# SpaceLearner/SessionRec-pytorch

Measured on AMD Instinct MI355X. Metric: sessions/sec training, Yoochoose-1/64 batch 512, higher is better.
Workload: dtype bf16 (MFMA operands; fp32 accumulate, master weights, scoring); 1 GPU; MSGIFSR training step, synthetic Yoochoose-1/64 shape (V=37484 items, d=256, batch 512 per GPU, session length<=20, order 3, dropout 0.1); global_batch=512, parallelism=single GPU

## Files before the change

### include/srec.h

```cpp
#ifndef SREC_H
#define SREC_H
#include "srec_hg.h"

#ifdef __cplusplus
extern "C" {
#endif

#define SREC_BAD_ARG 1001

int srec_gemm_f32(const float* A, int a_rs, int a_cs, const float* B, int b_rs, int b_cs, float* C, int ldc,
                  const float* bias, int M, int N, int K, const int* dyn, int dyn_mode, float alpha, float beta,
                  float* ws, long ws_floats, void* stream);

int srec_gemm_bf16_nt(const float* A, int lda, const float* B, int ldb, float* C, int ldc, const float* bias, int M,
                      int N, int K, const int* dyn, float alpha, float beta, float* ws, long ws_floats, void* stream);

int srec_gemm_bf16_tn(const float* A, int lda, const float* B, int ldb, float* C, int ldc, int Mred, int N, int K,
                      const int* dyn, float alpha, float beta, float* ws, long ws_floats, void* stream);

int srec_ce_plan(int B, int V, int d, int* n_item_tiles, int* n_ranges);
int srec_score_ce_fwd(const float* sr, int ld_sr, const float* E, int ld_e, const float* cs, const int* labels,
                      int B, int V, int d, const int* dynB, float* ws_stats, float* lab_logit, float* lse,
                      float* lossvec, float* loss, void* stream);
int srec_score_ce_bwd(const float* sr, int ld_sr, const float* E, int ld_e, const float* cs, const int* labels,
                      const float* lse, const float* gscale, const float* ga, const float* gc, int B, int V, int d,
                      const int* dynB, float* dE, int ld_de, float* ws_dsr, float* dsr, int parts, void* stream);
int srec_score_logp(const float* sr, int ld_sr, const float* E, int ld_e, const float* cs, const float* lse, int B,
                    int V, int d, const int* dynB, float* logp, long ld_logp, void* stream);

int srec_bf16_prepare(const float* src, int ld, int R, const int* dynR, int d, void* dst16, void* dstT16, int Rp,
                      void* stream);
int srec_ce_plan_bf16(int B, int V, int d, int* n_stat_slabs, int* n_ranges, int* d_pad);
int srec_score_ce_fwd_bf16(const void* sr16, int Bp, const void* E16, int Vp, const float* cs, const int* labels,
                           int B, int V, int d, const int* dynB, float* ws_stats, float* lab_logit, float* lse,
                           float* lossvec, float* loss, void* stream);
int srec_score_ce_bwd_bf16(const void* sr16, float* ws_de, int Bp, const void* E16, const void* ET16, int Vp,
                           const float* cs, const int* labels, const float* lse, const float* gscale, const float* ga,
                           const float* gc, int B, int V, int d, const int* dynB, float* dE, int ld_de, float* ws_dsr,
                           float* dsr, int parts, void* stream);
int srec_ce_de_split(int B, int V, int d, int* split);

int srec_gather_rows(const float* src, int ld_src, const int* idx, float* out, int ld_out, int n_cap,
                     const int* dyn, int d, void* stream);
int srec_expand_rows_sorted(const float* g, int ld_g, const int* idx, int n_cap, const int* dyn, int nrows, int d,
                            float* dst, int ld_dst, void* stream);
int srec_scatter_add_sorted(const float* g, int ld_g, const int* items, const int* ptr, const int* pos, float* dst,
                            int ld_dst, int u_cap, const int* dyn, int d, int accumulate, void* stream);
int srec_gather_rows_drop(const float* src, int ld_src, const int* idx, float* out, int ld_out, int n_cap, const int* dyn,
                          int d, float p, int seed, const int* counter, int salt, void* stream);
int srec_scatter_add_sorted_drop(const float* g, int ld_g, const int* items, const int* ptr, const int* pos, float* dst,
                                 int ld_dst, int u_cap, const int* dyn, int d, int accumulate, float p, int seed,
                                 const int* counter, int salt, void* stream);
int srec_scatter_add_sorted_ex(const float* g, int ld_g, const int* items, const int* ptr, const int* pos, float* dst,
                               int ld_dst, int u_cap, const int* dyn, int d, int accumulate, float p, int seed,
                               const int* counter, int salt, const float* projW, int ld_w, float* radial, void* stream);
int srec_add_rows_ranks(const float* rows, int d, const int* rel, const int* ids, int w, int ucap, float* dst, int ld_dst,
                        const float* projW, int ld_w, float* radial, void* stream);
int srec_renorm_rows(float* W, int ld, const int* idx, int n_cap, const int* dyn, int d, float max_norm,
                     void* stream);
int srec_renorm_rows_bf16(float* W, int ld, int n, int d, float max_norm, void* dst16, int Dp, void* stream);
int srec_row_invnorm(const float* W, int ld, int n, int d, int eps_mode, float eps, float scale, float* out,
                     void* stream);
int srec_normalize_fwd(const float* X, int ld_x, float* Y, int ld_y, float* inv, int n_cap, const int* dyn, int d,
                       int eps_mode, float eps, void* stream);
int srec_normalize_fwd_bf16(const float* X, int ld_x, float* Y, int ld_y, float* inv, int n_cap, const int* dyn, int d,
                            int eps_mode, float eps, void* dst16, int Dp, void* stream);
int srec_normalize_bwd(const float* Y, int ld_y, const float* dY, int ld_dy, const float* inv, float* dX, int ld_dx,
                       int n_cap, const int* dyn, int d, void* stream);
int srec_normalize_group_fwd(int np, const void* X, const int* ld, const int* n, const void* dyn, float* Y, int ld_y,
                             float* inv, int d, int eps_mode, float eps, void* stream);
int srec_normalize_group_bwd(int np, const void* dX, const int* ld, const int* n, const void* dyn, const float* Y, int ld_y,
                             const float* dY, int ld_dy, const float* inv, int d, void* stream);
int srec_cat_cols(const float* a, int lda, int da, const float* b, int ldb, int db, int n, float* out, void* stream);
int srec_rownorm_project(const float* W, int ld_w, const float* cs, float inv_scale, float* G, int ld_g, int n, int d,
                         void* stream);
int srec_rownorm_project_radial(const float* W, int ld_w, const float* cs, float inv_scale, float* G, int ld_g, int n, int d,
                                float* radial, void* stream);
int srec_col_sum(const float* X, int ld, const float* wgt, int H, int D, int n_cap, const int* dyn, int ncol,
                 float* out, int accumulate, float* ws, void* stream);

int srec_limits(int* max_session_nodes, int* max_degree, int* max_degree_sgat);

int srec_copy_words(const int* src, int* dst, long n, void* stream);
int srec_copy_words_mailbox(const int* mailbox, int M, const int* counter, int* dst, long cap, int* err, void* stream);

int srec_seg_attn_fwd(const float* U, int ld_u, const float* Vq, int ld_v, const float* we, const float* X, int ld_x,
                      const int* seg, int B, const int* dynB, int h, int D, float* alpha, float* out, int ld_out, void* stream);
int srec_seg_attn_bwd(const float* dout, int ld_do, const float* X, int ld_x, const float* alpha, const float* U,
                      int ld_u, const float* Vq, int ld_v, const float* we, const int* seg, int B, const int* dynB,
                      int h, int D, int n_cap, float* dX, int ld_dx, float* dU, int ld_du, float* dVq, int ld_dv,
                      float* dwe_part, int ld_dw, void* stream);
int srec_seg_mean_add_fwd(const float* H, int ld_h, const float* F, int ld_f, const int* seg, int B, const int* dynB,
                          int D, float* out, int ld_out, void* stream);
int srec_seg_mean_add_bwd(const float* dout, int ld_do, const int* seg, int B, const int* dynB, int D, float* dF,
                          int ld_df, void* stream);

int srec_head_dot(const float* X, int ld, const float* a, int n_cap, const int* dyn, int H, int D, float* out,
                  void* stream);
int srec_gat_agg_fwd(const float* Fs, int ld_s, const float* el, const float* er, const int* in_ptr,
                     const int* in_idx, const int* esrc, int nd_cap, const int* dyn_nd, int H, int D, float slope,
                     float* A, float* rst, int ld_r, void* stream);
int srec_gat_bwd_dst(const float* dR, int ld_r, const float* Fs, int ld_s, const float* el, const float* er,
                     const float* A, const int* in_ptr, const int* in_idx, const int* esrc, int nd_cap,
                     const int* dyn_nd, int H, int D, float slope, float* DP, float* der, void* stream);
int srec_gat_bwd_src(const float* dR, int ld_r, const float* A, const float* DP, const float* attn_l,
                     const int* out_ptr, const int* out_idx, const int* edst, int ns_cap, const int* dyn_ns, int H,
                     int D, float* dFs, int ld_s, float* del, const float* der, const float* attn_r, void* stream);
int srec_head_outer(const float* wgt, const float* a, int n_cap, const int* dyn, int H, int D, float* out, int ld,
                    void* stream);
int srec_head_combine_fwd(const float* const* rsts, int n_rst, int ld_r, const float* x, int ld_x, const float* bias,
                          float nres, int n_cap, const int* dyn, int H, int D, float* out, int ld_o,
                          unsigned char* arg, void* stream);
int srec_head_combine_bwd(const float* dout, int ld_o, const unsigned char* arg, int n_cap, const int* dyn, int H,
                          int D, float* dR, int ld_r, void* stream);

int srec_gru_pointwise_fwd(const float* GI, int ld_gi, const float* GH, int ld_gh, const float* bhh, const float* Hp,
                           int ld_hp, int n_cap, const int* dyn, int d, float* Hn, int ld_hn, float* gates,
                           void* stream);
int srec_gru_pointwise_bwd(const float* dHn, int ld_dh, const float* gates, const float* GH, int ld_gh,
                           const float* bhh, const float* Hp, int ld_hp, int n_cap, const int* dyn, int d, float* dGI,
                           int ld_dgi, float* dGH, int ld_dgh, float* dHp, int ld_dhp, void* stream);
int srec_gram_combine_fwd(const float* X, const float* Hl, int ld_h, int n_cap, const int* dyn, int k, int d,
                          float* out, int ld_o, void* stream);
int srec_gram_combine_bwd(const float* dout, int ld_o, int n_cap, const int* dyn, int k, int d, float* dX, float* dHl,
                          int ld_h, void* stream);

int srec_edge_coef(const int* ptr, const int* idx, const int* ew, int n_cap, const int* dyn, float* coef,
                   void* stream);
int srec_edge_agg(const float* X, int ld_x, const int* ptr, const int* idx, const int* other, const float* coef,
                  int n_cap, const int* dyn, int D, float* out, int ld_o, void* stream);

int srec_bn_fwd_train(const float* X, int ld_x, int n_cap, const int* dyn, int D, const float* gamma, const float* beta,
                      float eps, float momentum, float* rmean, float* rvar, long long* nbt, float* mean, float* var,
                      float* Y, int ld_y, float* ws, void* stream);
int srec_bn_apply_fwd(const float* X, int ld_x, const float* mean, const float* var, float eps, const float* gamma,
                      const float* beta, int n_cap, const int* dyn, int D, float* Y, int ld_y, void* stream);
int srec_bn_bwd(const float* dY, int ld_dy, const float* X, int ld_x, const float* mean, const float* var, float eps,
                const float* gamma, int training, int n_cap, const int* dyn, int D, float* dX, int ld_dx,
                float* dgamma, float* dbeta, float* ws, void* stream);
int srec_prelu_fwd(const float* X, int ld_x, const float* a, int n_cap, const int* dyn, int D, float* Y, int ld_y,
                   void* stream);
int srec_prelu_bwd(const float* dY, int ld_dy, const float* X, int ld_x, const float* a, int n_cap, const int* dyn,
                   int D, float* dX, int ld_dx, float* da, float* ws, void* stream);
int srec_gru_seq_fwd(const float* GI, int ld_gi, const float* Whh, const float* WhhT, const float* bhh,
                     const int* in_ptr, const int* in_idx, const int* esrc, int n_cap, const int* dyn, int D,
                     float* neigh, int ld_n, float* gates, float* Hprev, float* ghn, void* stream);
int srec_gru_seq_bwd(const float* dneigh, int ld_dn, const float* Whh, const float* gates, const float* Hprev,
                     const float* ghn, const int* in_ptr, const int* in_idx, int n_cap, const int* dyn, int D,
                     float* dGIe, float* dGHe, void* stream);
int srec_sgat_fwd(const float* Q, int ld_q, const float* K, int ld_k, const float* we, const float* Vf, int ld_v,
                  const int* in_ptr, const int* in_idx, const int* esrc, int n_cap, const int* dyn, int Hh, int Do,
                  float* A, float* out, int ld_o, void* stream);
int srec_sgat_bwd_dst(const float* dout, int ld_o, const float* Q, int ld_q, const float* K, int ld_k,
                      const float* we, const float* Vf, int ld_v, const float* A, const int* in_ptr,
                      const int* in_idx, const int* esrc, int n_cap, const int* dyn, int Hh, int Do, float* dQe,
                      float* dK, int ld_dk, float* dwe_part, int ld_dw, void* stream);
int srec_sgat_bwd_src(const float* dout, int ld_o, const float* A, const float* dQe, const int* out_ptr,
                      const int* out_idx, const int* edst, int n_cap, const int* dyn, int Hh, int Do, float* dQ,
                      int ld_dq, float* dVf, int ld_dv, void* stream);

int srec_localize_idx(const long long* idx, long n, long lo, int n_loc, int* out, void* stream);
int srec_localize_idx32(const int* idx, long n, long lo, int n_loc, int* out, float* zero, long zero_from, void* stream);

int srec_inverse_index(const int* ptr, const int* pos, int U, int n, int* inv, void* stream);
int srec_merge_stats(const float* st, int w, int B, const long long* lab_all, float* lse, float* lab, float* loss,
                     float* gw, void* stream);
int srec_merge_stats32(const float* st, int w, int B, const int* lab_all, float* lse, float* lab, float* loss,
                       float* gw, void* stream);

int srec_adam_flat(float* p, const float* g, float* m, float* v, long n, const float* hyper, int use_wd,
                   void* stream);
int srec_adam_hyper(int* counter, const void* cfg, float* hyper, void* stream);
int srec_adam_hyper_multi(int n, const void* counter, const void* cfg, const void* hyper, const int* tap_counter,
                          const float* tap_src, float* tap_ring, int tap_n, const int* skip, void* stream);
typedef struct srec_adam_multi_desc {
    int nt;
    const int* use_wd;
    const long* numel;
    float* const* p;
    const float* const* g;
    float* const* m;
    float* const* v;
} srec_adam_multi_desc;
int srec_adam_multi(const void* desc, const float* hyper, void* stream);
int srec_adam_rows(float* W, const float* G, float* M, float* V, int n, int d, int ld, const float* hyper,
                   int use_wd, float max_norm, int renorm_write, float* cs_out, float cs_scale, int eps_mode,
                   float cs_eps, void* dst16, int Dp, void* stream);
int srec_adam_rows_proj(float* W, const float* G, float* M, float* V, int n, int d, int ld, const float* hyper, int use_wd,
                        float max_norm, int renorm_write, float* cs_out, float cs_scale, int eps_mode, float cs_eps,
                        const float* proj_cs, float proj_inv_scale, float* radial, void* dst16, int Dp, void* stream);

int srec_hg_ws_floats(const void* desc, long* n_floats);
int srec_hg_fwd(const void* desc, const float* x, int ld_x, float* out, int ld_out, unsigned char* arg, void* stream);
int srec_hg_fold(const void* desc, void* stream);
int srec_step_prep(const void* desc, void* stream);
int srec_hg_drop_prep(const float* x, const float* cnt, int rows, int D, float p, int seed, const int* counter, int salt,
                      float* ms, float* xc, float* rm, float* xres, float pa, long na, float* mk, void* stream);
int srec_hg_drop_prep16(const float* x, const float* cnt, int rows, int D, float p, int seed, const int* counter, int salt,
                        float* ms, float* xc, float* rm, float* xres, float pa, long na, float* mk, void* xc16, void* stream);
int srec_hg_drop_merge(const float* t, int S, const float* ms, long n, float* dx, float p, int seed, const int* counter,
                       int salt, void* stream);
int srec_hg_pre_merge(const void* desc, const float* g, int ld_g, const float* t, int S, float* dx, int ld_dx, void* stream);
int srec_hg_bwd(const void* desc, const float* x, int ld_x, const float* g, int ld_g, const unsigned char* arg, float* dx,
                int ld_dx, float* ws, void* stream);

int srec_gemm_group_bf16(const void* desc, int mode, void* stream);

int srec_gemm_f32_group_run(const void* desc, float* ws, long ws_floats, void* stream);
int srec_gemm_f32_group_run_defer(const void* desc, float* ws, long ws_floats, long* slab_off, int* slab_n, void* stream);
int srec_gemm16_nt(const void* desc, void* stream);
int srec_gemm16_tn(const void* desc, void* stream);
int srec_rows_bf16(const float* src, int ld, int n, const int* dyn, int d, void* dst16, void* stream);
int srec_sum_slabs(const float* part, int C, int R, long n, float* out, void* stream);
int srec_weights_bf16(int n, const void* W, const void* W16, const void* WT16, const int* R, const int* Cc, void* stream);
int srec_norm_perm_pick_fwd(const float* x, int ld_x, const int* perm, int n_cap, const int* dyn_t, int D, int eps_mode,
                            float eps, float* allf, float* invr, int npick, int B, const int* dyn_b, const void* pick,
                            const void* pout, const int* ld_p, void* stream);
int srec_norm_perm_pick_bwd(const float* allf, const float* invr, const float* g_allf, int ld_g, const int* perm, int n_cap,
                            const int* cat_seg, int B, const int* dyn_b, int D, int npick, const void* pick, const void* g_pick,
                            const int* ld_gp, float* dx, int ld_dx, int nt, const int* row0, const int* ncap, const void* dyn_n,
                            int n_rows, void* stream);
int srec_gru_step_fwd(const void* desc, void* stream);
int srec_gru_step_bwd(const void* desc, void* stream);
int srec_gru_fused_fwd(const void* desc, void* stream);
int srec_gru_wfrag(int n, const void* W, const void* dst, int d, void* stream);
int srec_gru_fused_bwd(const void* desc, void* stream);
int srec_gru_fused_nodes(int np, const int* n, int d, int* nodes);
int srec_gru_fused_wide(int np, const int* n, const int* k, int* mask);
int srec_gru_fused_waves(int d, int* waves);
int srec_gru_wfrag_t(int n, const void* W, const void* dst, int d, void* stream);
int srec_gru_wfrag_both(int n, const void* W, const void* dst_fwd, const void* dst_bwd, int d, void* stream);
int srec_gru_bias_final(int np, const void* part, const int* rows, int ncol, const void* out, void* stream);
int srec_sum_slabs_multi(int np, const void* part, const int* R, const long* n, const void* out, const int* tall,
                         void* stream);
int srec_sum_slabs_multi_ld(int np, const void* part, const int* R, const long* n, const void* out, const int* tall,
                            const int* w, const int* ld, void* stream);
int srec_sum_slabs_multi_hyper(int np, const void* part, const int* R, const long* n, const void* out, const int* tall,
                               const int* w, const int* ld, int nh, const void* counter, const void* cfg, const void* hyper,
                               const int* tap_counter, const float* tap_src, float* tap_ring, int tap_n, const int* skip,
                               void* stream);

int srec_score_topk_ws(int B, int V, int K, long* bytes);
int srec_score_topk(const float* sr, int ld_sr, const float* E, int ld_e, const float* cs, int B, int V, int d, int K,
                    float* out_val, int* out_idx, void* ws, void* stream);

int srec_score_rank_ws(int B, int V, int d, int C, int L, long* bytes);
int srec_score_rank(const float* sr, int ld_sr, long comp_stride, const float* E, int ld_e, const float* cs,
                    const float* off_ex, const float* off_in, const int* listed, int L, const int* labels, long id_lo,
                    int B, int V, int d, int C, float* target, int target_given, int* rank, void* ws, void* stream);

#define SREC_SELECT_MAXK 128
#define SREC_LISTED_SCORE 0
#define SREC_LISTED_DROP 1
int srec_score_select_ws(int B, int V, int d, int C, int L, int K, long* bytes);
int srec_score_select(const float* sr, int ld_sr, long comp_stride, const float* E, int ld_e, const float* cs,
                      const float* off_ex, const float* off_in, const int* listed, int L, int listed_mode,
                      long id_lo, int B, int V, int d, int C, int K,
                      float* out_val, int* out_idx, void* ws, void* stream);

int srec_head_wfrag(int n, const void* W, const void* dst, const int* rows, const int* cols, const int* trans, void* stream);
int srec_head_fwd(const void* desc, void* stream);
int srec_head_bwd(const void* desc, void* stream);

#ifdef __cplusplus
}
#endif
#endif
```

### include/srec_hg.h

```cpp
#ifndef SREC_HG_H
#define SREC_HG_H

#define SREC_HG_MAXT 4
#define SREC_HG_MAXM 8
#define SREC_HG_MAXB 16
#define SREC_HG_MAXI 16

#define SREC_HG_P16_BF16 1
#define SREC_HG_SKIP_DEAD_DP 2
#define SREC_HG_LATE_DX 4
#define SREC_HG_FOLDED 8

typedef struct {
    int H, D, n_types, n_mods, n_blocks, n_inst, B;
    float slope;
    int p16;
    const int* dynB;
    int row0[SREC_HG_MAXT], ncap[SREC_HG_MAXT];
    const int* dyn_n[SREC_HG_MAXT];
    const int* seg[SREC_HG_MAXT];
    const void* P[SREC_HG_MAXM];
    void* dP[SREC_HG_MAXM];
    const float* W[SREC_HG_MAXM];
    float* V[SREC_HG_MAXM];
// ... 128 lines not shown
    const float* H[SREC_GRU_MAXP];
    const float* dout[SREC_GRU_MAXP];
    const void* Wih_f[SREC_GRU_MAXP];
    const void* Whh_f[SREC_GRU_MAXP];
    void* dGI16[SREC_GRU_MAXP];
    void* dGH16[SREC_GRU_MAXP];
    float* dX[SREC_GRU_MAXP];
    float* bias_part[SREC_GRU_MAXP];
    int part_row0[SREC_GRU_MAXP];
} srec_gru_fused_bwd_desc;

#define SREC_HEAD_SESSIONS 16
#define SREC_HEAD_ROWS 64
#define SREC_HEAD_WINDOW 32
#define SREC_HEAD_MAXH 4
#define SREC_HEAD_MAXW 16
typedef struct {
    int nh, d, B, NT, ld_x, ld16, eps_mode;
    float eps;
    const float* X;
    const int* seg;
    const int* dynB;
    float* cat[SREC_HEAD_MAXH];
    const void* Wu_f[SREC_HEAD_MAXH];
    const void* Wv_f[SREC_HEAD_MAXH];
    const void* Wsr_f[SREC_HEAD_MAXH];
    const float* bu[SREC_HEAD_MAXH];
    const float* we[SREC_HEAD_MAXH];
    float* alpha[SREC_HEAD_MAXH];
    float* U[SREC_HEAD_MAXH];
    float* Vq[SREC_HEAD_MAXH];
    float* y[SREC_HEAD_MAXH];
    float* inv[SREC_HEAD_MAXH];
    void* y16[SREC_HEAD_MAXH];
} srec_head_desc;

typedef struct {
    int nh, d, B, NT, ld_x, ld_gy;
    const float* X;
    const int* seg;
    const int* dynB;
    const float* gy[SREC_HEAD_MAXH];
    const float* y[SREC_HEAD_MAXH];
    const float* inv[SREC_HEAD_MAXH];
    const void* WsrT_f[SREC_HEAD_MAXH];
    const float* alpha[SREC_HEAD_MAXH];
    const float* U[SREC_HEAD_MAXH];
    const float* Vq[SREC_HEAD_MAXH];
    const float* we[SREC_HEAD_MAXH];
    float* gs[SREC_HEAD_MAXH];
    float* gcat[SREC_HEAD_MAXH];
    float* dX[SREC_HEAD_MAXH];
    float* dU[SREC_HEAD_MAXH];
    float* dVq[SREC_HEAD_MAXH];
    float* dwp[SREC_HEAD_MAXH];
} srec_head_bwd_desc;

typedef struct {
    const void* hg;
    int n_w16;
    const void* w16_W;
    const void* w16_out;
    const void* w16_T;
    const int* w16_R;
    const int* w16_C;
    int n_gru, gru_d;
    const void* gru_W;
    const void* gru_fwd;
    const void* gru_bwd;
    int n_head;
    const void* head_W;
    const void* head_out;
    const int* head_rows;
    const int* head_cols;
    const int* head_trans;
    const int* mailbox;
    int M;
    const int* counter;
    int* box_dst;
    long box_cap;
    int* box_err;
} srec_step_prep_desc;

#endif
```

### sessionrec-pytorch_amd/csrc/adam.hip

```cpp
#include "common.h"
#include "hyper_role.h"

namespace {

struct Hyper { float step, b1, b2, eps, wd, omb1, omb2, bc2s; };

__device__ __forceinline__ Hyper load_hyper(const float* __restrict__ h) {
    Hyper r{h[0], h[1], h[2], h[3], h[4], h[5], h[6], h[7]};
    return r;
}

__device__ __forceinline__ float adam1(float& p, float g, float& m, float& v, const Hyper& h, float wd,
                                       float step, float bc2s) {
    g += wd * p;
    m = m + h.omb1 * (g - m);
    v = h.b2 * v + h.omb2 * g * g;
    p -= step * (m / (sqrtf(v) / bc2s + h.eps));
    return p;
}

__global__ void adam_flat_kernel(float* __restrict__ p, const float* __restrict__ g, float* __restrict__ m,
                                 float* __restrict__ v, size_t n, const float* __restrict__ hyper, int use_wd) {
    const Hyper h = load_hyper(hyper);
    const float wd = use_wd ? h.wd : 0.f, step = h.step, rs2 = h.bc2s;
    const size_t stride = (size_t)gridDim.x * blockDim.x * 4;
    for (size_t i = ((size_t)blockIdx.x * blockDim.x + threadIdx.x) * 4; i < n; i += stride) {
        if (i + 3 < n) {
            float4 pp = *reinterpret_cast<float4*>(p + i);
            const float4 gg = *reinterpret_cast<const float4*>(g + i);
            float4 mm = *reinterpret_cast<float4*>(m + i);
            float4 vv = *reinterpret_cast<float4*>(v + i);
            adam1(pp.x, gg.x, mm.x, vv.x, h, wd, step, rs2);
            adam1(pp.y, gg.y, mm.y, vv.y, h, wd, step, rs2);
            adam1(pp.z, gg.z, mm.z, vv.z, h, wd, step, rs2);
            adam1(pp.w, gg.w, mm.w, vv.w, h, wd, step, rs2);
            *reinterpret_cast<float4*>(p + i) = pp;
            *reinterpret_cast<float4*>(m + i) = mm;
            *reinterpret_cast<float4*>(v + i) = vv;
        } else {
            for (size_t j = i; j < n; ++j) adam1(p[j], g[j], m[j], v[j], h, wd, step, rs2);
        }
    }
}

template <bool HOLD>
__global__ void adam_rows_kernel(float* __restrict__ W, const float* __restrict__ G, float* __restrict__ M,
                                 float* __restrict__ Vv, int n, int d, int ld, const float* __restrict__ hyper,
                                 int use_wd, float max_norm, int renorm_write, float* __restrict__ cs_out, float cs_scale,
                                 int eps_mode, float cs_eps, const float* __restrict__ proj_cs, float proj_inv_scale,
                                 float* __restrict__ radial, unsigned short* __restrict__ dst16, int Dp) {
    const int i = blockIdx.x * 4 + (threadIdx.x >> 6), lane = threadIdx.x & 63;
    if (i >= n) return;
    const Hyper h = load_hyper(hyper);
    const float wd = use_wd ? h.wd : 0.f, step = h.step, rs2 = h.bc2s;
    if (h.step == 0.f && h.omb1 == 0.f && h.omb2 == 0.f && h.b2 == 1.f) renorm_write = 0;
    const size_t off = (size_t)i * ld;
    float pcoef = 0.f;
    float4 pw[4], gw[4];
    if (HOLD) {
#pragma unroll
        for (int j = 0; j < 4; ++j) {
            const int c = lane * 4 + j * 256;
            pw[j] = make_float4(0.f, 0.f, 0.f, 0.f); gw[j] = pw[j];
            if (c < d) { pw[j] = *reinterpret_cast<const float4*>(W + off + c); gw[j] = *reinterpret_cast<const float4*>(G + off + c); }
        }
    }
    if (proj_cs != nullptr) {
        float dot = 0.f;
        if (HOLD) {
#pragma unroll
            for (int j = 0; j < 4; ++j) dot += pw[j].x * gw[j].x + pw[j].y * gw[j].y + pw[j].z * gw[j].z + pw[j].w * gw[j].w;
        } else {
            for (int c = lane * 4; c < d; c += 256) {
                const float4 pp = *reinterpret_cast<const float4*>(W + off + c);
                const float4 gg = *reinterpret_cast<const float4*>(G + off + c);
                dot += pp.x * gg.x + pp.y * gg.y + pp.z * gg.z + pp.w * gg.w;
            }
        }
        dot = wave_sum(dot);
        const float iv = proj_cs[i] * proj_inv_scale;
        if (radial != nullptr) {
            dot -= radial[i];
            if (lane == 0) radial[i] = 0.f;
        }
        pcoef = dot * iv * iv;
    }
    float ss = 0.f;
    if (HOLD) {
#pragma unroll
        for (int j = 0; j < 4; ++j) {
            const int c = lane * 4 + j * 256;
            if (c < d) {
                float4 pp = pw[j], gg = gw[j];
                gg.x -= pp.x * pcoef; gg.y -= pp.y * pcoef; gg.z -= pp.z * pcoef; gg.w -= pp.w * pcoef;
                float4 mm = *reinterpret_cast<float4*>(M + off + c);
                float4 vv = *reinterpret_cast<float4*>(Vv + off + c);
                adam1(pp.x, gg.x, mm.x, vv.x, h, wd, step, rs2);
                adam1(pp.y, gg.y, mm.y, vv.y, h, wd, step, rs2);
                adam1(pp.z, gg.z, mm.z, vv.z, h, wd, step, rs2);
                adam1(pp.w, gg.w, mm.w, vv.w, h, wd, step, rs2);
                ss += pp.x * pp.x + pp.y * pp.y + pp.z * pp.z + pp.w * pp.w;
                pw[j] = pp;
                *reinterpret_cast<float4*>(M + off + c) = mm;
                *reinterpret_cast<float4*>(Vv + off + c) = vv;
            }
        }
        float nrm = 0.f;
        float sc = 1.f;
        if (max_norm > 0.f || cs_out != nullptr) {
            nrm = sqrtf(wave_sum(ss));
            if (max_norm > 0.f && nrm > max_norm) {
                const float s1 = max_norm / (nrm + 1e-7f);
                if (renorm_write) sc = s1;
                nrm *= s1;
            }
        }
#pragma unroll
        for (int j = 0; j < 4; ++j) {
            const int c = lane * 4 + j * 256;
            float4 pp = pw[j];
            if (sc != 1.f) { pp.x *= sc; pp.y *= sc; pp.z *= sc; pp.w *= sc; }
            if (c < d) *reinterpret_cast<float4*>(W + off + c) = pp;
            if (dst16 != nullptr && c < Dp)
                *reinterpret_cast<uint2*>(dst16 + (size_t)i * Dp + c) = make_uint2(srec_pack_bf16(pp.x, pp.y), srec_pack_bf16(pp.z, pp.w));
        }
        if (cs_out != nullptr && lane == 0)
            cs_out[i] = cs_scale * (eps_mode == 0 ? 1.f / fmaxf(nrm, cs_eps) : 1.f / (nrm + cs_eps));
        return;
    }
    for (int c = lane * 4; c < d; c += 256) {
        float4 pp = *reinterpret_cast<float4*>(W + off + c);
        float4 gg = *reinterpret_cast<const float4*>(G + off + c);
        gg.x -= pp.x * pcoef; gg.y -= pp.y * pcoef; gg.z -= pp.z * pcoef; gg.w -= pp.w * pcoef;
        float4 mm = *reinterpret_cast<float4*>(M + off + c);
        float4 vv = *reinterpret_cast<float4*>(Vv + off + c);
        adam1(pp.x, gg.x, mm.x, vv.x, h, wd, step, rs2);
        adam1(pp.y, gg.y, mm.y, vv.y, h, wd, step, rs2);
        adam1(pp.z, gg.z, mm.z, vv.z, h, wd, step, rs2);
        adam1(pp.w, gg.w, mm.w, vv.w, h, wd, step, rs2);
        ss += pp.x * pp.x + pp.y * pp.y + pp.z * pp.z + pp.w * pp.w;
        *reinterpret_cast<float4*>(W + off + c) = pp;
        *reinterpret_cast<float4*>(M + off + c) = mm;
        *reinterpret_cast<float4*>(Vv + off + c) = vv;
    }
    if (max_norm <= 0.f && cs_out == nullptr) return;
    float nrm = sqrtf(wave_sum(ss));
    if (max_norm > 0.f && nrm > max_norm) {
        const float sc = max_norm / (nrm + 1e-7f);
        for (int c = lane * 4; renorm_write && c < d; c += 256) {
            float4 pp = *reinterpret_cast<float4*>(W + off + c);
            pp.x *= sc; pp.y *= sc; pp.z *= sc; pp.w *= sc;
            *reinterpret_cast<float4*>(W + off + c) = pp;
        }
        nrm *= sc;
    }
    if (cs_out != nullptr && lane == 0)
        cs_out[i] = cs_scale * (eps_mode == 0 ? 1.f / fmaxf(nrm, cs_eps) : 1.f / (nrm + cs_eps));
}

constexpr int MT = 88;
constexpr int MCHUNK = 4096;
struct MultiArgs {
    float* p[MT];
    const float* g[MT];
    float* m[MT];
    float* v[MT];
    int n[MT];
    int blk0[MT + 1];
    unsigned long long wd_mask[2];
    const float* hyper;
    int nt;
};

__global__ __launch_bounds__(256) void adam_multi_kernel(MultiArgs a) {
    int lo = 0, hi = a.nt;
    while (hi - lo > 1) {
        const int mid = (lo + hi) >> 1;
        if (a.blk0[mid] <= (int)blockIdx.x) lo = mid; else hi = mid;
    }
    const int t = lo;
    float* __restrict__ p = a.p[t];
    const float* __restrict__ g = a.g[t];
    float* __restrict__ m = a.m[t];
    float* __restrict__ v = a.v[t];
    const int n = a.n[t];
    const Hyper h = load_hyper(a.hyper);
    const float wd = ((a.wd_mask[t >> 6] >> (t & 63)) & 1ull) ? h.wd : 0.f, step = h.step, rs2 = h.bc2s;
    const int e0 = ((int)blockIdx.x - a.blk0[t]) * MCHUNK;
    const bool vec = ((((uintptr_t)p | (uintptr_t)g | (uintptr_t)m | (uintptr_t)v) & 15) == 0);
#pragma unroll
    for (int u = 0; u < MCHUNK / 1024; ++u) {
        const int i = e0 + u * 1024 + (int)threadIdx.x * 4;
        if (i >= n) break;
        if (vec && i + 3 < n) {
            float4 pp = *reinterpret_cast<float4*>(p + i);
            const float4 gg = *reinterpret_cast<const float4*>(g + i);
            float4 mm = *reinterpret_cast<float4*>(m + i);
            float4 vv = *reinterpret_cast<float4*>(v + i);
            adam1(pp.x, gg.x, mm.x, vv.x, h, wd, step, rs2);
            adam1(pp.y, gg.y, mm.y, vv.y, h, wd, step, rs2);
            adam1(pp.z, gg.z, mm.z, vv.z, h, wd, step, rs2);
            adam1(pp.w, gg.w, mm.w, vv.w, h, wd, step, rs2);
            *reinterpret_cast<float4*>(p + i) = pp;
            *reinterpret_cast<float4*>(m + i) = mm;
            *reinterpret_cast<float4*>(v + i) = vv;
        } else {
            for (int j = i; j < n && j < i + 4; ++j) adam1(p[j], g[j], m[j], v[j], h, wd, step, rs2);
        }
    }
}

}

extern "C" int srec_adam_multi(const void* desc_, const float* hyper, void* stream) {
    struct Desc { int nt; const int* use_wd; const long* numel; float* const* p; const float* const* g; float* const* m; float* const* v; };
    const Desc* d = (const Desc*)desc_;
    if (d == nullptr || d->nt < 0 || hyper == nullptr) return SREC_BAD_ARG;
    for (int t0 = 0; t0 < d->nt; t0 += MT) {
        MultiArgs a{};
        a.nt = d->nt - t0 < MT ? d->nt - t0 : MT;
        a.hyper = hyper;
        int blocks = 0;
        for (int t = 0; t < a.nt; ++t) {
            const int s = t0 + t;
            if (d->numel[s] <= 0 || d->numel[s] > 0x7fffffffL || d->p[s] == nullptr || d->g[s] == nullptr ||
                d->m[s] == nullptr || d->v[s] == nullptr || (((uintptr_t)d->p[s] | (uintptr_t)d->g[s] | (uintptr_t)d->m[s] | (uintptr_t)d->v[s]) & 3))
                return SREC_BAD_ARG;
            a.p[t] = d->p[s]; a.g[t] = d->g[s]; a.m[t] = d->m[s]; a.v[t] = d->v[s];
            a.n[t] = (int)d->numel[s];
            if (d->use_wd[s]) a.wd_mask[t >> 6] |= 1ull << (t & 63);
            a.blk0[t] = blocks;
            blocks += (a.n[t] + MCHUNK - 1) / MCHUNK;
        }
        a.blk0[a.nt] = blocks;
        hipLaunchKernelGGL(adam_multi_kernel, dim3(blocks), dim3(256), 0, (hipStream_t)stream, a);
    }
    SREC_LAUNCH_CHECK();
    return 0;
}

namespace {
__global__ void adam_hyper_kernel(int* __restrict__ counter, const double* __restrict__ cfg, float* __restrict__ hyper) {
    if (threadIdx.x != 0 || blockIdx.x != 0) return;
    const int t = *counter + 1;
    *counter = t;
    const double lr = cfg[0], b1 = cfg[1], b2 = cfg[2], eps = cfg[3], wd = cfg[4];
    hyper[0] = (float)(lr / (1.0 - pow(b1, (double)t)));
    hyper[1] = (float)b1; hyper[2] = (float)b2; hyper[3] = (float)eps; hyper[4] = (float)wd;
    hyper[5] = (float)(1.0 - b1); hyper[6] = (float)(1.0 - b2);
    hyper[7] = (float)sqrt(1.0 - pow(b2, (double)t));
}
}

namespace {
__global__ void adam_hyper_multi_kernel(HyperArgs a) { hyper_role(a, (int)threadIdx.x); }
}

extern "C" int srec_adam_hyper_multi(int n, const void* counter, const void* cfg, const void* hyper, const int* tap_counter,
                                     const float* tap_src, float* tap_ring, int tap_n, const int* skip, void* stream) {
    if (n <= 0) return 0;
    HyperArgs a{};
    if (int rc = hyper_fill(n, counter, cfg, hyper, tap_counter, tap_src, tap_ring, tap_n, skip, a)) return rc;
    hipLaunchKernelGGL(adam_hyper_multi_kernel, dim3(1), dim3(64), 0, (hipStream_t)stream, a);
    SREC_LAUNCH_CHECK();
    return 0;
}

extern "C" int srec_adam_hyper(int* counter, const void* cfg, float* hyper, void* stream) {
    if (counter == nullptr || cfg == nullptr || hyper == nullptr) return SREC_BAD_ARG;
    hipLaunchKernelGGL(adam_hyper_kernel, dim3(1), dim3(64), 0, (hipStream_t)stream, counter, (const double*)cfg, hyper);
    SREC_LAUNCH_CHECK();
    return 0;
}

extern "C" int srec_adam_flat(float* p, const float* g, float* m, float* v, long n, const float* hyper, int use_wd,
                              void* stream) {
    if (n <= 0) return 0;
    if (((uintptr_t)p | (uintptr_t)g | (uintptr_t)m | (uintptr_t)v) & 15) return SREC_BAD_ARG;
    long blocks = (n / 4 + 255) / 256;
    if (blocks > 2048) blocks = 2048;
    if (blocks < 1) blocks = 1;
    hipLaunchKernelGGL(adam_flat_kernel, dim3((unsigned)blocks), dim3(256), 0, (hipStream_t)stream, p, g, m, v,
                       (size_t)n, hyper, use_wd);
    SREC_LAUNCH_CHECK();
    return 0;
}

static int adam_rows_run(float* W, const float* G, float* M, float* V, int n, int d, int ld, const float* hyper, int use_wd,
                         float max_norm, int renorm_write, float* cs_out, float cs_scale, int eps_mode, float cs_eps,
                         const float* proj_cs, float proj_inv_scale, float* radial, void* dst16, int Dp, void* stream) {
    if (n <= 0) return 0;
    if (d <= 0 || (d & 3) || (ld & 3)) return SREC_BAD_ARG;
    if (dst16 != nullptr && (d > 1024 || Dp < d || (Dp & 3) || Dp > 1024)) return SREC_BAD_ARG;
    if (d <= 1024)
        hipLaunchKernelGGL(adam_rows_kernel<true>, dim3(cdiv(n, 4)), dim3(256), 0, (hipStream_t)stream, W, G, M, V, n, d, ld, hyper,
                           use_wd, max_norm, renorm_write, cs_out, cs_scale, eps_mode, cs_eps, proj_cs, proj_inv_scale, radial,
                           (unsigned short*)dst16, Dp);
    else
        hipLaunchKernelGGL(adam_rows_kernel<false>, dim3(cdiv(n, 4)), dim3(256), 0, (hipStream_t)stream, W, G, M, V, n, d, ld, hyper,
                           use_wd, max_norm, renorm_write, cs_out, cs_scale, eps_mode, cs_eps, proj_cs, proj_inv_scale, radial,
                           (unsigned short*)nullptr, 0);
    SREC_LAUNCH_CHECK();
    return 0;
}

extern "C" int srec_adam_rows(float* W, const float* G, float* M, float* V, int n, int d, int ld, const float* hyper,
                              int use_wd, float max_norm, int renorm_write, float* cs_out, float cs_scale, int eps_mode,
                              float cs_eps, void* dst16, int Dp, void* stream) {
    return adam_rows_run(W, G, M, V, n, d, ld, hyper, use_wd, max_norm, renorm_write, cs_out, cs_scale, eps_mode, cs_eps, nullptr,
                         0.f, nullptr, dst16, Dp, stream);
}

extern "C" int srec_adam_rows_proj(float* W, const float* G, float* M, float* V, int n, int d, int ld, const float* hyper,
                                   int use_wd, float max_norm, int renorm_write, float* cs_out, float cs_scale, int eps_mode,
                                   float cs_eps, const float* proj_cs, float proj_inv_scale, float* radial, void* dst16, int Dp,
                                   void* stream) {
    if (proj_cs == nullptr) return SREC_BAD_ARG;
    return adam_rows_run(W, G, M, V, n, d, ld, hyper, use_wd, max_norm, renorm_write, cs_out, cs_scale, eps_mode, cs_eps, proj_cs,
                         proj_inv_scale, radial, dst16, Dp, stream);
}
```

### sessionrec-pytorch_amd/csrc/hgat.hip

```cpp
#include "common.h"
#include "../../include/srec_hg.h"

extern "C" int srec_hg_fold(const void* desc, void* stream);

namespace {

constexpr int WPB = 4;
constexpr int MAXDEG = SREC_MAX_DEGREE;
constexpr int MAXH = 8;
constexpr int NCHUNK_C = 32;
constexpr int SEGCAP = 1025;
constexpr int NCHUNK = 16;
constexpr int MAXT = SREC_HG_MAXT, MAXM = SREC_HG_MAXM, MAXB = SREC_HG_MAXB, MAXI = SREC_HG_MAXI;

typedef __bf16 bf16x4_t __attribute__((ext_vector_type(4)));
typedef float f32x4_t __attribute__((ext_vector_type(4)));
__device__ __forceinline__ float4 ld4(const float* p) { return *reinterpret_cast<const float4*>(p); }
__device__ __forceinline__ float4 ld4(const unsigned short* p) {
    const uint2 v = *reinterpret_cast<const uint2*>(p);
    return make_float4(__uint_as_float(v.x << 16), __uint_as_float(v.x & 0xffff0000u), __uint_as_float(v.y << 16),
                       __uint_as_float(v.y & 0xffff0000u));
}
__device__ __forceinline__ float ld1(const float* p) { return *p; }
__device__ __forceinline__ float ld1(const unsigned short* p) { return __uint_as_float((unsigned)*p << 16); }
__device__ __forceinline__ void st4(float* p, float4 v) { *reinterpret_cast<float4*>(p) = v; }
__device__ __forceinline__ void st4(unsigned short* p, float4 v) {
    const f32x4_t f = {v.x, v.y, v.z, v.w};
    const bf16x4_t b = __builtin_convertvector(f, bf16x4_t);
    *reinterpret_cast<uint2*>(p) = __builtin_bit_cast(uint2, b);
}

template <int N>
__device__ __forceinline__ int find_range(const int (&start)[N], int n, int x) {
    int b = 0;
#pragma unroll
    for (int i = 1; i < N; ++i)
        if (i < n && x >= start[i]) b = i;
    return b;
}

struct DotsArgs {
    const float* V[MAXB];
    float* eL[MAXB]; float* eR[MAXB];
    const int* dyn[MAXB];
    int ncap[MAXB], row0[MAXB];
    int start[MAXB + 1];
    int nb, H, D;
    const float* x[MAXB]; int ld_x;
    int nt, B; const int* dynB;
    const int* seg[MAXT]; int trow0[MAXT];
    const float* xm;
    float* smean[MAXT]; int* sess;
};

#ifndef SREC_DOTS_NODES
#define SREC_DOTS_NODES 64
#endif
constexpr int DOTS_NODES = SREC_DOTS_NODES;
typedef float f32x4v __attribute__((ext_vector_type(4)));
__global__ __launch_bounds__(256) void hg_dots_kernel(DotsArgs a) {
    extern __shared__ float vt[];
    if ((int)blockIdx.x >= a.start[a.nb]) {
        const int e = (int)blockIdx.x - a.start[a.nb], t = e / a.B, sb = e - t * a.B;
        if (t >= a.nt || sb >= dyn_count(a.dynB, a.B)) return;
        const int s0 = a.seg[t][sb], s1 = a.seg[t][sb + 1];
        for (int j = s0 + (int)threadIdx.x; j < s1; j += 256) a.sess[a.trow0[t] + j] = sb;
        for (int c = threadIdx.x; c < a.D; c += 256) {
            const float* xp = a.xm + (size_t)a.trow0[t] * a.ld_x + c;
            float m = 0.f;
            int j = s0;
            for (; j + 3 < s1; j += 4) {
                const float x0 = xp[(size_t)j * a.ld_x], x1 = xp[(size_t)(j + 1) * a.ld_x], x2 = xp[(size_t)(j + 2) * a.ld_x],
                            x3 = xp[(size_t)(j + 3) * a.ld_x];
                m += x0; m += x1; m += x2; m += x3;
            }
            for (; j < s1; ++j) m += xp[(size_t)j * a.ld_x];
            a.smean[t][(size_t)sb * a.D + c] = m / (float)(s1 - s0 > 0 ? s1 - s0 : 1);
        }
        return;
    }
    const int b = find_range(a.start, a.nb, (int)blockIdx.x);
    const int H = a.H, D = a.D, LDV = D + 4;
    const int Dp = (D + 15) & ~15;
    for (int i = threadIdx.x; i < 16 * LDV + 16; i += 256) vt[i] = 0.f;
    __syncthreads();
    if ((H & 3) == 0) {
// ... 609 lines not shown
    const int c = lane * 4;
    float4 g4 = make_float4(0.f, 0.f, 0.f, 0.f);
    uchar4 a4 = make_uchar4(0, 0, 0, 0);
    if (c < D) {
        const size_t row = (size_t)(a.row0_d[i] + v);
        g4 = *reinterpret_cast<const float4*>(a.g + row * a.ld_g + c);
        a4 = *reinterpret_cast<const uchar4*>(a.arg + row * D + c);
    }
    const T* P = static_cast<const T*>(a.Ps[i]);
    for (int j = 0; j < deg; ++j) {
        float ph[MAXH];
#pragma unroll
        for (int h = 0; h < MAXH; ++h) ph[h] = 0.f;
        if (c < D) {
            const T* pr = P + (size_t)su[w][j] * HD + c;
            const float v0 = g4.x * ld1(pr + a4.x * D), v1 = g4.y * ld1(pr + a4.y * D + 1);
            const float v2 = g4.z * ld1(pr + a4.z * D + 2), v3 = g4.w * ld1(pr + a4.w * D + 3);
#pragma unroll
            for (int h = 0; h < MAXH; ++h)
                ph[h] = (a4.x == h ? v0 : 0.f) + (a4.y == h ? v1 : 0.f) + (a4.z == h ? v2 : 0.f) + (a4.w == h ? v3 : 0.f);
        }
        {
            const bool b0 = lane & 1, b1 = lane & 2, b2 = lane & 4;
            float q4[4];
#pragma unroll
            for (int k = 0; k < 4; ++k) {
                const float keep = b0 ? ph[k + 4] : ph[k], send = b0 ? ph[k] : ph[k + 4];
                q4[k] = keep + __shfl_xor(send, 1, 64);
            }
            float q2[2];
#pragma unroll
            for (int k = 0; k < 2; ++k) {
                const float keep = b1 ? q4[k + 2] : q4[k], send = b1 ? q4[k] : q4[k + 2];
                q2[k] = keep + __shfl_xor(send, 2, 64);
            }
            float t = (b2 ? q2[1] : q2[0]) + __shfl_xor(b2 ? q2[0] : q2[1], 4, 64);
            t += __shfl_xor(t, 8, 64); t += __shfl_xor(t, 16, 64); t += __shfl_xor(t, 32, 64);
            const int hb = (b0 ? 4 : 0) + (b1 ? 2 : 0) + (b2 ? 1 : 0);
            if (lane < MAXH) {
                if (a.Mk[i] != nullptr && hb < H) t *= a.Mk[i][(size_t)idx[j] * H + hb];
                da[w][j][hb] = t;
            }
        }
    }
    __builtin_amdgcn_wave_barrier();
    if (hl >= H) return;
    float tsum = 0.f;
    for (int j = jl; j < deg; j += 8) tsum += a.A[i][(size_t)idx[j] * H + hl] * da[w][j][hl];
    tsum += __shfl_xor(tsum, 8, 64); tsum += __shfl_xor(tsum, 16, 64); tsum += __shfl_xor(tsum, 32, 64);
    const float erv = a.eRd[i][(size_t)v * H + hl];
    float dsum = 0.f;
    for (int j = jl; j < deg; j += 8) {
        const int e = idx[j];
        const float p = a.A[i][(size_t)e * H + hl];
        const float pre = a.eLs[i][(size_t)su[w][j] * H + hl] + erv;
        const float dp = p * (da[w][j][hl] - tsum) * (pre > 0.f ? 1.f : a.slope);
        a.DP[i][(size_t)e * H + hl] = dp;
        dsum += dp;
    }
    dsum += __shfl_xor(dsum, 8, 64); dsum += __shfl_xor(dsum, 16, 64); dsum += __shfl_xor(dsum, 32, 64);
    if (jl == 0) a.der[i][(size_t)v * H + hl] = dsum;
}

__device__ __forceinline__ float head_sums8(const float (&ph)[MAXH], int lane, int* hb) {
    const bool b0 = lane & 1, b1 = lane & 2, b2 = lane & 4;
    float q4[4];
#pragma unroll
    for (int k = 0; k < 4; ++k) {
        const float keep = b0 ? ph[k + 4] : ph[k], send = b0 ? ph[k] : ph[k + 4];
        q4[k] = keep + __shfl_xor(send, 1, 64);
    }
    float q2[2];
#pragma unroll
    for (int k = 0; k < 2; ++k) {
        const float keep = b1 ? q4[k + 2] : q4[k], send = b1 ? q4[k] : q4[k + 2];
        q2[k] = keep + __shfl_xor(send, 2, 64);
    }
    float t = (b2 ? q2[1] : q2[0]) + __shfl_xor(b2 ? q2[0] : q2[1], 4, 64);
    t += __shfl_xor(t, 8, 64); t += __shfl_xor(t, 16, 64); t += __shfl_xor(t, 32, 64);
    *hb = (b0 ? 4 : 0) + (b1 ? 2 : 0) + (b2 ? 1 : 0);
    return t;
}

template <typename T, int DIF, int WV>
__global__ __launch_bounds__(256, WV) void hg_bwd_dst_node_kernel(DstArgs a) {
    __shared__ float da[WPB][MAXDEG][MAXH];
    __shared__ int su[WPB][MAXDEG];
    const int w = __builtin_amdgcn_readfirstlane(threadIdx.x >> 6), lane = threadIdx.x & 63;
    HGT_BEGIN();
    const int row = blockIdx.x * WPB + w;
    if (row >= a.row0_t[a.nt]) return;
    const int t = find_range(a.row0_t, a.nt, row);
    const int v = row - a.row0_t[t];
    const int H = a.H, D = a.D, HD = H * D;
    const int ni = a.ninst_t[t];
    if (v >= dyn_count(a.dyn_t[t], a.ncap_t[t])) {
        for (int q = 0; q < ni; ++q)
            if (lane < H) a.der[a.inst_t[t][q]][(size_t)v * H + lane] = 0.f;
        return;
    }
    const int q = lane >> 3, j = lane & 7;
    int i = -1, beg = 0, deg = 0;
    if (q < ni && q < 8) {
        i = a.inst_t[t][q];
        beg = a.in_ptr[i][v];
        deg = a.in_ptr[i][v + 1] - beg;
    }
    const int c = lane * 4;
    float4 g4 = make_float4(0.f, 0.f, 0.f, 0.f);
    uchar4 a4 = make_uchar4(0, 0, 0, 0);
    if (c < D) {
        g4 = *reinterpret_cast<const float4*>(a.g + (size_t)row * a.ld_g + c);
        a4 = *reinterpret_cast<const uchar4*>(a.arg + (size_t)row * D + c);
    }
    const bool valid = i >= 0 && j < deg;
    HGT_W(1);
    int e = 0, src = 0;
    if (valid) {
        e = a.in_idx[i][beg + j];
        src = a.esrc[i][e];
    }
    HGT_W(2);
    if (__ballot(deg > 8) != 0ull) {
        for (int qq = 0; qq < ni; ++qq) {
            const int ig = a.inst_t[t][qq];
            const int bg = a.in_ptr[ig][v];
            const int dg = min(a.in_ptr[ig][v + 1] - bg, MAXDEG);
            const int* idx = a.in_idx[ig] + bg;
            for (int jj = lane; jj < dg; jj += 64) su[w][jj] = a.esrc[ig][idx[jj]];
            __builtin_amdgcn_wave_barrier();
            const T* P = static_cast<const T*>(a.Ps[ig]);
            for (int jj = 0; jj < dg; ++jj) {
                float ph[MAXH];
#pragma unroll
                for (int h = 0; h < MAXH; ++h) ph[h] = 0.f;
                if (c < D) {
                    const T* pr = P + (size_t)su[w][jj] * HD + c;
                    const float v0 = g4.x * ld1(pr + a4.x * D), v1 = g4.y * ld1(pr + a4.y * D + 1);
                    const float v2 = g4.z * ld1(pr + a4.z * D + 2), v3 = g4.w * ld1(pr + a4.w * D + 3);
#pragma unroll
                    for (int h = 0; h < MAXH; ++h)
                        ph[h] = (a4.x == h ? v0 : 0.f) + (a4.y == h ? v1 : 0.f) + (a4.z == h ? v2 : 0.f) + (a4.w == h ? v3 : 0.f);
                }
                int hb;
                float ts = head_sums8(ph, lane, &hb);
                if (lane < MAXH) {
                    if (a.Mk[ig] != nullptr && hb < H) ts *= a.Mk[ig][(size_t)idx[jj] * H + hb];
                    da[w][jj][hb] = ts;
                }
            }
            __builtin_amdgcn_wave_barrier();
            const int hl = lane & 7, jl = lane >> 3;
            if (hl < H) {
                float tsum = 0.f;
                for (int jj = jl; jj < dg; jj += 8) tsum += a.A[ig][(size_t)idx[jj] * H + hl] * da[w][jj][hl];
                tsum += __shfl_xor(tsum, 8, 64); tsum += __shfl_xor(tsum, 16, 64); tsum += __shfl_xor(tsum, 32, 64);
                const float erv = a.eRd[ig][(size_t)v * H + hl];
                float dsum = 0.f;
                for (int jj = jl; jj < dg; jj += 8) {
                    const int ee = idx[jj];
                    const float p = a.A[ig][(size_t)ee * H + hl];
                    const float pre = a.eLs[ig][(size_t)su[w][jj] * H + hl] + erv;
                    const float dp = p * (da[w][jj][hl] - tsum) * (pre > 0.f ? 1.f : a.slope);
                    a.DP[ig][(size_t)ee * H + hl] = dp;
                    dsum += dp;
                }
                dsum += __shfl_xor(dsum, 8, 64); dsum += __shfl_xor(dsum, 16, 64); dsum += __shfl_xor(dsum, 32, 64);
                if (jl == 0) a.der[ig][(size_t)v * H + hl] = dsum;
            }
            __builtin_amdgcn_wave_barrier();
        }
        return;
    }
// ... 37 lines not shown
#pragma unroll
        for (int u = 0; u < DIF; ++u) {
            const bool on = mask != 0ull;
            const int l = on ? __builtin_ctzll(mask) : 0;
            if (on) mask &= mask - 1ull;
            ls[u] = on ? l : -1;
            const int ii = __builtin_amdgcn_readlane(i, l), ss = __builtin_amdgcn_readlane(src, l);
            const T* rp = static_cast<const T*>(a.Ps[ii >= 0 ? ii : 0]) + (size_t)ss * HD + half * D + c8;
#pragma unroll
            for (int k = 0; k < 4; ++k)
                if (on && cok8) f[u][k].load(rp + 2 * k * D); else f[u][k].zero();
        }
#pragma unroll
        for (int u = 0; u < DIF; ++u) {
            if (ls[u] < 0) break;
            float ph[4];
#pragma unroll
            for (int k = 0; k < 4; ++k) {
                float fv[8];
                f[u][k].get(fv);
                float sacc = 0.f;
#pragma unroll
                for (int x = 0; x < 8; ++x) sacc += (kx[x] == k ? gsel[x] : 0.f) * fv[x];
                ph[k] = sacc;
            }
            const bool b0 = lane & 1, b1 = lane & 2;
            const float k0 = b0 ? ph[2] : ph[0], s0 = b0 ? ph[0] : ph[2];
            const float k1 = b0 ? ph[3] : ph[1], s1 = b0 ? ph[1] : ph[3];
            const float q0 = k0 + __shfl_xor(s0, 1, 64), q1 = k1 + __shfl_xor(s1, 1, 64);
            float ts = (b1 ? q1 : q0) + __shfl_xor(b1 ? q0 : q1, 2, 64);
            ts += __shfl_xor(ts, 4, 64); ts += __shfl_xor(ts, 8, 64); ts += __shfl_xor(ts, 16, 64);
            const int hb = 2 * ((b0 ? 2 : 0) + (b1 ? 1 : 0)) + half;
            if ((lane & 28) == 0) da[w][ls[u]][hb] = ts;
        }
    }
    HGT_W(4);
    __builtin_amdgcn_wave_barrier();
    float dv[8];
    ld8f(&da[w][lane][0], dv);
    float dp[8];
#pragma unroll
    for (int h = 0; h < 8; ++h) {
        const float d_a = valid ? dv[h] * mk[h] : 0.f;
        float tsum = valid ? pa[h] * d_a : 0.f;
        tsum += __shfl_xor(tsum, 1, 64); tsum += __shfl_xor(tsum, 2, 64); tsum += __shfl_xor(tsum, 4, 64);
        dp[h] = valid ? pa[h] * (d_a - tsum) * ((pos >> h) & 1u ? 1.f : a.slope) : 0.f;
    }
    if (valid) {
        float* o = a.DP[i] + (size_t)e * 8;
        *reinterpret_cast<float4*>(o) = make_float4(dp[0], dp[1], dp[2], dp[3]);
        *reinterpret_cast<float4*>(o + 4) = make_float4(dp[4], dp[5], dp[6], dp[7]);
    }
#pragma unroll
    for (int h = 0; h < 8; ++h) {
        float dsum = dp[h];
        dsum += __shfl_xor(dsum, 1, 64); dsum += __shfl_xor(dsum, 2, 64); dsum += __shfl_xor(dsum, 4, 64);
        dp[h] = dsum;
    }
    if (i >= 0 && j == 0) {
        float* o = a.der[i] + (size_t)v * 8;
        *reinterpret_cast<float4*>(o) = make_float4(dp[0], dp[1], dp[2], dp[3]);
        *reinterpret_cast<float4*>(o + 4) = make_float4(dp[4], dp[5], dp[6], dp[7]);
    }
    HGT_W(5);
    HGT_END();
}

struct SrcArgs {
    void* dP[MAXB]; float* wL[MAXB]; float* wR[MAXB];
    const float* al[MAXB]; const float* ar[MAXB];
    const int* dyn[MAXB];
    int ncap[MAXB], nsrc[MAXB], ndst[MAXB], src[MAXB][4], dst[MAXB][4];
    int start[MAXB + 1];
    const float* A[MAXI]; const float* DP[MAXI]; const float* der[MAXI]; const float* Mk[MAXI];
    const int* out_ptr[MAXI]; const int* out_idx[MAXI]; const int* edst[MAXI];
    int row0_d[MAXI];
    int nb, H, D;
    const float* g; int ld_g;
    const unsigned char* arg;
    int skip_dead;
};

constexpr int WPB_SRC = 4;
template <typename T, int WV, bool DER_FIRST>
__global__ __launch_bounds__(64 * WPB_SRC, WV) void hg_bwd_src_kernel(SrcArgs a) {
    extern __shared__ __attribute__((aligned(16))) float alr[];
    HGT_BEGIN();
    const int b = find_range(a.start, a.nb, (int)blockIdx.x);
    const int lane = threadIdx.x & 63;
    const int u = ((int)blockIdx.x - a.start[b]) * WPB_SRC + (threadIdx.x >> 6);
    const int H = a.H, D = a.D, HD = H * D;
    {
        const float* al = a.al[b]; const float* ar = a.ar[b];
        for (int i = threadIdx.x * 4; i < HD; i += 64 * WPB_SRC * 4) {
            *reinterpret_cast<float4*>(alr + i) = *reinterpret_cast<const float4*>(al + i);
            *reinterpret_cast<float4*>(alr + HD + i) = *reinterpret_cast<const float4*>(ar + i);
        }
    }
    const bool in_range = u < a.ncap[b];
    const bool live = in_range && u < dyn_count(a.dyn[b], a.ncap[b]);
    const int c = lane * 4, hl = lane & 7, jl = lane >> 3;
    float4 o[MAXH];
#pragma unroll
    for (int h = 0; h < MAXH; ++h) o[h] = make_float4(0.f, 0.f, 0.f, 0.f);
    float wl = 0.f, wr = 0.f;
    if (DER_FIRST && live && hl < H)
        for (int q = 0; q < a.ndst[b]; ++q) wr += a.der[a.dst[b][q]][(size_t)u * H + hl];
    bool fast = false;
    if (H == MAXH) {
        const int sl = lane >> 4, j = lane & 15;
        int i = -1, beg = 0, deg = 0;
        if (live && sl < a.nsrc[b]) {
            i = a.src[b][sl];
            beg = a.out_ptr[i][u];
            deg = a.out_ptr[i][u + 1] - beg;
        }
        fast = __ballot(deg > 16) == 0ull;
        if (fast) {
            const bool valid = i >= 0 && j < deg;
            int drow = 0;
            float p8[8], d8[8];
#pragma unroll
            for (int h = 0; h < 8; ++h) { p8[h] = 0.f; d8[h] = 0.f; }
            if (valid) {
                const int e = a.out_idx[i][beg + j];
                drow = a.row0_d[i] + a.edst[i][e];
                ld8f(a.DP[i] + (size_t)e * 8, d8);
                ld8f(a.A[i] + (size_t)e * 8, p8);
                if (a.Mk[i] != nullptr) {
                    float m8[8];
                    ld8f(a.Mk[i] + (size_t)e * 8, m8);
#pragma unroll
                    for (int h = 0; h < 8; ++h) p8[h] *= m8[h];
                }
            }
            HGT_W(1);
            {
                int hb;
                const float ts = head_sums8(d8, lane, &hb);
                const int rev = ((hl & 1) << 2) | (hl & 2) | ((hl & 4) >> 2);
                wl = __shfl(ts, rev, 64);
            }
            unsigned long long mask = __ballot(valid);
            while (mask != 0ull) {
                constexpr int SIF = 2;
                float4 gv[SIF]; uchar4 bi[SIF]; int ls[SIF];
#pragma unroll
                for (int x = 0; x < SIF; ++x) {
                    const bool on = mask != 0ull;
                    const int l = on ? __builtin_ctzll(mask) : 0;
                    if (on) mask &= mask - 1ull;
                    ls[x] = on ? l : -1;
                    const size_t row = (size_t)__builtin_amdgcn_readlane(drow, l);
                    gv[x] = make_float4(0.f, 0.f, 0.f, 0.f); bi[x] = make_uchar4(255, 255, 255, 255);
                    if (on && c < D) {
                        gv[x] = *reinterpret_cast<const float4*>(a.g + row * a.ld_g + c);
                        bi[x] = *reinterpret_cast<const uchar4*>(a.arg + row * D + c);
                    }
                }
#pragma unroll
                for (int x = 0; x < SIF; ++x) {
                    if (ls[x] < 0) break;
#pragma unroll
                    for (int h = 0; h < MAXH; ++h) {
                        const float ph = rdlane(p8[h], ls[x]);
                        o[h].x += bi[x].x == h ? ph * gv[x].x : 0.f; o[h].y += bi[x].y == h ? ph * gv[x].y : 0.f;
                        o[h].z += bi[x].z == h ? ph * gv[x].z : 0.f; o[h].w += bi[x].w == h ? ph * gv[x].w : 0.f;
                    }
                }
// ... 341 lines not shown
            const int m = d->blk_mod[b], t = d->blk_type[b];
            a.V[b] = d->V[m];
            a.x[b] = d->xin[m] != nullptr ? d->xin[m] : x;
            a.eL[b] = d->eL[b]; a.eR[b] = d->eR[b];
            a.dyn[b] = d->dyn_n[t]; a.ncap[b] = d->ncap[t]; a.row0[b] = d->row0[t];
            a.start[b] = blocks;
            blocks += cdiv(d->ncap[t], DOTS_NODES);
        }
        a.start[d->n_blocks] = blocks;
        a.nt = d->n_types; a.B = d->B; a.dynB = d->dynB; a.xm = x; a.sess = d->sess;
        for (int t = 0; t < d->n_types; ++t) { a.seg[t] = d->seg[t]; a.trow0[t] = d->row0[t]; a.smean[t] = d->smean[t]; }
        blocks += d->n_types * d->B;
        if (blocks > 0) hipLaunchKernelGGL(hg_dots_kernel, dim3(blocks), dim3(256), (size_t)(16 * (D + 4) + 16) * 4, st, a);
    }
    AggArgs g{};
    g.nt = d->n_types; g.B = d->B; g.dynB = d->dynB; g.H = H; g.D = D; g.slope = d->slope;
    g.x = x; g.ld_x = ld_x; g.out = out; g.ld_out = ld_out; g.arg = arg; g.xres = d->xres; g.sess = d->sess;
    for (int t = 0; t < d->n_types; ++t) g.smean[t] = d->smean[t];
    int rows = 0;
    for (int t = 0; t < d->n_types; ++t) {
        if (d->row0[t] != rows) return SREC_BAD_ARG;
        g.seg[t] = d->seg[t]; g.dyn_n[t] = d->dyn_n[t]; g.row0[t] = d->row0[t]; g.ncap[t] = d->ncap[t];
        g.ninst[t] = 0;
        g.bsum[t] = d->Z[t];
        rows += d->ncap[t];
    }
    g.row0[d->n_types] = rows;
    for (int i = 0; i < d->n_inst; ++i) {
        const int sb = d->inst_sblk[i], db = d->inst_dblk[i], m = d->inst_mod[i], t = d->blk_type[db];
        if (g.ninst[t] >= 8) return SREC_BAD_ARG;
        g.inst[t][g.ninst[t]++] = i;
        g.Ps[i] = (const char*)d->P[m] + (size_t)d->blk_row[sb] * HD * esz;
        g.eLs[i] = d->eL[sb]; g.eRd[i] = d->eR[db]; g.bias[i] = d->bias[m];
        g.in_ptr[i] = d->in_ptr[i]; g.in_idx[i] = d->in_idx[i]; g.esrc[i] = d->esrc[i];
        g.A[i] = d->A[i]; g.Mk[i] = d->Mk[i];
    }
    if (rows > 0) {
        auto al16 = [](const void* p) { return ((size_t)p & 15) == 0; };
        bool node = H == MAXH && (D & 7) == 0 && (ld_x & 3) == 0 && (ld_out & 3) == 0 && al16(out) && al16(arg) &&
                    al16(x) && al16(g.xres);
        for (int t = 0; node && t < d->n_types; ++t) node = al16(g.smean[t]) && (g.ninst[t] == 0 || al16(g.bsum[t]));
        for (int i = 0; node && i < d->n_inst; ++i)
            node = al16(g.Ps[i]) && al16(g.eLs[i]) && al16(g.eRd[i]) && al16(g.A[i]) && al16(g.Mk[i]);
        if (node) {
            if (d->p16 & SREC_HG_P16_BF16) hipLaunchKernelGGL((hg_agg_node_kernel<unsigned short, 1, 5>), dim3(cdiv(rows, WPB)), dim3(64 * WPB), 0, st, g);
            else hipLaunchKernelGGL((hg_agg_node_kernel<float, 2, 3>), dim3(cdiv(rows, WPB)), dim3(64 * WPB), 0, st, g);
        } else if (d->p16 & SREC_HG_P16_BF16) hipLaunchKernelGGL(hg_agg_kernel<unsigned short>, dim3(rows), dim3(512), 0, st, g);
        else hipLaunchKernelGGL(hg_agg_kernel<float>, dim3(rows), dim3(512), 0, st, g);
    }
    SREC_LAUNCH_CHECK();
    return 0;
}

static int fill_pre(const srec_hg_desc* d, const float* g, int ld_g, float* dx, int ld_dx, PreArgs& a) {
    int ninst_t[MAXT] = {0, 0, 0, 0};
    for (int i = 0; i < d->n_inst; ++i) ninst_t[d->blk_type[d->inst_dblk[i]]]++;
    a.nt = d->n_types; a.B = d->B; a.D = d->D; a.dynB = d->dynB; a.g = g; a.ld_g = ld_g; a.dx = dx; a.ld_dx = ld_dx; a.rm = d->rm;
    a.rm_cnt = d->rm_cnt; a.rm_p = d->rm_p; a.rm_rng = srec_rng{(unsigned)d->rm_seed, d->rm_counter, (unsigned)d->rm_salt, d->rm_p};
    a.sess = d->sess;
    if (d->sess == nullptr) return SREC_BAD_ARG;
    int rows = 0;
    for (int t = 0; t < d->n_types; ++t) {
        a.seg[t] = d->seg[t]; a.dyn_n[t] = d->dyn_n[t]; a.row0[t] = d->row0[t]; a.ncap[t] = d->ncap[t];
        a.ninst[t] = ninst_t[t];
        rows += d->ncap[t];
    }
    a.row0[d->n_types] = rows;
    return 0;
}

extern "C" int srec_hg_pre_merge(const void* desc_, const float* g, int ld_g, const float* t, int S, float* dx, int ld_dx,
                                 void* stream) {
    const srec_hg_desc* d = (const srec_hg_desc*)desc_;
    if (bad_desc(d) || (ld_g & 3) || (ld_dx & 3) || t == nullptr || S < 1 || d->rm_cnt == nullptr) return SREC_BAD_ARG;
    PreArgs a{};
    if (int rc = fill_pre(d, g, ld_g, dx, ld_dx, a)) return rc;
    const int rows = a.row0[d->n_types];
    if ((long)2 * rows * d->D > 0xffffffffL) return SREC_BAD_ARG;
    if (rows > 0) hipLaunchKernelGGL(hg_pre_kernel<true>, dim3(cdiv(rows, WPB)), dim3(256), 0, (hipStream_t)stream, a, t, S);
    SREC_LAUNCH_CHECK();
    return 0;
}

extern "C" int srec_hg_bwd(const void* desc_, const float* x, int ld_x, const float* g, int ld_g, const unsigned char* arg,
                           float* dx, int ld_dx, float* ws, void* stream) {
    const srec_hg_desc* d = (const srec_hg_desc*)desc_;
    if (bad_desc(d) || (ld_g & 3) || (ld_dx & 3) || (ld_x & 3) || ws == nullptr) return SREC_BAD_ARG;
    hipStream_t st = (hipStream_t)stream;
    const int H = d->H, D = d->D, HD = H * D;
    const size_t esz = (d->p16 & SREC_HG_P16_BF16) ? 2 : 4;
    int ninst_t[MAXT] = {0, 0, 0, 0};
    for (int i = 0; i < d->n_inst; ++i) ninst_t[d->blk_type[d->inst_dblk[i]]]++;
    int rows = 0;
    for (int t = 0; t < d->n_types; ++t) rows += d->ncap[t];
    if (!(d->p16 & SREC_HG_LATE_DX)) {
        PreArgs a{};
        if (int rc = fill_pre(d, g, ld_g, dx, ld_dx, a)) return rc;
        if (rows > 0) hipLaunchKernelGGL(hg_pre_kernel<false>, dim3(cdiv(rows, WPB)), dim3(256), 0, st, a, (const float*)nullptr, 0);
    }
    if (d->n_inst > 0) {
        DstArgs a{};
        a.ni = d->n_inst; a.H = H; a.D = D; a.slope = d->slope; a.g = g; a.ld_g = ld_g; a.arg = arg;
        int blocks = 0;
        for (int i = 0; i < d->n_inst; ++i) {
            const int sb = d->inst_sblk[i], db = d->inst_dblk[i], m = d->inst_mod[i], t = d->blk_type[db];
            a.Ps[i] = (const char*)d->P[m] + (size_t)d->blk_row[sb] * HD * esz;
            a.eLs[i] = d->eL[sb]; a.eRd[i] = d->eR[db]; a.A[i] = d->A[i];
            a.in_ptr[i] = d->in_ptr[i]; a.in_idx[i] = d->in_idx[i]; a.esrc[i] = d->esrc[i];
            a.DP[i] = d->DP[i]; a.der[i] = d->der[i]; a.Mk[i] = d->Mk[i];
            a.dyn_d[i] = d->dyn_n[t]; a.ncap_d[i] = d->ncap[t]; a.row0_d[i] = d->row0[t];
            a.start[i] = blocks;
            blocks += cdiv(d->ncap[t], WPB);
        }
        a.start[d->n_inst] = blocks;
        auto al16 = [](const void* p) { return ((size_t)p & 15) == 0; };
        bool node = H == MAXH && (D & 7) == 0 && al16(g) && al16(arg);
        a.nt = d->n_types;
        int trows = 0;
        for (int t = 0; t < d->n_types; ++t) {
            a.dyn_t[t] = d->dyn_n[t]; a.row0_t[t] = d->row0[t]; a.ncap_t[t] = d->ncap[t]; a.ninst_t[t] = 0;
            trows += d->ncap[t];
        }
        a.row0_t[d->n_types] = trows;
        for (int i = 0; i < d->n_inst; ++i) {
            const int t = d->blk_type[d->inst_dblk[i]];
            if (a.ninst_t[t] >= 8) { node = false; continue; }
            a.inst_t[t][a.ninst_t[t]++] = i;
            node = node && al16(a.A[i]) && al16(a.Mk[i]) && al16(a.eLs[i]) && al16(a.eRd[i]) && al16(a.DP[i]) && al16(a.der[i]);
        }
        if (node && trows > 0) {
            if (d->p16 & SREC_HG_P16_BF16) hipLaunchKernelGGL((hg_bwd_dst_node_kernel<unsigned short, 2, 4>), dim3(cdiv(trows, WPB)), dim3(256), 0, st, a);
            else hipLaunchKernelGGL((hg_bwd_dst_node_kernel<float, 1, 3>), dim3(cdiv(trows, WPB)), dim3(256), 0, st, a);
        } else if (blocks > 0) {
            if (d->p16 & SREC_HG_P16_BF16) hipLaunchKernelGGL(hg_bwd_dst_kernel<unsigned short>, dim3(blocks), dim3(256), 0, st, a);
            else hipLaunchKernelGGL(hg_bwd_dst_kernel<float>, dim3(blocks), dim3(256), 0, st, a);
        }
    }
    if (d->n_blocks > 0) {
        SrcArgs a{};
        a.nb = d->n_blocks; a.H = H; a.D = D; a.g = g; a.ld_g = ld_g; a.arg = arg;
        a.skip_dead = (d->p16 & SREC_HG_SKIP_DEAD_DP) ? 1 : 0;
        int blocks = 0;
        for (int b = 0; b < d->n_blocks; ++b) {
            const int m = d->blk_mod[b], t = d->blk_type[b];
            a.dP[b] = (char*)d->dP[m] + (size_t)d->blk_row[b] * HD * esz;
            a.wL[b] = d->wL[b]; a.wR[b] = d->wR[b]; a.al[b] = d->attn_l[m]; a.ar[b] = d->attn_r[m];
            a.dyn[b] = d->dyn_n[t]; a.ncap[b] = d->ncap[t];
            a.nsrc[b] = a.ndst[b] = 0;
            a.start[b] = blocks;
            blocks += cdiv(d->ncap[t], WPB_SRC);
        }
        a.start[d->n_blocks] = blocks;
        for (int i = 0; i < d->n_inst; ++i) {
            const int sb = d->inst_sblk[i], db = d->inst_dblk[i];
            if (a.nsrc[sb] >= 4 || a.ndst[db] >= 4) return SREC_BAD_ARG;
            a.src[sb][a.nsrc[sb]++] = i;
            a.dst[db][a.ndst[db]++] = i;
            a.A[i] = d->A[i]; a.DP[i] = d->DP[i]; a.der[i] = d->der[i]; a.Mk[i] = d->Mk[i];
            a.out_ptr[i] = d->out_ptr[i]; a.out_idx[i] = d->out_idx[i]; a.edst[i] = d->edst[i];
            a.row0_d[i] = d->row0[d->blk_type[db]];
        }
        if (blocks > 0) {
            const size_t lds = (size_t)2 * HD * sizeof(float);
            if (d->p16 & SREC_HG_P16_BF16) hipLaunchKernelGGL((hg_bwd_src_kernel<unsigned short, 6, false>), dim3(blocks), dim3(64 * WPB_SRC), lds, st, a);
            else hipLaunchKernelGGL((hg_bwd_src_kernel<float, 4, false>), dim3(blocks), dim3(64 * WPB_SRC), lds, st, a);
        }
    }
    {
        ColArgs a{};
        a.nt = d->n_types; a.nm = d->n_mods; a.H = H; a.D = D; a.g = g; a.ld_g = ld_g; a.arg = arg; a.part = ws;
        a.ld_x = ld_x;
        for (int b = 0; b < d->n_blocks; ++b) {
            const int m = d->blk_mod[b], t = d->blk_type[b];
            a.xb[b] = d->xin[m] != nullptr ? d->xin[m] : x;
            a.wL[b] = d->wL[b]; a.wR[b] = d->wR[b]; a.dyn_b[b] = d->dyn_n[t]; a.ncap_b[b] = d->ncap[t];
            a.row0_b[b] = d->row0[t];
            if (a.mod_nb[m] >= 4) return SREC_BAD_ARG;
            a.mod_blk[m][a.mod_nb[m]++] = b;
        }
        int r = 0;
        for (int t = 0; t < d->n_types; ++t) {
            a.dyn_t[t] = d->dyn_n[t]; a.row0[t] = d->row0[t]; a.ncap_t[t] = d->ncap[t];
            r += d->ncap[t];
        }
        a.row0[d->n_types] = r;
        const bool cols = H == 8 && D <= 256 && (D & 3) == 0 && (a.ld_x & 3) == 0 && (a.ld_g & 3) == 0;
        ColFinalArgs f{};
        f.nm = d->n_mods; f.H = H; f.D = D; f.part = ws;
        if (cols) {
            hipLaunchKernelGGL(hg_colsum_cols_kernel, dim3(NCHUNK_C, d->n_types + d->n_blocks), dim3(256), 0, st, a);
            f.nchunk = NCHUNK_C;
        } else {
            hipLaunchKernelGGL(hg_colsum_part_kernel, dim3(cdiv(HD, 64), NCHUNK, d->n_types + d->n_mods), dim3(256), 0, st, a);
            f.nchunk = NCHUNK;
        }
        for (int m = 0; m < d->n_mods; ++m) {
            f.out[m] = d->d_bias[m];
            f.out[d->n_mods + m] = d->Z[m];
            if (cols) {
                for (int q = 0; q < a.mod_nb[m]; ++q) f.jobs[d->n_mods + m][f.njob[d->n_mods + m]++] = d->n_types + a.mod_blk[m][q];
            } else {
                f.njob[d->n_mods + m] = 1;
                f.jobs[d->n_mods + m][0] = d->n_types + m;
            }
        }
        for (int i = 0; i < d->n_inst; ++i) {
            const int m = d->inst_mod[i], t = d->blk_type[d->inst_dblk[i]];
            if (f.njob[m] >= 8) return SREC_BAD_ARG;
            f.jobs[m][f.njob[m]++] = t;
        }
        if (d->n_mods > 0) {
            hipLaunchKernelGGL(hg_colsum_final_kernel, dim3(cdiv(2 * HD, 256), 2 * d->n_mods), dim3(256), 0, st, f);
            DattnArgs q{};
            q.H = H; q.D = D;
            for (int m = 0; m < d->n_mods; ++m) { q.W[m] = d->W[m]; q.Z[m] = d->Z[m]; q.dal[m] = d->d_attn_l[m]; q.dar[m] = d->d_attn_r[m]; }
            hipLaunchKernelGGL(hg_dattn_kernel, dim3(d->n_mods * HD / WPB), dim3(256), 0, st, q);
        }
    }
    SREC_LAUNCH_CHECK();
    return 0;
}

namespace {
__global__ void hg_drop_prep_kernel(const float* __restrict__ x, const float* __restrict__ cnt, long n, int D, long rows,
                                    float p, srec_rng rng, float* __restrict__ ms, float* __restrict__ xc,
                                    float* __restrict__ rm, float* __restrict__ xres, int nb1, float pa, long na,
                                    float* __restrict__ mk, unsigned short* __restrict__ xc16) {
    const unsigned key = srec_rng_key(rng);
    if ((int)blockIdx.x >= nb1) {
        const long j = ((long)((int)blockIdx.x - nb1) * blockDim.x + threadIdx.x) * 4;
        const float sa = 1.f / (1.f - pa);
        for (int e = 0; e < 4; ++e)
            if (j + e < na) mk[j + e] = srec_keep(key ^ 0xA5A5A5A5u, (unsigned)(j + e), pa, sa);
        return;
    }
    const long i = ((long)blockIdx.x * blockDim.x + threadIdx.x) * 4;
    if (i >= n) return;
    const float sc = p > 0.f ? 1.f / (1.f - p) : 1.f;
    const long row = i / D;
    const float c0 = cnt[row], c1 = cnt[rows + row];
    const float4 xv = *reinterpret_cast<const float4*>(x + i);
    float4 m0, m1;
    const unsigned i0 = (unsigned)i, i1 = (unsigned)(n + i);
    m0.x = srec_keep(key, i0, p, sc); m0.y = srec_keep(key, i0 + 1, p, sc); m0.z = srec_keep(key, i0 + 2, p, sc); m0.w = srec_keep(key, i0 + 3, p, sc);
    m1.x = srec_keep(key, i1, p, sc); m1.y = srec_keep(key, i1 + 1, p, sc); m1.z = srec_keep(key, i1 + 2, p, sc); m1.w = srec_keep(key, i1 + 3, p, sc);
    if (ms != nullptr) {
        *reinterpret_cast<float4*>(ms + i) = m0;
        *reinterpret_cast<float4*>(ms + n + i) = m1;
    }
    const float4 x0 = make_float4(xv.x * m0.x, xv.y * m0.y, xv.z * m0.z, xv.w * m0.w);
    const float4 x1 = make_float4(xv.x * m1.x, xv.y * m1.y, xv.z * m1.z, xv.w * m1.w);
    *reinterpret_cast<float4*>(xc + i) = x0;
    *reinterpret_cast<float4*>(xc + n + i) = x1;
    if (xc16 != nullptr) {
        *reinterpret_cast<uint2*>(xc16 + i) = make_uint2(srec_pack_bf16(x0.x, x0.y), srec_pack_bf16(x0.z, x0.w));
        *reinterpret_cast<uint2*>(xc16 + n + i) = make_uint2(srec_pack_bf16(x1.x, x1.y), srec_pack_bf16(x1.z, x1.w));
    }
    const float4 r = make_float4(c0 * m0.x + c1 * m1.x, c0 * m0.y + c1 * m1.y, c0 * m0.z + c1 * m1.z, c0 * m0.w + c1 * m1.w);
    if (rm != nullptr) *reinterpret_cast<float4*>(rm + i) = r;
    *reinterpret_cast<float4*>(xres + i) = make_float4(xv.x * r.x, xv.y * r.y, xv.z * r.z, xv.w * r.w);
}

__global__ void hg_drop_merge_kernel(const float* __restrict__ t, int S, const float* __restrict__ ms, long n,
                                     float* __restrict__ dx, float p, srec_rng rng) {
    const long i = ((long)blockIdx.x * blockDim.x + threadIdx.x) * 4;
    if (i >= n) return;
    float4 a = *reinterpret_cast<const float4*>(t + i), b = *reinterpret_cast<const float4*>(t + (size_t)S * n + i);
    for (int s = 1; s < S; ++s) {
        const float4 a2 = *reinterpret_cast<const float4*>(t + (size_t)s * n + i);
        const float4 b2 = *reinterpret_cast<const float4*>(t + (size_t)(S + s) * n + i);
        a.x += a2.x; a.y += a2.y; a.z += a2.z; a.w += a2.w;
        b.x += b2.x; b.y += b2.y; b.z += b2.z; b.w += b2.w;
    }
    float4 m0, m1;
    if (ms != nullptr) {
        m0 = *reinterpret_cast<const float4*>(ms + i); m1 = *reinterpret_cast<const float4*>(ms + n + i);
    } else {
        const unsigned key = srec_rng_key(rng);
        const float sc = p > 0.f ? 1.f / (1.f - p) : 1.f;
        const unsigned i0 = (unsigned)i, i1 = (unsigned)(n + i);
        m0.x = srec_keep(key, i0, p, sc); m0.y = srec_keep(key, i0 + 1, p, sc); m0.z = srec_keep(key, i0 + 2, p, sc); m0.w = srec_keep(key, i0 + 3, p, sc);
        m1.x = srec_keep(key, i1, p, sc); m1.y = srec_keep(key, i1 + 1, p, sc); m1.z = srec_keep(key, i1 + 2, p, sc); m1.w = srec_keep(key, i1 + 3, p, sc);
    }
    float4 d = *reinterpret_cast<float4*>(dx + i);
    d.x += a.x * m0.x + b.x * m1.x; d.y += a.y * m0.y + b.y * m1.y; d.z += a.z * m0.z + b.z * m1.z; d.w += a.w * m0.w + b.w * m1.w;
    *reinterpret_cast<float4*>(dx + i) = d;
}

}

static int hg_drop_prep_run(const float* x, const float* cnt, int rows, int D, float p, int seed, const int* counter,
                            int salt, float* ms, float* xc, float* rm, float* xres, float pa, long na, float* mk,
                            unsigned short* xc16, void* stream) {
    if (rows <= 0) return 0;
    if (D <= 0 || (D & 3) || p < 0.f || p >= 1.f || pa < 0.f || pa >= 1.f) return SREC_BAD_ARG;
    const long n = (long)rows * D;
    if (2 * n > 0xffffffffL || na > 0xffffffffL) return SREC_BAD_ARG;
    const int nb1 = (int)((n / 4 + 255) / 256);
    const int nb2 = (pa > 0.f && na > 0 && mk != nullptr) ? (int)(((na + 3) / 4 + 255) / 256) : 0;
    hipLaunchKernelGGL(hg_drop_prep_kernel, dim3((unsigned)(nb1 + nb2)), dim3(256), 0, (hipStream_t)stream, x, cnt, n, D,
                       (long)rows, p, srec_rng{(unsigned)seed, counter, (unsigned)salt, p}, ms, xc, rm, xres, nb1, pa, na, mk, xc16);
    SREC_LAUNCH_CHECK();
    return 0;
// ... 24 lines not shown
```

### sessionrec-pytorch_amd/csrc/hyper_role.h

```cpp
#pragma once
#include "common.h"

namespace {
constexpr int HYPER_MAX = 16;
struct HyperArgs {
    int* counter[HYPER_MAX]; const double* cfg[HYPER_MAX]; float* hyper[HYPER_MAX]; int n;
    const int* tap_counter; const float* tap_src; float* tap_ring; int tap_n;
    const int* skip;
};

__device__ __forceinline__ void hyper_role(const HyperArgs& a, const int i) {
    if (i >= a.n) return;
    const int t = *a.counter[i] + 1;
    *a.counter[i] = t;
    const bool skip = a.skip != nullptr && *a.skip != 0;
    if (a.tap_ring != nullptr && a.counter[i] == a.tap_counter) a.tap_ring[(t - 1) % a.tap_n] = skip ? __int_as_float(0x7fc00000) : *a.tap_src;
    const double* cfg = a.cfg[i];
    float* hyper = a.hyper[i];
    const double lr = cfg[0], b1 = cfg[1], b2 = cfg[2], eps = cfg[3], wd = cfg[4];
    if (skip) {
        hyper[0] = 0.f; hyper[1] = 1.f; hyper[2] = 1.f; hyper[3] = (float)eps; hyper[4] = 0.f; hyper[5] = 0.f; hyper[6] = 0.f;
        hyper[7] = 1.f;
        return;
    }
    hyper[0] = (float)(lr / (1.0 - pow(b1, (double)t)));
    hyper[1] = (float)b1; hyper[2] = (float)b2; hyper[3] = (float)eps; hyper[4] = (float)wd;
    hyper[5] = (float)(1.0 - b1); hyper[6] = (float)(1.0 - b2);
    hyper[7] = (float)sqrt(1.0 - pow(b2, (double)t));
}

inline int hyper_fill(int n, const void* counter, const void* cfg, const void* hyper, const int* tap_counter, const float* tap_src,
                      float* tap_ring, int tap_n, const int* skip, HyperArgs& a) {
    a = HyperArgs{};
    if (n <= 0) return 0;
    if (n > HYPER_MAX || counter == nullptr || cfg == nullptr || hyper == nullptr) return SREC_BAD_ARG;
    if (tap_ring != nullptr && (tap_counter == nullptr || tap_src == nullptr || tap_n <= 0)) return SREC_BAD_ARG;
    a.n = n;
    a.tap_counter = tap_counter; a.tap_src = tap_src; a.tap_ring = tap_ring; a.tap_n = tap_n; a.skip = skip;
    for (int i = 0; i < n; ++i) {
        a.counter[i] = ((int* const*)counter)[i];
        a.cfg[i] = ((const double* const*)cfg)[i];
        a.hyper[i] = ((float* const*)hyper)[i];
        if (a.counter[i] == nullptr || a.cfg[i] == nullptr || a.hyper[i] == nullptr) return SREC_BAD_ARG;
    }
    return 0;
}
}
```

### sessionrec-pytorch_amd/csrc/rowops.hip

```cpp
#include "common.h"

namespace {

constexpr int WPB = 4;

__global__ void gather_rows_kernel(const float* __restrict__ src, int ld_src, const int* __restrict__ idx,
                                   float* __restrict__ out, int ld_out, int n_cap, const int* __restrict__ dyn,
                                   int d, srec_rng rng) {
    const int row = blockIdx.x * WPB + (threadIdx.x >> 6), lane = threadIdx.x & 63;
    if (row >= n_cap) return;
    const int n = dyn_count(dyn, n_cap);
    const int s = row < n ? idx[row] : -1;
    const bool live = s >= 0;
    const bool drop = rng.p > 0.f;
    const unsigned key = drop ? srec_rng_key(rng) : 0u;
    const float sc = drop ? 1.f / (1.f - rng.p) : 1.f;
    for (int c = lane * 4; c < d; c += 256) {
        float4 v = make_float4(0.f, 0.f, 0.f, 0.f);
        if (live) {
            v = *reinterpret_cast<const float4*>(src + (size_t)s * ld_src + c);
            if (drop) {
                const unsigned i0 = (unsigned)row * (unsigned)d + (unsigned)c;
                v.x *= srec_keep(key, i0, rng.p, sc); v.y *= srec_keep(key, i0 + 1, rng.p, sc);
                v.z *= srec_keep(key, i0 + 2, rng.p, sc); v.w *= srec_keep(key, i0 + 3, rng.p, sc);
            }
        }
        *reinterpret_cast<float4*>(out + (size_t)row * ld_out + c) = v;
    }
}

__global__ void expand_rows_sorted_kernel(const float* __restrict__ g, int ld_g, const int* __restrict__ idx, int n_cap,
                                          const int* __restrict__ dyn, int nrows, int d, float* __restrict__ dst, int ld_dst) {
    const int j = blockIdx.x * WPB + (threadIdx.x >> 6), lane = threadIdx.x & 63;
    if (j >= n_cap) return;
    const int n = dyn_count(dyn, n_cap);
    const float4 z = make_float4(0.f, 0.f, 0.f, 0.f);
    if (j < n) {
        const int hi = idx[j], lo = j > 0 ? idx[j - 1] + 1 : 0;
        for (int r = lo; r < hi; ++r)
            for (int c = lane * 4; c < d; c += 256) *reinterpret_cast<float4*>(dst + (size_t)r * ld_dst + c) = z;
        if (hi >= 0 && hi < nrows)
            for (int c = lane * 4; c < d; c += 256)
                *reinterpret_cast<float4*>(dst + (size_t)hi * ld_dst + c) = *reinterpret_cast<const float4*>(g + (size_t)j * ld_g + c);
    }
    const int tail = n > 0 ? idx[n - 1] + 1 : 0;
    for (int r = tail + j; r < nrows; r += n_cap)
        for (int c = lane * 4; c < d; c += 256) *reinterpret_cast<float4*>(dst + (size_t)r * ld_dst + c) = z;
}

__global__ void scatter_add_sorted_kernel(const float* __restrict__ g, int ld_g, const int* __restrict__ items,
                                          const int* __restrict__ ptr, const int* __restrict__ pos,
                                          float* __restrict__ dst, int ld_dst, int u_cap,
                                          const int* __restrict__ dyn, int d, int accumulate, srec_rng rng,
                                          const float* __restrict__ projW = nullptr, int ld_w = 0,
                                          float* __restrict__ radial = nullptr) {
    const int u = blockIdx.x * WPB + (threadIdx.x >> 6), lane = threadIdx.x & 63;
    if (u >= dyn_count(dyn, u_cap)) return;
    const int beg = ptr[u], end = ptr[u + 1], item = items[u];
    if (item < 0) return;
    float rdot = 0.f;
    if (rng.p > 0.f) {
        const unsigned key = srec_rng_key(rng);
        const float sc = 1.f / (1.f - rng.p);
        for (int c = lane * 4; c < d; c += 256) {
            float4 s = make_float4(0.f, 0.f, 0.f, 0.f);
            auto add = [&](int pp, const float4& v) {
                const unsigned i0 = (unsigned)pp * (unsigned)d + (unsigned)c;
                s.x += v.x * srec_keep(key, i0, rng.p, sc); s.y += v.y * srec_keep(key, i0 + 1, rng.p, sc);
                s.z += v.z * srec_keep(key, i0 + 2, rng.p, sc); s.w += v.w * srec_keep(key, i0 + 3, rng.p, sc);
            };
            int e = beg;
            for (; e + 4 <= end; e += 4) {
                const int p0 = pos[e], p1 = pos[e + 1], p2 = pos[e + 2], p3 = pos[e + 3];
                const float4 v0 = *reinterpret_cast<const float4*>(g + (size_t)p0 * ld_g + c);
                const float4 v1 = *reinterpret_cast<const float4*>(g + (size_t)p1 * ld_g + c);
                const float4 v2 = *reinterpret_cast<const float4*>(g + (size_t)p2 * ld_g + c);
                const float4 v3 = *reinterpret_cast<const float4*>(g + (size_t)p3 * ld_g + c);
                add(p0, v0); add(p1, v1); add(p2, v2); add(p3, v3);
            }
            for (; e < end; ++e) {
                const int pp = pos[e];
                add(pp, *reinterpret_cast<const float4*>(g + (size_t)pp * ld_g + c));
            }
            if (radial != nullptr) {
                const float4 wv = *reinterpret_cast<const float4*>(projW + (size_t)item * ld_w + c);
                rdot += wv.x * s.x + wv.y * s.y + wv.z * s.z + wv.w * s.w;
            }
            float4* o = reinterpret_cast<float4*>(dst + (size_t)item * ld_dst + c);
            if (accumulate) {
                const float4 t = *o;
                s.x += t.x; s.y += t.y; s.z += t.z; s.w += t.w;
            }
// ... 293 lines not shown
    const long long v = (long long)idx[i], r = v - lo;
    out[i] = (v >= 0 && r >= 0 && r < n_loc) ? (int)r : -1;
}

template <typename I>
__global__ __launch_bounds__(1024) void merge_stats_kernel(const float* __restrict__ st, int w, int B, const I* __restrict__ lab_all,
                                                          float* __restrict__ lse, float* __restrict__ lab, float* __restrict__ loss,
                                                          float* __restrict__ gw) {
    __shared__ float red[16];
    __shared__ int cnt[16];
    const int nw = blockDim.x >> 6;
    int c = 0;
    for (int b = threadIdx.x; b < B; b += blockDim.x) c += (lab_all == nullptr || lab_all[b] >= 0) ? 1 : 0;
#pragma unroll
    for (int o = 32; o > 0; o >>= 1) c += __shfl_xor(c, o, 64);
    if ((threadIdx.x & 63) == 0) cnt[threadIdx.x >> 6] = c;
    __syncthreads();
    int n_live = 0;
    for (int i = 0; i < nw; ++i) n_live += cnt[i];
    const float inv = 1.f / (float)(n_live > 0 ? n_live : 1);
    float acc = 0.f;
    for (int b = threadIdx.x; b < B; b += blockDim.x) {
        const bool live = lab_all == nullptr || lab_all[b] >= 0;
        float m = -INFINITY, t = 0.f, l = 0.f;
        for (int r0 = 0; r0 < w; r0 += 8) {
            float sv[8], tv[8];
#pragma unroll
            for (int k = 0; k < 8; ++k) {
                const int r = min(r0 + k, w - 1);
                sv[k] = st[((size_t)r * 2) * B + b];
                tv[k] = st[((size_t)r * 2 + 1) * B + b];
            }
            float mb = m;
#pragma unroll
            for (int k = 0; k < 8; ++k)
                if (r0 + k < w) { mb = fmaxf(mb, sv[k]); t += tv[k]; }
            l *= expf(m - mb);
            if (m == -INFINITY) l = 0.f;
#pragma unroll
            for (int k = 0; k < 8; ++k)
                if (r0 + k < w) l += expf(sv[k] - mb);
            m = mb;
        }
        const float v = m + logf(l);
        lse[b] = v;
        lab[b] = t;
        if (live) acc += v - t;
        if (gw != nullptr) gw[b] = live ? inv : 0.f;
    }
    acc = wave_sum(acc);
    if ((threadIdx.x & 63) == 0) red[threadIdx.x >> 6] = acc;
    __syncthreads();
    if (threadIdx.x == 0) {
        float s = 0.f;
        for (int i = 0; i < nw; ++i) s += red[i];
        loss[0] = s * inv;
    }
}

__global__ void inverse_index_kernel(const int* __restrict__ ptr, const int* __restrict__ pos, int U, int n,
                                     int* __restrict__ inv) {
    const int u = blockIdx.x * WPB + (threadIdx.x >> 6), lane = threadIdx.x & 63;
    if (u >= U) return;
    const int beg = ptr[u], end = ptr[u + 1];
    for (int e = beg + lane; e < end; e += 64) {
        const int p = pos[e];
        if (p >= 0 && p < n) inv[p] = u;
    }
}
__global__ void fill_int_kernel(int* __restrict__ p, int n, int v) {
    const int i = blockIdx.x * blockDim.x + threadIdx.x;
    if (i < n) p[i] = v;
}

inline bool bad_row_args(int d, int ld) { return d <= 0 || (d & 3) || (ld & 3); }

}

extern "C" int srec_gather_rows(const float* src, int ld_src, const int* idx, float* out, int ld_out, int n_cap,
                                const int* dyn, int d, void* stream) {
    if (n_cap <= 0) return 0;
    if (bad_row_args(d, ld_src) || (ld_out & 3)) return SREC_BAD_ARG;
    hipLaunchKernelGGL(gather_rows_kernel, dim3(cdiv(n_cap, WPB)), dim3(256), 0, (hipStream_t)stream, src, ld_src, idx,
                       out, ld_out, n_cap, dyn, d, srec_rng{0u, nullptr, 0u, 0.f});
    SREC_LAUNCH_CHECK();
    return 0;
}

extern "C" int srec_gather_rows_drop(const float* src, int ld_src, const int* idx, float* out, int ld_out, int n_cap,
                                     const int* dyn, int d, float p, int seed, const int* counter, int salt,
                                     void* stream) {
    if (n_cap <= 0) return 0;
    if (bad_row_args(d, ld_src) || (ld_out & 3) || p < 0.f || p >= 1.f || (long)n_cap * d > 0xffffffffL) return SREC_BAD_ARG;
    hipLaunchKernelGGL(gather_rows_kernel, dim3(cdiv(n_cap, WPB)), dim3(256), 0, (hipStream_t)stream, src, ld_src, idx,
                       out, ld_out, n_cap, dyn, d, srec_rng{(unsigned)seed, counter, (unsigned)salt, p});
    SREC_LAUNCH_CHECK();
    return 0;
}

extern "C" int srec_expand_rows_sorted(const float* g, int ld_g, const int* idx, int n_cap, const int* dyn, int nrows, int d,
                                       float* dst, int ld_dst, void* stream) {
    if (n_cap <= 0 || nrows <= 0) return 0;
    if (bad_row_args(d, ld_g) || (ld_dst & 3) || idx == nullptr) return SREC_BAD_ARG;
    hipLaunchKernelGGL(expand_rows_sorted_kernel, dim3(cdiv(n_cap, WPB)), dim3(256), 0, (hipStream_t)stream, g, ld_g, idx, n_cap,
                       dyn, nrows, d, dst, ld_dst);
    SREC_LAUNCH_CHECK();
    return 0;
}

extern "C" int srec_scatter_add_sorted(const float* g, int ld_g, const int* items, const int* ptr, const int* pos,
                                       float* dst, int ld_dst, int u_cap, const int* dyn, int d, int accumulate,
                                       void* stream) {
    if (u_cap <= 0) return 0;
    if (bad_row_args(d, ld_g) || (ld_dst & 3)) return SREC_BAD_ARG;
    hipLaunchKernelGGL(scatter_add_sorted_kernel, dim3(cdiv(u_cap, WPB)), dim3(256), 0, (hipStream_t)stream, g, ld_g,
                       items, ptr, pos, dst, ld_dst, u_cap, dyn, d, accumulate, srec_rng{0u, nullptr, 0u, 0.f});
    SREC_LAUNCH_CHECK();
    return 0;
}

extern "C" int srec_scatter_add_sorted_drop(const float* g, int ld_g, const int* items, const int* ptr, const int* pos,
                                            float* dst, int ld_dst, int u_cap, const int* dyn, int d, int accumulate,
                                            float p, int seed, const int* counter, int salt, void* stream) {
    if (u_cap <= 0) return 0;
    if (bad_row_args(d, ld_g) || (ld_dst & 3) || p < 0.f || p >= 1.f || ld_g != d) return SREC_BAD_ARG;
    hipLaunchKernelGGL(scatter_add_sorted_kernel, dim3(cdiv(u_cap, WPB)), dim3(256), 0, (hipStream_t)stream, g, ld_g,
                       items, ptr, pos, dst, ld_dst, u_cap, dyn, d, accumulate,
                       srec_rng{(unsigned)seed, counter, (unsigned)salt, p});
    SREC_LAUNCH_CHECK();
    return 0;
}

namespace {
__global__ void add_rows_ranks_kernel(const float* __restrict__ rows, int d, const int* __restrict__ rel,
                                      const int* __restrict__ ids, int w, int ucap, float* __restrict__ dst, int ld_dst,
                                      const float* __restrict__ projW, int ld_w, float* __restrict__ radial) {
    const int q = blockIdx.x * WPB + (threadIdx.x >> 6), lane = threadIdx.x & 63;
    if (q >= w * ucap) return;
    const int item = rel[q];
    if (item < 0) return;
    const int r_me = q / ucap, gid = ids[q];
    int found = -1;
    if (lane < w) {
        if (lane == r_me) found = q;
        else {
            const int* L = ids + (size_t)lane * ucap;
            int lo = 0, hi = ucap;
            while (lo < hi) {
                const int mid = (lo + hi) >> 1;
                const int v = L[mid];
                if (v >= 0 && v < gid) lo = mid + 1; else hi = mid;
            }
            if (lo < ucap && L[lo] == gid) found = lane * ucap + lo;
        }
    }
    const unsigned long long have = __ballot(found >= 0);
    if ((have & ((1ull << r_me) - 1ull)) != 0ull) return;
    float rd = 0.f;
    const bool proj = radial != nullptr;
    if (proj && lane == 0) rd = radial[item];
    float dots[16];
#pragma unroll
    for (int k = 0; k < 16; ++k) dots[k] = 0.f;
    for (int c = lane * 4; c < d; c += 256) {
        float4 s = *reinterpret_cast<const float4*>(dst + (size_t)item * ld_dst + c);
        float4 wv = make_float4(0.f, 0.f, 0.f, 0.f);
        if (proj) wv = *reinterpret_cast<const float4*>(projW + (size_t)item * ld_w + c);
        float4 v[16];
#pragma unroll
        for (int k = 0; k < 16; ++k) {
            const int slot = __shfl(found, k, 64);
            v[k] = (k < w && slot >= 0) ? *reinterpret_cast<const float4*>(rows + (size_t)slot * d + c) : make_float4(0.f, 0.f, 0.f, 0.f);
        }
#pragma unroll
        for (int k = 0; k < 16; ++k) {
            if (k < w && ((have >> k) & 1ull)) {
                s.x += v[k].x; s.y += v[k].y; s.z += v[k].z; s.w += v[k].w;
                dots[k] += wv.x * v[k].x + wv.y * v[k].y + wv.z * v[k].z + wv.w * v[k].w;
// ... 493 lines not shown
```

### sessionrec-pytorch_amd/graph.py

```python
import os

import torch

from .batch import FlatBatch


LOSS_RING = 512
_STAGE_SLOTS = 16
_MAILBOX = 64


class GraphedTrainStep:
    def __init__(self, model, optimizer, inputs, labels, after_backward=None, warmup=2):
        import gc
        gc.collect()
        assert all(x.meta.get('padded') for x in inputs), 'graph capture needs capacity-padded batches (collate caps=...)'
        self.model, self.opt, self.after_backward = model, optimizer, after_backward
        self.static_inputs = [FlatBatch(x.buf.clone(), x.layout, dict(x.meta)) for x in inputs]
        self.labels_in_batch = self.static_inputs[0].has('labels') and self.static_inputs[0].cap('labels') == labels.numel()
        self.static_labels = (self.static_inputs[0].field('labels') if self.labels_in_batch else labels.to(torch.int32))
        self._one = torch.ones((), device=labels.device, dtype=torch.float32)
        self._sig = [self._signature(x) for x in inputs]
        snap_o = optimizer.snapshot()
        snap_p = [p.detach().clone() for p in model.parameters()]
        snap_b = [b.detach().clone() for b in model.buffers()]
        T0 = getattr(optimizer, '_T', 0)
        s = self._stream = torch.cuda.Stream()
        try:
            s.wait_stream(torch.cuda.current_stream())
            with torch.cuda.stream(s):
                for _ in range(warmup):
                    self._eager()
            torch.cuda.current_stream().wait_stream(s)
            torch.cuda.synchronize()
        finally:
            self._restore(model, optimizer, snap_p, snap_b, snap_o)
        optimizer.zero_grad(set_to_none=True)
        ms = model.__dict__.get('_srec_state')
        if ms is not None and getattr(model, '_cosine', lambda: None)() is not None and hasattr(model, '_col_scale'):
            with torch.no_grad():
                if hasattr(model, '_prepare_table'):
                    model._prepare_table()
                ms['cs_fresh'] = False
                model._col_scale(ms)
            ms['cs_fresh'] = ms.get('cs') is not None
        ms = model.__dict__.get('_srec_state')
        if ms is not None and getattr(optimizer, 'folds_table_prep', lambda: False)() and hasattr(model, '_table_copy'):
            with torch.no_grad():
                W = model._table()
                mn = float(getattr(model, '_max_norm', 0.0) or 0.0)
                tb = model._table_copy(ms, W)
                ms.pop('table_prepared', None)
                from ._lib import lib as _lib, ptr as _ptr, stream as _stream
                if tb is not None:
                    tb.refresh(W, mn)
                elif mn > 0:
                    _lib.srec_renorm_rows(_ptr(W), W.stride(0), None, W.shape[0], None, W.shape[1], mn, _stream())
                ms['table_prepared'] = (True, tb is not None, W._version)
        import os
        try:
            self.graph = torch.cuda.CUDAGraph(keep_graph=True)
        except TypeError:
            self.graph = torch.cuda.CUDAGraph()
        self.loss_ring, self.last_T = None, None
        self._pending_advance = None
        self._setup_mailbox(optimizer, labels.device)
        if self._mb is not None:
            self.loss_ring = torch.zeros(LOSS_RING, device=labels.device, dtype=torch.float32)
        work = None
        from . import dist as _dist
        self.capture_mode = self._capture_mode()
        self._quiesce_collectives()
        c0 = dict(_dist.STATS)
        err = None
        try:
            with torch.cuda.graph(self.graph, stream=self._stream, capture_error_mode=self.capture_mode):
                try:
                    self._capture_intake()
                    self.loss = self.model.fused_loss(*self.static_inputs, self.static_labels)
                    from . import ops as _ops
                    if _ops.STEP.intake_pending():
                        raise RuntimeError('the model never launched the batch intake of its captured step (ops.flush_intake)')
                    tap = (self.loss.detach(), self.loss_ring) if self._mb is not None else None
                    skip = self._mb['err'] if self._mb is not None else None
                    if hasattr(optimizer, 'hyper_rider') and os.environ.get('SREC_HYPER_RIDER', '1') != '0':
                        optimizer.hyper_rider(tap, skip)
                    self.loss.backward(self._one)
                    if self.after_backward is not None:
                        self.after_backward()
                    work = optimizer._work()
                    optimizer._frozen = work
                    optimizer.advance(work)
                    optimizer.launch(work, tap=tap, skip=skip)
                    if self._mb is not None and (0, 0) not in getattr(optimizer, '_used_keys', ()):
                        raise RuntimeError('captured step does not advance the optimizer step counter the batch mailbox is keyed by')
                except BaseException as e:
                    err = e
                    if os.environ.get('SREC_DEBUG_CAPTURE'):
                        import traceback
                        traceback.print_exception(type(e), e, e.__traceback__)
            if err is not None:
                raise err
        except BaseException:
            self._discard((snap_p, snap_b, snap_o))
            raise
        self.collectives = {k: _dist.STATS[k] - c0[k] for k in c0}
        for _, _, items in work:
            for _, _, st in items:
                st['step'] -= 1
        optimizer._T -= 1
        assert optimizer._T == T0, (optimizer._T, T0)
        self.work = work
        if hasattr(self.graph, 'instantiate'):
            try:
                self.graph.instantiate()
            except Exception:
                pass

    @staticmethod
    def _nccl_group():
        import torch.distributed as dist
        if dist.is_available() and dist.is_initialized():
            try:
                return dist.get_backend() == 'nccl'
            except Exception:
                return False
        return False

    @classmethod
    def _capture_mode(cls):
        m = os.environ.get('SREC_CAPTURE_MODE')
        if m in ('global', 'thread_local', 'relaxed'):
            return m
        return 'thread_local' if cls._nccl_group() else 'global'

    @classmethod
    def _quiesce_collectives(cls):
        if cls._nccl_group():
            torch.cuda.synchronize()
            t = float(os.environ.get('SREC_CAPTURE_SLEEP', '0.3') or 0)
            if t > 0:
                import time
                time.sleep(t)

    def _setup_mailbox(self, optimizer, device):
        self._mb = None
        ent = getattr(optimizer, '_hyper', {}).get((0, 0)) if isinstance(getattr(optimizer, '_hyper', None), dict) else None
        if ent is None or (0, 0) not in getattr(optimizer, '_used_keys', ()) or any(x.buf.numel() % 4 for x in self.static_inputs):
            return
        n = len(self.static_inputs)
        box = torch.zeros(n, _MAILBOX, 4, dtype=torch.int32).pin_memory()
        box[:, :, 3] = -1
        self._mb = dict(box=box, np=box.numpy(), counter=ent['counter'], err=torch.zeros(1, dtype=torch.int32, device=device),
                        events=[], held=[], calls=0)

    def check(self):
        if self._mb is not None and int(self._mb['err'].item()):
            raise RuntimeError('a replayed step found another step count in its batch mailbox than the host wrote: that step and '
                               'every later one were skipped (parameters and optimizer state are those before it)')

    def _capture_intake(self):
        if self._mb is None:
            return
        from . import ops
        ops.STEP.offer_intake([(self._mb['box'][i].data_ptr(), _MAILBOX, self._mb['counter'].data_ptr(), st.buf.data_ptr(),
                                st.buf.numel(), self._mb['err'].data_ptr(), self._mb) for i, st in enumerate(self.static_inputs)])

    def _post(self, i, x, T):
        buf = x.buf
# ... 203 lines not shown
```

### sessionrec-pytorch_amd/hgat.py

```python
import ctypes as _ct
from collections import namedtuple

import torch

from . import ops
from ._lib import CONST, lib, ptr, stream
from .ops import GemmProb, HgDesc, _ld, _rows

DropState = namedtuple('DropState', 'xc xres mk ms rng cnt')


class HgPlan:

    def __init__(self, H, D, slope, B, dynB, types, modules, blocks, insts, mod_conv=None, layer_id=0, live=None):
        self.mod_conv = mod_conv if mod_conv is not None else [0] * len(modules)
        self.layer_id, self.live = layer_id, dict(live or {})
        self.H, self.D, self.slope, self.B, self.dynB = H, D, slope, B, dynB
        self.types, self.modules, self.blocks, self.insts, self._fold = types, modules, blocks, insts, None
        assert (len(types) <= CONST['SREC_HG_MAXT'] and len(modules) <= CONST['SREC_HG_MAXM'] and
                len(blocks) <= CONST['SREC_HG_MAXB'] and len(insts) <= CONST['SREC_HG_MAXI'])

    def put_fold(self, small, lay):
        self._fold = (small, lay)

# ... 68 lines not shown

_HG_WS = {}
_CNT_CACHE = {}


def _inst_counts(plan, NT, dev):
    key = (str(dev), NT, tuple(plan.mod_conv), tuple((m, tuple(plan.types[plan.blocks[db][1]][:2])) for (m, sb, db, gr) in plan.insts))
    cnt = _CNT_CACHE.get(key)
    if cnt is None:
        host = torch.zeros(2, NT, 1)
        for (m, sb, db, gr) in plan.insts:
            t0, nc = plan.types[plan.blocks[db][1]][:2]
            host[plan.mod_conv[m], t0:t0 + nc] += 1.0
        if torch.cuda.is_current_stream_capturing():
            raise RuntimeError('instance counts must be cached by an eager warm-up step before graph capture')
        cnt = _CNT_CACHE[key] = host.to(dev)
    return cnt


def gemm_strategy(mode, D, ldx, n_mods, w_contiguous):
    if mode != 'bf16' or D % 8 or ldx != D or not 0 < n_mods <= 8:
        return 'plain'
    return 'g16' if D % 64 == 0 and w_contiguous else 'grouped'


def _drop_prep(x, plan, drop, strategy):
    (pf, pa), (NT, D), dev, tap = drop, x.shape, x.device, ops.DROP_TAP
    cnt = _inst_counts(plan, NT, dev)
    ms = torch.empty(2, NT, D, device=dev, dtype=torch.float32) if tap is not None else None
    xcs, xres = torch.empty(2, NT, D, device=dev, dtype=torch.float32), torch.empty(NT, D, device=dev)
    sizes = [max(gr[4].numel(), 1) * plan.H for (_, _, _, gr) in plan.insts] if pa > 0 else []
    na = sum(sizes)
    allm = torch.empty(na, device=dev, dtype=torch.float32) if pa > 0 else None
    mk = list(torch.split(allm, sizes)) if pa > 0 else None
    seed, rc = ops.rng_args(dev)
    salt = 101 + 2 * plan.layer_id
    args = (ptr(x), ptr(cnt), NT, D, float(pf), seed, rc, salt, ptr(ms), ptr(xcs), None, ptr(xres), float(pa), na, ptr(allm))
    x16 = torch.empty(2, NT, D, device=dev, dtype=torch.bfloat16) if strategy == 'g16' else None
    if x16 is not None:
        lib.srec_hg_drop_prep16(*args, ptr(x16), stream())
    else:
        lib.srec_hg_drop_prep(*args, stream())
    if tap is not None:
        tap.append(dict(ms=ms.clone(), mk=[m.clone() for m in mk] if mk is not None else None))
    return DropState([xcs[0], xcs[1]], xres, mk, ms, (float(pf), seed, rc, salt), cnt), x16


def _project(xin, x16, plan, params, strategy, dev):
    D, HD, nm = plan.D, plan.H * plan.D, len(plan.modules)
    P = [torch.empty(nr, HD, device=dev, dtype=torch.float32 if strategy == 'plain' else torch.bfloat16)
         for (r0, nr, dyn) in plan.modules]
    if strategy == 'g16':
        w16, wt16 = ops.weights_bf16([params[4 * m] for m in range(nm)])
        xin16 = [x16[cv] for cv in plan.mod_conv] if x16 is not None else [ops.rows_bf16(xin[0])] * nm
        probs = [GemmProb(nc, HD, D, [(xin16[m][t0:t0 + nc], w16[m])], P[m][o:o + nc], dyn_t, mhint=plan.live.get(t0, 0))
                 for m in range(nm) for (o, t0, nc, dyn_t) in plan.pieces(m)]
        for i in range(0, len(probs), ops.G16_MAXP):
            ops.gemm16('nt', probs[i:i + ops.G16_MAXP], D, D, HD, c16=True, keep_dead=True)
        return P, (xin16, wt16)
    if strategy == 'grouped':
        ops.gemm_group(0, [(nr, HD, D, [(xin[m][r0:r0 + nr], params[4 * m])], P[m], dyn)
                           for m, (r0, nr, dyn) in enumerate(plan.modules)], D, D, HD, c16=True)
    else:
        for m, (r0, nr, dyn) in enumerate(plan.modules):
            ops.gemm_nt(xin[m][r0:r0 + nr], _rows(params[4 * m]), P[m], None, dyn, 1 if dyn is not None else 0)
    return P, None


def _backward_graph(ctx, x, g, small, arg, P, params, late_dx):
    plan, nm = ctx.plan, len(ctx.plan.modules)
    cov = [sum(plan.types[bt][1] for bm, bt in plan.blocks if bm == m) for m in range(nm)]
    dP = [torch.empty_like(p) if cov[m] == p.shape[0] else torch.zeros_like(p) for m, p in enumerate(P)]
    grads = [[ops.grad_buf(params[4 * m + 1 + j]).view(-1) for j in range(3)] for m in range(nm)]
    dx = torch.empty(x.shape, device=x.device, dtype=torch.float32)
    flat = [p.reshape(-1) if i % 4 else p for i, p in enumerate(params)]
    desc = plan.fill(HgDesc(), small, ctx.lay, P, dP, flat, grads, ctx.drop)
    desc.p16 |= (CONST['SREC_HG_SKIP_DEAD_DP'] if ctx.strategy == 'g16' else 0) | (CONST['SREC_HG_LATE_DX'] if late_dx else 0)
    n = _ct.c_long()
    lib.srec_hg_ws_floats(_ct.addressof(desc), _ct.addressof(n))
    key = (x.device.index, n.value)
    ws = _HG_WS.get(key)
    if ws is None:
        ws = _HG_WS[key] = torch.empty(max(n.value, 1), device=x.device, dtype=torch.float32)
    lib.srec_hg_bwd(_ct.addressof(desc), ptr(x), _ld(x), ptr(g), _ld(g), ptr(arg), ptr(dx), x.shape[1], ptr(ws), stream())
    return desc, dP, grads, dx


def _backward_data(ctx, dP, params, dx):
    plan, strategy, drop = ctx.plan, ctx.strategy, ctx.drop
    NT, D = dx.shape
    HD, nt = plan.H * D, len(plan.types)
    tgts, S, full = None, 1, False
    if drop is not None:
        nproj = {len(plan.projectors(cv, t)) for cv in (0, 1) for t in range(nt)}
        full = strategy != 'plain' and min(nproj) > 0
        if strategy == 'g16' and full and len(nproj) == 1 and 1 < min(nproj) <= 4:
            S = min(nproj)
        tgts = (torch.empty if full else torch.zeros)(2, S, NT, D, device=dx.device, dtype=torch.float32)
    beta, convs = 0.0 if full else 1.0, (0, 1) if drop is not None else (None,)
    tgt = lambda cv, j=0: dx if cv is None else tgts[cv, j]
    if strategy == 'plain':
        for cv in convs:
            for m, (r0, nr, dyn) in enumerate(plan.modules):
                if cv is None or plan.mod_conv[m] == cv:
                    ops.gemm_nn(dP[m], _rows(params[4 * m]), tgt(cv)[r0:r0 + nr], dyn, 1 if dyn is not None else 0, beta=1.0)
        return tgts, S
    W = ctx.g16[1] if strategy == 'g16' else params[::4]

    def problems(cv):
        out = []
        for t, (t0, nc, dyn_t, _) in enumerate(plan.types):
            mods = plan.projectors(cv, t)
            for j, grp in enumerate([[m] for m in mods] if S > 1 else [mods] if mods else []):
                segs = [(dP[m][t0 - plan.modules[m][0]:][:nc], W[m]) for m in grp]
                out.append(GemmProb(nc, D, HD, segs, tgt(cv, j)[t0:t0 + nc], dyn_t, mhint=plan.live.get(t0, 0)))
        return out
    if strategy == 'grouped':
        for probs in filter(None, map(problems, convs)):
            ops.gemm_group(1, probs, HD, D, D, beta=beta, a16=True)
    else:
        probs = [q for cv in convs for q in problems(cv)]
        for i in range(0, len(probs), ops.G16_MAXP):
            ops.gemm16('nt', probs[i:i + ops.G16_MAXP], HD, HD, D, beta=beta)
    return tgts, S


def _weight_grads(ctx, x, dP, gWs):
    plan, D, HD, nm = ctx.plan, x.shape[1], ctx.plan.H * x.shape[1], len(ctx.plan.modules)
    xin = [ctx.drop.xc[cv] for cv in plan.mod_conv] if ctx.drop is not None else [x] * nm
    if ctx.strategy == 'g16':
        xin16 = ctx.g16[0]
        pcs = [plan.pieces(m) for m in range(nm)]
        slabs = {m: torch.empty(len(pcs[m]), HD, D, device=x.device, dtype=torch.float32) for m in range(nm) if len(pcs[m]) > 1}
        probs = [GemmProb(HD, D, nc, [(dP[m][o:o + nc], xin16[m][t0:t0 + nc])], slabs[m][pi:pi + 1] if m in slabs else gWs[m], dyn_t)
                 for m in range(nm) for pi, (o, t0, nc, dyn_t) in enumerate(pcs[m])]
        for i in range(0, len(probs), ops.G16_MAXP):
            ops.gemm16('tn', probs[i:i + ops.G16_MAXP], HD, D, D)
        if slabs and ops.can_defer(ctx.defer, [ctx.wparams[m] for m in slabs]):
            for m, sl in slabs.items():
                ops.defer_slab_sum(sl, gWs[m])
        elif slabs:
            ops._launch_slab_sums([(sl, gWs[m]) for m, sl in slabs.items()])
    elif ctx.strategy == 'grouped':
        ops.gemm_group(2, [(HD, D, nr, [(dP[m], xin[m][r0:r0 + nr])], gWs[m], dyn)
                           for m, (r0, nr, dyn) in enumerate(plan.modules)], HD, D, D, a16=True)
    else:
        for m, (r0, nr, dyn) in enumerate(plan.modules):
            ops.gemm_tn(dP[m], xin[m][r0:r0 + nr], gWs[m], dyn)


class HGATLayer(torch.autograd.Function):

    @staticmethod
    def forward(ctx, x, plan, drop, *params):
        x = _rows(x)
        (NT, D), dev, nm = x.shape, x.device, len(plan.modules)
        strategy = gemm_strategy(ops.PRECISION['matmul'], D, _ld(x), nm, all(params[4 * m].is_contiguous() for m in range(nm)))
        dstate, x16 = None, None
        if drop is not None and (drop[0] > 0 or drop[1] > 0):
            x = x.contiguous()
            dstate, x16 = _drop_prep(x, plan, drop, strategy)
        xin = [dstate.xc[cv] for cv in plan.mod_conv] if dstate is not None else [x] * nm
        P, g16 = _project(xin, x16, plan, params, strategy, dev)
        fold = plan.take_fold()
        small, lay = fold or plan.scratch(dev)
        out = torch.empty(NT, D, device=dev, dtype=torch.float32)
        arg = torch.empty(NT, D, device=dev, dtype=torch.uint8)
# ... 33 lines not shown
```

### sessionrec-pytorch_amd/ops.py

```python
import ctypes as _ct
import os
from collections import namedtuple

import torch

from ._lib import CONST, STRUCTS, lib, ptr, ptr_array, stream
from .stepq import StepQueue

HgDesc = STRUCTS['srec_hg_desc']
GemmGroup = STRUCTS['srec_gemm_group']
GemmGroup16 = STRUCTS['srec_gemm16_group']
GemmF32Group = STRUCTS['srec_gemm_f32_group']
GruStepDesc = STRUCTS['srec_gru_step_desc']
GruFusedDesc = STRUCTS['srec_gru_fused_desc']
GruFusedBwdDesc = STRUCTS['srec_gru_fused_bwd_desc']
HeadDesc = STRUCTS['srec_head_desc']
HeadBwdDesc = STRUCTS['srec_head_bwd_desc']
StepPrepDesc = STRUCTS['srec_step_prep_desc']
G16_MAXP, GEMM32_MAXP, GRU_MAXP = CONST['SREC_G16_MAXP'], CONST['SREC_GEMM32_MAXP'], CONST['SREC_GRU_MAXP']
HEAD_MAXH, HEAD_MAXW = CONST['SREC_HEAD_MAXH'], CONST['SREC_HEAD_MAXW']


def _rows(t):
    assert t.dim() == 2 and t.dtype == torch.float32, (t.shape, t.dtype)
# ... 310 lines not shown
    return LinearCat.apply(weight, bias, dyn, exact, *xs)


class CatCols(torch.autograd.Function):

    @staticmethod
    def forward(ctx, a, b):
        a, b = _rows(a), _rows(b)
        n, da, db = a.shape[0], a.shape[1], b.shape[1]
        out = torch.empty(n, da + db, device=a.device, dtype=torch.float32)
        lib.srec_cat_cols(ptr(a), _ld(a), da, ptr(b), _ld(b), db, n, ptr(out), stream())
        ctx.da = da
        return out

    @staticmethod
    def backward(ctx, g):
        return g[:, :ctx.da], g[:, ctx.da:]


def cat_cols(a, b):
    return CatCols.apply(a, b)


RNG_COUNTER = {}


_NONCE = {'seed': None, 'gen': None}


def seed_dropout(seed=None):
    base = torch.initial_seed()
    _NONCE['seed'] = base
    _NONCE['gen'] = torch.Generator().manual_seed(base if seed is None else int(seed))


def _nonce():
    if _NONCE['gen'] is None or _NONCE['seed'] != torch.initial_seed():
        seed_dropout()
    return int(torch.randint(0, 0x7fffffff, (1,), generator=_NONCE['gen']).item())


def rng_args(device):
    c = RNG_COUNTER.get(str(device))
    dev = torch.device(device)
    if c is None and dev.type == 'cuda' and torch.cuda.is_current_stream_capturing():
        raise RuntimeError('dropout inside a captured step needs a device-side step counter: construct FusedAdam(..., '
                           'model=model) before capturing (a frozen nonce alone would replay the same mask every step)')
    return _nonce(), (c.data_ptr() if c is not None else None)


class TableGrad:

    def __init__(self, weight, defer=False):
        self.buf = torch.zeros_like(weight)
        self.fresh = False
        self.defer = defer
        self.pending = None
        self.radial = torch.zeros(weight.shape[0], device=weight.device, dtype=torch.float32) if defer else None
        self.radial_dirty = False

    def overwritten(self):
        self.pending = None
        if self.radial is not None and self.radial_dirty:
            self.radial.zero_()
        self.radial_dirty = False

    def reset(self):
        self.fresh = False
        self.overwritten()

    def materialize(self):
        if self.pending is not None:
            table, cs, inv_scale = self.pending
            lib.srec_rownorm_project_radial(ptr(table), table.stride(0), ptr(cs), float(inv_scale), ptr(self.buf),
                                            self.buf.stride(0), table.shape[0], table.shape[1], ptr(self.radial), stream())
            self.pending = None
            self.radial_dirty = False
        return self.buf


class EmbeddingLookup(torch.autograd.Function):

    @staticmethod
    def forward(ctx, table, idx, uniq, tgrad, dyn_n, dyn_u, drop=None):
        n = idx.numel()
        d = table.shape[1]
        out = torch.empty(n, d, device=table.device, dtype=torch.float32)
        ctx.drop = None
        if drop is not None and drop[0] > 0:
            seed, cnt = rng_args(table.device)
            ctx.drop = (float(drop[0]), seed, cnt, int(drop[1]))
            lib.srec_gather_rows_drop(ptr(table), table.stride(0), ptr(idx), ptr(out), d, n, ptr(dyn_n), d, ctx.drop[0],
                                      seed, cnt, ctx.drop[3], stream())
        else:
            lib.srec_gather_rows(ptr(table), table.stride(0), ptr(idx), ptr(out), d, n, ptr(dyn_n), d, stream())
        ctx.uniq, ctx.tgrad, ctx.dyn_u, ctx.shape = uniq, tgrad, dyn_u, tuple(table.shape)
        return out

    @staticmethod
    def backward(ctx, g):
        items, uptr, upos = ctx.uniq[:3]
        tg = ctx.tgrad
        g = _rows(g)
        V, d = ctx.shape
        if ctx.drop is not None:
            g = g.contiguous()
            pdrop, seed, cnt, salt = ctx.drop

            def first_level(gp, ldg, it, pt, ps, dst, ldd, ucap, dyn, acc):
                lib.srec_scatter_add_sorted_drop(gp, ldg, it, pt, ps, dst, ldd, ucap, dyn, d, acc, pdrop, seed, cnt, salt, stream())
        else:
            def first_level(gp, ldg, it, pt, ps, dst, ldd, ucap, dyn, acc):
                lib.srec_scatter_add_sorted(gp, ldg, it, pt, ps, dst, ldd, ucap, dyn, d, acc, stream())
        radial = ptable = None
        if tg is not None and tg.pending is not None:
            radial, ptable = tg.radial, tg.pending[0]
            tg.radial_dirty = True
        if tg is not None:
            dst, acc, ret = tg.buf, 1, None
        else:
            dst = torch.zeros(V, d, device=g.device, dtype=torch.float32)
            acc, ret = 0, dst
        if len(ctx.uniq) == 5:
            cptr, chunk_ptr = ctx.uniq[3], ctx.uniq[4]
            C = chunk_ptr.numel() - 1
            part = torch.empty(max(C, 1), d, device=g.device, dtype=torch.float32)
            ar = _arange(C + 1, g.device)
            first_level(ptr(g), _ld(g), ptr(ar), ptr(chunk_ptr), ptr(upos), ptr(part), d, C, None, 0)
            if radial is not None:
                lib.srec_scatter_add_sorted_ex(ptr(part), d, ptr(items), ptr(cptr), ptr(ar), ptr(dst), dst.stride(0),
                                               items.numel(), ptr(ctx.dyn_u), d, acc, 0.0, 0, None, 0, ptr(ptable),
                                               ptable.stride(0), ptr(radial), stream())
            else:
                lib.srec_scatter_add_sorted(ptr(part), d, ptr(items), ptr(cptr), ptr(ar), ptr(dst), dst.stride(0),
                                            items.numel(), ptr(ctx.dyn_u), d, acc, stream())
        elif radial is not None:
            pdrop, seed, cnt, salt = ctx.drop if ctx.drop is not None else (0.0, 0, None, 0)
            lib.srec_scatter_add_sorted_ex(ptr(g), _ld(g), ptr(items), ptr(uptr), ptr(upos), ptr(dst), dst.stride(0),
                                           items.numel(), ptr(ctx.dyn_u), d, acc, pdrop, seed, cnt, salt, ptr(ptable),
                                           ptable.stride(0), ptr(radial), stream())
        else:
            first_level(ptr(g), _ld(g), ptr(items), ptr(uptr), ptr(upos), ptr(dst), dst.stride(0), items.numel(),
                        ptr(ctx.dyn_u), acc)
        return ret, None, None, None, None, None, None


def embedding_lookup(table, idx, uniq, tgrad=None, dyn_n=None, dyn_u=None, drop=None):
    return EmbeddingLookup.apply(table, idx, uniq, tgrad, dyn_n, dyn_u, drop)


class RowGather(torch.autograd.Function):

    @staticmethod
    def forward(ctx, x, idx, dyn, ascending=False):
        x = _rows(x)
        n, d = idx.numel(), x.shape[1]
        out = torch.empty(n, d, device=x.device, dtype=torch.float32)
        lib.srec_gather_rows(ptr(x), _ld(x), ptr(idx), ptr(out), d, n, ptr(dyn), d, stream())
        ctx.save_for_backward(idx)
        ctx.nrows, ctx.dyn, ctx.ascending = x.shape[0], dyn, ascending
        return out

    @staticmethod
    def backward(ctx, g):
        (idx,) = ctx.saved_tensors
        g = _rows(g)
        n, d = g.shape
        if ctx.ascending and d % 4 == 0:
            gx = torch.empty(ctx.nrows, d, device=g.device, dtype=torch.float32)
            lib.srec_expand_rows_sorted(ptr(g), _ld(g), ptr(idx), n, ptr(ctx.dyn), ctx.nrows, d, ptr(gx), d, stream())
            return gx, None, None, None
        gx = torch.zeros(ctx.nrows, d, device=g.device, dtype=torch.float32)
        ar = _arange(n + 1, g.device)
        lib.srec_scatter_add_sorted(ptr(g), _ld(g), ptr(idx), ptr(ar), ptr(ar), ptr(gx), d, n, ptr(ctx.dyn), d, 0,
                                    stream())
        return gx, None, None, None


_ARANGE = {}


def _arange(n, device):
    key = (str(device),)
    t = _ARANGE.get(key)
    if t is None or t.numel() < n:
        t = torch.arange(max(n, 4096), device=device, dtype=torch.int32)
        _ARANGE[key] = t
    return t


def row_gather(x, idx, dyn=None, ascending=False):
    return RowGather.apply(x, idx, dyn, ascending)


class PermuteAndPick(torch.autograd.Function):

    @staticmethod
    def forward(ctx, x, perm, inv, dyn_n, dyn_b, *picks):
        x = _rows(x)
        d = x.shape[1]
        outs = []
        for k, (idx, dyn) in enumerate([(perm, dyn_n)] + [(p, dyn_b) for p in picks]):
            if k == 0:
                o = torch.empty(idx.numel(), d, device=x.device, dtype=torch.float32)
            else:
                o = torch.empty(idx.numel(), 2 * d, device=x.device, dtype=torch.float32)[:, :d]
            lib.srec_gather_rows(ptr(x), _ld(x), ptr(idx), ptr(o), _ld(o), idx.numel(), ptr(dyn), d, stream())
            outs.append(o)
        ctx.save_for_backward(inv, *picks)
        ctx.nrows, ctx.dyn_b = x.shape[0], dyn_b
        return tuple(outs)

    @staticmethod
    def backward(ctx, g_perm, *g_picks):
        inv, *picks = ctx.saved_tensors
        g_perm = _rows(g_perm)
        d = g_perm.shape[1]
        gx = torch.empty(ctx.nrows, d, device=g_perm.device, dtype=torch.float32)
        lib.srec_gather_rows(ptr(g_perm), _ld(g_perm), ptr(inv), ptr(gx), d, ctx.nrows, None, d, stream())
        for idx, g in zip(picks, g_picks):
            if g is None:
                continue
            g = _rows(g)
            ar = _arange(idx.numel() + 1, g.device)
            lib.srec_scatter_add_sorted(ptr(g), _ld(g), ptr(idx), ptr(ar), ptr(ar), ptr(gx), d, idx.numel(),
                                        ptr(ctx.dyn_b), d, 1, stream())
        return (gx, None, None, None, None) + (None,) * len(picks)


def permute_and_pick(x, perm, inv, picks, dyn_n=None, dyn_b=None):
    outs = PermuteAndPick.apply(x, perm, inv, dyn_n, dyn_b, *picks)
# ... 1117 lines not shown
```

### sessionrec-pytorch_amd/optim.py

```python
import ctypes as _ct

import torch

from ._lib import STRUCTS, lib, ptr, ptr_array, stream

_AdamMultiDesc = STRUCTS['srec_adam_multi_desc']


class FusedAdam(torch.optim.Optimizer):
    def __init__(self, params, lr=1e-3, betas=(0.9, 0.999), eps=1e-8, weight_decay=0, model=None, fuse_projection=False):
        defaults = dict(lr=lr, betas=betas, eps=eps, weight_decay=weight_decay)
        super().__init__(params, defaults)
        self.model = model
        if fuse_projection and model is not None and hasattr(model, '_cosine') and model._cosine() is not None \
                and model._table().is_cuda:
            model._defer_projection = True
            shard = getattr(model, 'shard', None)
            if shard is None:
                model.__dict__.pop('_srec_state', None)
            elif getattr(shard.local, 'fused_dropout', False):
                tg = shard.tgrad
                tg.defer = True
                if tg.radial is None:
                    tg.radial = torch.zeros(tg.buf.shape[0], device=tg.buf.device, dtype=torch.float32)
        self._hyper = {}
        self._frozen = None

    def folds_table_prep(self):
        m = self.model
        if m is None or not getattr(m, '_fold_table_prep', False) or not hasattr(m, '_table'):
            return False
        W = m._table()
        return bool(W.is_cuda and W.dim() == 2 and (W.shape[1] & 3) == 0 and W.shape[1] <= 1024 and W.is_contiguous()
                    and any(p is W for g in self.param_groups for p in g['params']))

    def zero_grad(self, set_to_none=True):
        super().zero_grad(set_to_none=set_to_none)
        st = self.model.__dict__.get('_srec_state') if self.model is not None else None
        if st is not None and st.get('tgrad') is not None:
            st['tgrad'].reset()

    def _table_info(self):
        model = self.model
        table, tgrad, st = None, None, None
        if model is not None and hasattr(model, '_table'):
            table = model._table()
            st = model.__dict__.get('_srec_state')
            if st is not None and st.get('tgrad') is not None and st['tgrad'].fresh:
                tgrad = st['tgrad']
        return table, tgrad, st

    grad_override = None

    def _grad_of(self, p, table, tgrad, zero_ids):
        g = p.grad
        if self.grad_override and id(p) in self.grad_override:
            g = self.grad_override[id(p)]
        if table is not None and p is table and tgrad is not None:
            if g is not None:
                tgrad.materialize()
            g = tgrad.buf if g is None else g.add_(tgrad.buf)
        if g is None and id(p) in zero_ids:
            cache = self.__dict__.setdefault('_zero_grads', {})
            g = cache.get(id(p))
            if g is None or g.shape != p.shape or g.device != p.device:
                g = cache[id(p)] = torch.zeros_like(p)
        return g

    def _buffers(self, gi, off, device):
        key = (gi, off)
        if key not in self._hyper:
            from . import ops
            self._hyper[key] = dict(counter=torch.zeros(1, dtype=torch.int32, device=device),
                                    cfg=torch.zeros(5, dtype=torch.float64, device=device),
                                    hyper=torch.zeros(8, dtype=torch.float32, device=device), cfg_host=None,
                                    fresh=True)
            if key == (0, 0):
                if self.model is not None:
                    self.model.__dict__['_srec_rng_counter'] = self._hyper[key]['counter']
                ops.RNG_COUNTER[str(device)] = self._hyper[key]['counter']
        return self._hyper[key]

    def _cfg(self, group):
        b1, b2 = group['betas']
        return (float(group['lr']), float(b1), float(b2), float(group['eps']), float(group['weight_decay']))

    def _vals(self, group, step):
        b1, b2 = group['betas']
        return [group['lr'] / (1.0 - b1 ** step), b1, b2, group['eps'], group['weight_decay'], 1.0 - b1, 1.0 - b2,
                (1.0 - b2 ** step) ** 0.5]

    def reset_steps(self):
        self._T = 0
        for st in self.state.values():
            if 'step' in st:
                st['step'] = 0
        for ent in self._hyper.values():
            if isinstance(ent, dict):
                ent['counter'].zero_()
                ent['fresh'] = False

    def snapshot(self):
        return dict(T=getattr(self, '_T', 0),
                    state={p: (st['step'], st['exp_avg'].clone(), st['exp_avg_sq'].clone())
                           for p, st in self.state.items() if 'exp_avg' in st})

    def restore(self, snap):
        self._T = snap['T']
        with torch.no_grad():
            for p, st in self.state.items():
                if 'exp_avg' not in st:
                    continue
                if p in snap['state']:
                    st['step'] = snap['state'][p][0]
                    st['exp_avg'].copy_(snap['state'][p][1])
                    st['exp_avg_sq'].copy_(snap['state'][p][2])
                else:
                    st['step'] = 0
                    st['exp_avg'].zero_()
                    st['exp_avg_sq'].zero_()
            for key, ent in self._hyper.items():
                ent['counter'].fill_(max(self._T - key[1], 0))
                ent['fresh'] = False

    def load_state_dict(self, state_dict):
        super().load_state_dict(state_dict)
        steps = [int(st['step']) for st in self.state.values() if 'step' in st]
        for st in self.state.values():
            if 'step' in st:
                st['step'] = int(st['step'])
        self._T = max(steps) if steps else 0
        self._hyper = {}
        self._frozen = None

    def _work(self):
        from . import ops
        ops.STEP.finish()
        table, tgrad, _ = self._table_info()
        zero_ids = {}
        if self.model is not None and hasattr(self.model, 'zero_grad_params'):
            zero_ids = {id(p): p for p in self.model.zero_grad_params()}
        work = []
        for gi, group in enumerate(self.param_groups):
            items = []
            for p in group['params']:
                g = self._grad_of(p, table, tgrad, zero_ids)
                if g is None:
                    continue
                state = self.state[p]
                if len(state) == 0:
                    state['step'] = 0
                    state['exp_avg'] = torch.zeros_like(p, memory_format=torch.contiguous_format)
                    state['exp_avg_sq'] = torch.zeros_like(p, memory_format=torch.contiguous_format)
                items.append((p, g, state))
            work.append((gi, group, items))
        return work

    def advance(self, work=None):
        if work is None:
            work = self._frozen
        self._T = getattr(self, '_T', 0) + 1
        for gi, group, items in work:
            offs = set()
            for p, g, state in items:
                state['step'] += 1
                offs.add(self._T - state['step'])
            cfg = self._cfg(group)
            for off in offs:
                ent = self._buffers(gi, off, items[0][0].device)
                if ent['fresh']:
                    ent['counter'].fill_(self._T - off - 1)
                    ent['fresh'] = False
                if ent['cfg_host'] != cfg:
                    ent['cfg'].copy_(torch.tensor(cfg, dtype=torch.float64))
                    ent['cfg_host'] = cfg
        return work

    def _hyper_args(self, ents, tap, skip):
        n = len(ents)
        cs, cf, hy = (ptr_array([e[k] for e in ents]) for k in ('counter', 'cfg', 'hyper'))
        first = self._hyper.get((0, 0)) if isinstance(self._hyper, dict) else None
        if tap is not None and first is not None and any(e is first for e in ents):
            tapped = (ptr(first['counter']), ptr(tap[0]), ptr(tap[1]), tap[1].numel())
        else:
            tapped = (None, None, None, 0)
        return (n, _ct.addressof(cs), _ct.addressof(cf), _ct.addressof(hy)) + tapped + (ptr(skip),), (cs, cf, hy, tap, skip)

    def hyper_rider(self, tap=None, skip=None):
        from . import ops
        ops.STEP.rider_result()
        keys = sorted(getattr(self, '_used_keys', ()) or ())
        if not keys or len(keys) > 16 or not isinstance(getattr(self, '_hyper', None), dict):
            return False
        ents = [self._hyper.get(k) for k in keys]
        if any(ent is None or ent.get('cfg_host') is None for ent in ents):
            return False
        args, keep = self._hyper_args(ents, tap, skip)
        ops.STEP.offer_rider(args, keys, keep)
        return True

    def launch(self, work, tap=None, skip=None):
        from . import ops as _ops
        done = _ops.STEP.rider_result()
        table, tgrad, st = self._table_info()
        model = self.model
        T = getattr(self, '_T', 0)
        ents, used = [], set()
        for gi, group, items in work:
            for off in sorted({T - state['step'] for _, _, state in items}):
                ent = self._buffers(gi, off, items[0][0].device)
                if ent['cfg_host'] is None:
                    ent['cfg'].copy_(torch.tensor(self._cfg(group), dtype=torch.float64))
                    ent['cfg_host'] = self._cfg(group)
                ents.append(ent)
                used.add((gi, off))
        self._used_keys = used
        if done is not None and done != frozenset(used):
            raise RuntimeError('the step scalars were advanced for other slots than this step uses (hyper_rider): %r vs %r'
                               % (sorted(done), sorted(used)))
        for i in range(0, len(ents) if done is None else 0, 16):
            args, keep = self._hyper_args(ents[i:i + 16], tap, skip)
            lib.srec_adam_hyper_multi(*args, stream())
        merged = {}
        for gi, group, items in work:
            if not items:
                continue
            use_wd = 1 if group['weight_decay'] != 0 else 0
            slot_of = {}
            for _, _, state in items:
                slot_of.setdefault(state['step'], T - state['step'])
            multi = {}
            for p, g, state in items:
                hyper = self._buffers(gi, slot_of[state['step']], p.device)['hyper']
                g = g.contiguous()
                is_table = table is not None and p is table
                if not is_table and p.is_contiguous() and p.numel() < (1 << 22):
                    multi.setdefault(slot_of[state['step']], []).append((p, g, state))
                    continue
                if is_table and p.dim() == 2 and (p.shape[1] & 3) == 0:
                    cos = model._cosine() if hasattr(model, '_cosine') else None
                    cs_out, cs_scale, eps_mode = None, 1.0, 0
                    if cos is not None and st is not None and st.get('cs') is not None:
                        cs_out, cs_scale, eps_mode = st['cs'], float(cos[0]), int(cos[1])
                    mn_model = float(getattr(model, '_max_norm', 0.0) or 0.0)
                    mn = mn_model if cs_out is not None else 0.0
                    fold = st is not None and self.folds_table_prep()
                    tb = model._table_copy(st, p) if (fold and hasattr(model, '_table_copy')) else None
                    renorm_write = 1 if (fold and mn_model > 0) else 0
                    if renorm_write:
                        mn = mn_model
                    d16, dp16 = (tb.E16, tb.E16.shape[1]) if tb is not None else (None, 0)
                    shard = getattr(model, 'shard', None)
                    n_rows = shard.n_live if (shard is not None and 0 < shard.n_live < p.shape[0]) else p.shape[0]
                    pend = tgrad.pending if (tgrad is not None and g.data_ptr() == tgrad.buf.data_ptr()) else None
                    if pend is not None:
                        lib.srec_adam_rows_proj(ptr(p), ptr(g), ptr(state['exp_avg']), ptr(state['exp_avg_sq']), n_rows,
                                                p.shape[1], p.stride(0), ptr(hyper), use_wd, mn, renorm_write, ptr(cs_out), cs_scale,
                                                eps_mode, 1e-12, ptr(pend[1]), float(pend[2]), ptr(tgrad.radial), ptr(d16), dp16,
                                                stream())
                        tgrad.pending = None
                        tgrad.radial_dirty = False
                    else:
                        if tgrad is not None:
                            tgrad.materialize()
                        lib.srec_adam_rows(ptr(p), ptr(g), ptr(state['exp_avg']), ptr(state['exp_avg_sq']), n_rows,
                                           p.shape[1], p.stride(0), ptr(hyper), use_wd, mn, renorm_write, ptr(cs_out), cs_scale,
                                           eps_mode, 1e-12, ptr(d16), dp16, stream())
                    if fold:
                        st['table_prepared'] = (bool(renorm_write) or mn_model <= 0, tb is not None, p._version)
                    if cs_out is not None:
                        st['cs_fresh'] = True
                else:
                    self._join_grads()
                    lib.srec_adam_flat(ptr(p), ptr(g), ptr(state['exp_avg']), ptr(state['exp_avg_sq']), p.numel(),
                                       ptr(hyper), use_wd, stream())
            for slot, rows in multi.items():
                b1, b2 = group['betas']
                key = (float(group['lr']), float(b1), float(b2), float(group['eps']), slot, str(rows[0][0].device))
                wd = float(group['weight_decay'])
                ent = merged.get(key)
                if ent is not None and wd != 0 and ent[1] != 0 and ent[1] != wd:
                    key = key + (wd,)
                    ent = merged.get(key)
                if ent is None:
                    ent = merged[key] = [gi, wd, []]
                elif wd != 0 and ent[1] == 0:
                    ent[0], ent[1] = gi, wd
                ent[2] += [(p, g, st_, use_wd) for p, g, st_ in rows]
        self._join_grads()
        for key, (gi, _, rows) in merged.items():
            slot = key[4]
            nt = len(rows)
            keep = [(_ct.c_int * nt)(*[r[3] for r in rows]), (_ct.c_long * nt)(*[r[0].numel() for r in rows]),
                    ptr_array([r[0] for r in rows]), ptr_array([r[1] for r in rows]),
                    ptr_array([r[2]['exp_avg'] for r in rows]), ptr_array([r[2]['exp_avg_sq'] for r in rows])]
            desc = _AdamMultiDesc(nt, *[_ct.addressof(a) for a in keep])
            hyper = self._buffers(gi, slot, rows[0][0].device)['hyper']
            lib.srec_adam_multi(_ct.addressof(desc), ptr(hyper), stream())
        if tgrad is not None:
            tgrad.fresh = False
        from . import ops
        ops.weights_changed()

    grad_join = None

    def _join_grads(self):
        j, self.grad_join = self.grad_join, None
        if j is not None:
            j()

    @torch.no_grad()
    def step(self, closure=None):
        work = self._work()
        self.advance(work)
        self.launch(work)
        return None
```

### sessionrec-pytorch_amd/srgnn.py

```python
import math

import torch
import torch.nn as nn
import torch.nn.functional as F

from . import ops


class _ScoringMixin:

    def _table(self):
        return self.embedding.weight

    def _cosine(self):
        return None

    def _state(self, B):
        dev = self._table().device
        st = self.__dict__.setdefault('_srec_state', {})
        if st.get('dev') != dev:
            st.clear()
            st['dev'] = dev
            st['tgrad'] = ops.TableGrad(self._table(), defer=bool(getattr(self, '_defer_projection', False)))
            st['ws'] = {}
# ... 3 lines not shown
            V, d = self._table().shape
            st['ws'][B] = ops.CEWorkspace(B, V, d, dev)
        return st

    @property
    def table_grad(self):
        tg = self._state(1)['tgrad']
        tg.materialize()
        return tg

    def _col_scale(self, st):
        cos = self._cosine()
        if cos is None:
            return None, 1.0
        scale, eps_mode = cos
        W = self._table()
        if st['cs'] is None:
            st['cs'] = torch.empty(W.shape[0], device=W.device, dtype=torch.float32)
        if not st['cs_fresh']:
            from ._lib import lib, ptr, stream
            lib.srec_row_invnorm(ptr(W), W.stride(0), W.shape[0], W.shape[1], eps_mode, 1e-12, float(scale),
                                 ptr(st['cs']), stream())
        st['cs_fresh'] = False
        return st['cs'], 1.0 / float(scale)

    def _prepare_table(self):
        self._table_ready = False

    _fold_table_prep = True

    def _table_copy(self, st, W):
        if not ops.use_bf16_scoring(W.shape[1]) or not W.is_cuda:
            return None
        if self.shard is not None:
            local, n_live = self.shard.local, self.shard.n_live
            if not hasattr(local, '_tb') or n_live <= 0:
                return None
            live = W[:n_live] if n_live < W.shape[0] else W
            tb = local._tb(live, False)
            local._tb_written = ((live.data_ptr(), tuple(live.shape)), W._version)
            return tb
        if st.get('tb16') is None:
            st['tb16'] = ops.TableBF16(W)
        return st['tb16']

    def _take_prepared(self, st, mark=True):
        prep = st.pop('table_prepared', None) if st is not None else None
        if prep is None or prep[2] != self._table()._version:
            return False, False
        if mark and prep[1] and self.shard is None:
            self._tb16_fresh = self._table()._version
        return prep[0], prep[1] and self.shard is None

    def _pop_tb16_fresh(self):
        v = self.__dict__.pop('_tb16_fresh', None)
        return v is not None and v is not False and v == self._table()._version

    def table_written(self):
        self.__dict__.pop('_tb16_fresh', None)
        self.__dict__.pop('_table_ready', None)
        st = self.__dict__.get('_srec_state')
        if st is not None:
            st.pop('table_prepared', None)
            st['cs_fresh'] = False

    shard = None
    graph_capable = False

    def _lookup(self, idx, uniq, tgrad, dyn_n=None, dyn_u=None, drop=None, inv=None):
        p = drop.p if isinstance(drop, nn.Dropout) and drop.training else 0.0
        ops.flush_intake()
        W = self._table()
        c = self.__dict__.get('_srec_rng_counter')
        if c is not None and c.device == W.device:
            ops.RNG_COUNTER[str(W.device)] = c
        else:
            ops.RNG_COUNTER.pop(str(W.device), None)
        if self.shard is not None:
            fused = p > 0 and getattr(self.shard.local, 'fused_dropout', False)
            rows = self.shard.lookup(self._table(), idx, uniq, (p, 7) if fused else None, inv=inv)
            return rows if (fused or drop is None) else drop(rows)
        if drop is not None and not isinstance(drop, nn.Dropout):
            return drop(ops.embedding_lookup(self._table(), idx, uniq, tgrad, dyn_n, dyn_u))
        return ops.embedding_lookup(self._table(), idx, uniq, tgrad, dyn_n, dyn_u, (p, 7) if p > 0 else None)

    def fused_loss(self, *inputs_and_labels, dynB=None):
        *inputs, labels = inputs_and_labels
        B = labels.numel()
        if dynB is None and hasattr(inputs[0], 'dynp'):
            dynB = inputs[0].dynp('B')
        st = self._state(B)
        self._prepare_table()
        cs, inv_scale = self._col_scale(st)
        if self.shard is not None:
            self.shard.labels_hint = labels
        self._sr_ws = st['ws'][B] if (self.shard is None and ops.use_bf16_scoring(self._table().shape[1])) else None
        defer = ops.STEP.may_defer or (self.training and self._table().is_cuda and getattr(self, 'defer_slab_sums', True))
        try:
            with ops.STEP.deferring(defer):
                sr = self.session_repr(*inputs, tgrad=st['tgrad'])
        finally:
            self._sr_ws = None
        if self.shard is not None:
            return self.shard.loss(sr, self._table(), cs, labels, inv_scale)
        loss, _ = ops.score_ce(sr, self._table(), cs, labels.to(torch.int32), st['ws'][B], st['tgrad'], dynB, inv_scale,
                               self._table_bf16(st))
        return loss

    def _table_bf16(self, st):
        W = self._table()
        if not ops.use_bf16_scoring(W.shape[1]):
            return None
        if st.get('tb16') is None:
            st['tb16'] = ops.TableBF16(W)
        if self._pop_tb16_fresh():
            return st['tb16']
        if self._take_prepared(st, mark=False)[1]:
            return st['tb16']
        return st['tb16'].refresh(W)

    def topk(self, *inputs, k=20):
        with torch.no_grad():
            sr = self.session_repr(*inputs)
            mixed = isinstance(sr, (list, tuple)) or getattr(self, 'extra', False)
            if mixed:
                v, i = self(*inputs).topk(k)
                return v, i.to(torch.int32)
            st = self._state(sr.shape[0])
            cs, _ = self._col_scale(st)
            if self.shard is not None:
                return self.shard.topk(sr, self._table(), cs, k, data_parallel=self.shard.eval_data_parallel)
            return ops.score_topk(sr, self._table(), cs, k)

    def target_rank(self, *inputs, labels):
        with torch.no_grad():
            sr = self.session_repr(*inputs)
            cs, _ = self._col_scale(self._state(sr.shape[0]))
            return self._rank_of([sr], cs, labels, None, None, None)

    def _rank_of(self, srs, cs, labels, off_ex, off_in, listed):
        if self.shard is not None:
            return self.shard.target_rank(srs, self._table(), cs, labels, off_ex, off_in, listed,
                                          data_parallel=self.shard.eval_data_parallel)
        rank = ops.score_rank(srs, self._table(), cs, labels, off_ex, off_in, listed)[0]
        if listed is not None:
            rank = torch.where(labels >= 0, rank.clamp(min=0), rank)
        return rank

    def recommend(self, *inputs, k=20, exclude_seen=False):
        was_training = self.training
        self.eval()
        try:
            with torch.no_grad():
                return self._recommend(*inputs, k=k, exclude_seen=exclude_seen)
        finally:
            self.train(was_training)

    def _recommend(self, *inputs, k, exclude_seen):
        sr = self.session_repr(*inputs)
        st = self._state(sr.shape[0])
        cs, inv_scale = self._col_scale(st)
        off_ex = -self._lse(sr, cs, inv_scale, st).unsqueeze(0)
        listed = self._session_items(inputs[0]) if exclude_seen else None
        return self._select_of([sr], cs, k, off_ex, None, listed, exclude_seen)

    def _lse(self, sr, cs, inv_scale, st, labels=None):
        B = sr.shape[0]
# ... 139 lines not shown
```

### sessionrec-pytorch_amd/stepq.py

```python
import contextlib

import torch


class StepQueue:

    def __init__(self, launch_slab_sums, launch_intake):
        self._launch_slab_sums, self._launch_intake = launch_slab_sums, launch_intake
        self._on, self._depth = False, 0
        self._sums, self._intake = [], []
        self._rider, self._done = None, None

    @property
    def may_defer(self):
        return self._on

    @contextlib.contextmanager
    def deferring(self, on):
        prev = self._on
        if not self._depth:
            self.drop_stale()
        self._depth += 1
        self._on = bool(on)
        try:
            yield
        finally:
            self._depth -= 1
            self._on = prev

    def defer_slab_sum(self, part, out, ok=True, tall=False):
        if ok and not self._sums:
            try:
                torch.autograd.Variable._execution_engine.queue_callback(self.finish)
            except RuntimeError:
                ok = False
        if not ok:
            self._launch_slab_sums([(part, out, tall)])
            return
        self._sums.append((part, out.detach(), tall))

    def waiting(self):
        return len(self._sums)

    def drop_stale(self):
        self._sums = []

    def flush(self):
        if self._sums:
            tasks, self._sums = self._sums, []
            self._launch_slab_sums(tasks, None)

    def finish(self):
        if self._sums:
            tasks, self._sums = self._sums, []
            rider, self._rider = self._rider, None
            self._launch_slab_sums(tasks, rider[0] if rider is not None else None)
            if rider is not None:
                self._done = rider[1]

    def offer_rider(self, args, slots, keepalive=None):
        self._rider, self._done = (args, frozenset(slots), keepalive), None

    def rider_result(self):
        done, self._rider, self._done = self._done, None, None
        return done

    def offer_intake(self, entries):
        self._intake = list(entries)

    def intake_pending(self):
        return bool(self._intake)

    def flush_intake(self):
        while self._intake:
            self._launch_intake(*self._intake.pop(0)[:6])

    def take_intake(self):
        box = self._intake.pop() if self._intake else None
        self.flush_intake()
        return box

    def abort(self):
        self._sums, self._intake, self._rider, self._done = [], [], None, None
```

Measured before the change: 675,600 sessions/s.

## Split item-table Adam pass so untouched rows update early during backward

```diff
diff --git a/include/srec.h b/include/srec.h
--- a/include/srec.h
+++ b/include/srec.h
@@ -48,6 +48,9 @@
                             int ld_dst, int u_cap, const int* dyn, int d, int accumulate, void* stream);
 int srec_gather_rows_drop(const float* src, int ld_src, const int* idx, float* out, int ld_out, int n_cap, const int* dyn,
                           int d, float p, int seed, const int* counter, int salt, void* stream);
+int srec_gather_rows_stamp(const float* src, int ld_src, const int* idx, float* out, int ld_out, int n_cap, const int* dyn,
+                           int d, float p, int seed, const int* counter, int salt, const int* items, int u_cap,
+                           const int* dyn_u, int* stamp, const int* stamp_counter, int n_rows, void* stream);
 int srec_scatter_add_sorted_drop(const float* g, int ld_g, const int* items, const int* ptr, const int* pos, float* dst,
                                  int ld_dst, int u_cap, const int* dyn, int d, int accumulate, float p, int seed,
                                  const int* counter, int salt, void* stream);
@@ -190,6 +193,11 @@
                         float max_norm, int renorm_write, float* cs_out, float cs_scale, int eps_mode, float cs_eps,
                         const float* proj_cs, float proj_inv_scale, float* radial, void* dst16, int Dp, void* stream);
 
+int srec_adam_rows_early(const void* tp_ptrs, const int* tp_ints, const float* tp_flts, int row0, int row1, int n_role,
+                         void* stream);
+int srec_adam_rows_late(const void* tp_ptrs, const int* tp_ints, const float* tp_flts, void* stream);
+int srec_adam_hyper_eval(const int* counter, const void* cfg, const int* skip, float* out, void* stream);
+
 int srec_hg_ws_floats(const void* desc, long* n_floats);
 int srec_hg_fwd(const void* desc, const float* x, int ld_x, float* out, int ld_out, unsigned char* arg, void* stream);
 int srec_hg_fold(const void* desc, void* stream);
@@ -203,6 +211,9 @@
 int srec_hg_pre_merge(const void* desc, const float* g, int ld_g, const float* t, int S, float* dx, int ld_dx, void* stream);
 int srec_hg_bwd(const void* desc, const float* x, int ld_x, const float* g, int ld_g, const unsigned char* arg, float* dx,
                 int ld_dx, float* ws, void* stream);
+int srec_hg_bwd_carry(const void* desc, const float* x, int ld_x, const float* g, int ld_g, const unsigned char* arg, float* dx,
+                      int ld_dx, float* ws, const void* tp_ptrs, const int* tp_ints, const float* tp_flts, int rows_dst, int n_role,
+                      void* stream);
 
 int srec_gemm_group_bf16(const void* desc, int mode, void* stream);
 
diff --git a/include/srec_hg.h b/include/srec_hg.h
--- a/include/srec_hg.h
+++ b/include/srec_hg.h
@@ -234,4 +234,32 @@
     int* box_err;
 } srec_step_prep_desc;
 
+#define SREC_TP_W 0
+#define SREC_TP_G 1
+#define SREC_TP_M 2
+#define SREC_TP_V 3
+#define SREC_TP_HYPER 4
+#define SREC_TP_CS_OUT 5
+#define SREC_TP_PROJ_CS 6
+#define SREC_TP_RADIAL 7
+#define SREC_TP_DST16 8
+#define SREC_TP_STAMP 9
+#define SREC_TP_COUNTER 10
+#define SREC_TP_CFG 11
+#define SREC_TP_SKIP 12
+#define SREC_TP_NPTR 13
+#define SREC_TP_N 0
+#define SREC_TP_D 1
+#define SREC_TP_LD 2
+#define SREC_TP_USE_WD 3
+#define SREC_TP_RENORM_WRITE 4
+#define SREC_TP_EPS_MODE 5
+#define SREC_TP_DP 6
+#define SREC_TP_NINT 7
+#define SREC_TP_MAX_NORM 0
+#define SREC_TP_CS_SCALE 1
+#define SREC_TP_CS_EPS 2
+#define SREC_TP_PROJ_INV_SCALE 3
+#define SREC_TP_NFLT 4
+
 #endif
diff --git a/sessionrec-pytorch_amd/csrc/adam.hip b/sessionrec-pytorch_amd/csrc/adam.hip
--- a/sessionrec-pytorch_amd/csrc/adam.hip
+++ b/sessionrec-pytorch_amd/csrc/adam.hip
@@ -1,23 +1,8 @@
 #include "common.h"
-#include "hyper_role.h"
+#include "adam_rows_role.h"
+#include "../../include/srec_hg.h"
 
 namespace {
-
-struct Hyper { float step, b1, b2, eps, wd, omb1, omb2, bc2s; };
-
-__device__ __forceinline__ Hyper load_hyper(const float* __restrict__ h) {
-    Hyper r{h[0], h[1], h[2], h[3], h[4], h[5], h[6], h[7]};
-    return r;
-}
-
-__device__ __forceinline__ float adam1(float& p, float g, float& m, float& v, const Hyper& h, float wd,
-                                       float step, float bc2s) {
-    g += wd * p;
-    m = m + h.omb1 * (g - m);
-    v = h.b2 * v + h.omb2 * g * g;
-    p -= step * (m / (sqrtf(v) / bc2s + h.eps));
-    return p;
-}
 
 __global__ void adam_flat_kernel(float* __restrict__ p, const float* __restrict__ g, float* __restrict__ m,
                                  float* __restrict__ v, size_t n, const float* __restrict__ hyper, int use_wd) {
@@ -43,119 +28,41 @@
     }
 }
 
-template <bool HOLD>
-__global__ void adam_rows_kernel(float* __restrict__ W, const float* __restrict__ G, float* __restrict__ M,
-                                 float* __restrict__ Vv, int n, int d, int ld, const float* __restrict__ hyper,
-                                 int use_wd, float max_norm, int renorm_write, float* __restrict__ cs_out, float cs_scale,
-                                 int eps_mode, float cs_eps, const float* __restrict__ proj_cs, float proj_inv_scale,
-                                 float* __restrict__ radial, unsigned short* __restrict__ dst16, int Dp) {
+__global__ void adam_rows_kernel(AdamRowsArgs a) {
     const int i = blockIdx.x * 4 + (threadIdx.x >> 6), lane = threadIdx.x & 63;
-    if (i >= n) return;
-    const Hyper h = load_hyper(hyper);
-    const float wd = use_wd ? h.wd : 0.f, step = h.step, rs2 = h.bc2s;
-    if (h.step == 0.f && h.omb1 == 0.f && h.omb2 == 0.f && h.b2 == 1.f) renorm_write = 0;
-    const size_t off = (size_t)i * ld;
-    float pcoef = 0.f;
-    float4 pw[4], gw[4];
-    if (HOLD) {
+    if (i >= a.n || !adam_rows_wanted(a, i)) return;
+    adam_rows_row<true>(a, i, lane, load_hyper(a.hyper));
+}
+
+__global__ __launch_bounds__(256) void adam_rows_early_kernel(AdamRowsArgs a) {
+    __shared__ float role_h[8];
+    adam_rows_role<true>(a, (int)blockIdx.x, role_h);
+}
+
+__global__ __launch_bounds__(256) void adam_rows_stream_kernel(AdamRowsArgs a) {
+    __shared__ float role_h[8];
+    const bool early = a.cfg != nullptr;
+    if (early) {
+        if (threadIdx.x == 0) {
+            float h8[8];
+            hyper_eval(*a.counter + 1, a.cfg, a.skip != nullptr && *a.skip != 0, h8);
 #pragma unroll
-        for (int j = 0; j < 4; ++j) {
-            const int c = lane * 4 + j * 256;
-            pw[j] = make_float4(0.f, 0.f, 0.f, 0.f); gw[j] = pw[j];
-            if (c < d) { pw[j] = *reinterpret_cast<const float4*>(W + off + c); gw[j] = *reinterpret_cast<const float4*>(G + off + c); }
-        }
-    }
-    if (proj_cs != nullptr) {
-        float dot = 0.f;
-        if (HOLD) {
-#pragma unroll
-            for (int j = 0; j < 4; ++j) dot += pw[j].x * gw[j].x + pw[j].y * gw[j].y + pw[j].z * gw[j].z + pw[j].w * gw[j].w;
-        } else {
-            for (int c = lane * 4; c < d; c += 256) {
-                const float4 pp = *reinterpret_cast<const float4*>(W + off + c);
-                const float4 gg = *reinterpret_cast<const float4*>(G + off + c);
-                dot += pp.x * gg.x + pp.y * gg.y + pp.z * gg.z + pp.w * gg.w;
-            }
-        }
-        dot = wave_sum(dot);
-        const float iv = proj_cs[i] * proj_inv_scale;
-        if (radial != nullptr) {
-            dot -= radial[i];
-            if (lane == 0) radial[i] = 0.f;
-        }
-        pcoef = dot * iv * iv;
-    }
-    float ss = 0.f;
-    if (HOLD) {
-#pragma unroll
-        for (int j = 0; j < 4; ++j) {
-            const int c = lane * 4 + j * 256;
-            if (c < d) {
-                float4 pp = pw[j], gg = gw[j];
-                gg.x -= pp.x * pcoef; gg.y -= pp.y * pcoef; gg.z -= pp.z * pcoef; gg.w -= pp.w * pcoef;
-                float4 mm = *reinterpret_cast<float4*>(M + off + c);
-                float4 vv = *reinterpret_cast<float4*>(Vv + off + c);
-                adam1(pp.x, gg.x, mm.x, vv.x, h, wd, step, rs2);
-                adam1(pp.y, gg.y, mm.y, vv.y, h, wd, step, rs2);
-                adam1(pp.z, gg.z, mm.z, vv.z, h, wd, step, rs2);
-                adam1(pp.w, gg.w, mm.w, vv.w, h, wd, step, rs2);
-                ss += pp.x * pp.x + pp.y * pp.y + pp.z * pp.z + pp.w * pp.w;
-                pw[j] = pp;
-                *reinterpret_cast<float4*>(M + off + c) = mm;
-                *reinterpret_cast<float4*>(Vv + off + c) = vv;
-            }
-        }
-        float nrm = 0.f;
-        float sc = 1.f;
-        if (max_norm > 0.f || cs_out != nullptr) {
-            nrm = sqrtf(wave_sum(ss));
-            if (max_norm > 0.f && nrm > max_norm) {
-                const float s1 = max_norm / (nrm + 1e-7f);
-                if (renorm_write) sc = s1;
-                nrm *= s1;
-            }
-        }
-#pragma unroll
-        for (int j = 0; j < 4; ++j) {
-            const int c = lane * 4 + j * 256;
-            float4 pp = pw[j];
-            if (sc != 1.f) { pp.x *= sc; pp.y *= sc; pp.z *= sc; pp.w *= sc; }
-            if (c < d) *reinterpret_cast<float4*>(W + off + c) = pp;
-            if (dst16 != nullptr && c < Dp)
-                *reinterpret_cast<uint2*>(dst16 + (size_t)i * Dp + c) = make_uint2(srec_pack_bf16(pp.x, pp.y), srec_pack_bf16(pp.z, pp.w));
-        }
-        if (cs_out != nullptr && lane == 0)
-            cs_out[i] = cs_scale * (eps_mode == 0 ? 1.f / fmaxf(nrm, cs_eps) : 1.f / (nrm + cs_eps));
-        return;
-    }
-    for (int c = lane * 4; c < d; c += 256) {
-        float4 pp = *reinterpret_cast<float4*>(W + off + c);
-        float4 gg = *reinterpret_cast<const float4*>(G + off + c);
-        gg.x -= pp.x * pcoef; gg.y -= pp.y * pcoef; gg.z -= pp.z * pcoef; gg.w -= pp.w * pcoef;
-        float4 mm = *reinterpret_cast<float4*>(M + off + c);
-        float4 vv = *reinterpret_cast<float4*>(Vv + off + c);
-        adam1(pp.x, gg.x, mm.x, vv.x, h, wd, step, rs2);
-        adam1(pp.y, gg.y, mm.y, vv.y, h, wd, step, rs2);
-        adam1(pp.z, gg.z, mm.z, vv.z, h, wd, step, rs2);
-        adam1(pp.w, gg.w, mm.w, vv.w, h, wd, step, rs2);
-        ss += pp.x * pp.x + pp.y * pp.y + pp.z * pp.z + pp.w * pp.w;
-        *reinterpret_cast<float4*>(W + off + c) = pp;
-        *reinterpret_cast<float4*>(M + off + c) = mm;
-        *reinterpret_cast<float4*>(Vv + off + c) = vv;
-    }
-    if (max_norm <= 0.f && cs_out == nullptr) return;
-    float nrm = sqrtf(wave_sum(ss));
-    if (max_norm > 0.f && nrm > max_norm) {
-        const float sc = max_norm / (nrm + 1e-7f);
-        for (int c = lane * 4; renorm_write && c < d; c += 256) {
-            float4 pp = *reinterpret_cast<float4*>(W + off + c);
-            pp.x *= sc; pp.y *= sc; pp.z *= sc; pp.w *= sc;
-            *reinterpret_cast<float4*>(W + off + c) = pp;
-        }
-        nrm *= sc;
-    }
-    if (cs_out != nullptr && lane == 0)
-        cs_out[i] = cs_scale * (eps_mode == 0 ? 1.f / fmaxf(nrm, cs_eps) : 1.f / (nrm + cs_eps));
+            for (int k = 0; k < 8; ++k) role_h[k] = h8[k];
+        }
+        __syncthreads();
+    }
+    const Hyper h = load_hyper(early ? role_h : a.hyper);
+    const int lane = threadIdx.x & 63;
+    for (int i = a.row0 + (int)blockIdx.x * 4 + (int)(threadIdx.x >> 6); i < a.row1; i += a.n_role * 4)
+        if (adam_rows_wanted(a, i)) adam_rows_row<false>(a, i, lane, h);
+}
+
+__global__ void adam_hyper_eval_kernel(const int* __restrict__ counter, const double* __restrict__ cfg, const int* __restrict__ skip,
+                                       float* __restrict__ out) {
+    if (threadIdx.x != 0 || blockIdx.x != 0) return;
+    float h[8];
+    hyper_eval(*counter + 1, cfg, skip != nullptr && *skip != 0, h);
+    for (int k = 0; k < 8; ++k) out[k] = h[k];
 }
 
 constexpr int MT = 88;
@@ -286,20 +193,88 @@
     return 0;
 }
 
+static int adam_rows_fill(float* W, const float* G, float* M, float* V, int n, int d, int ld, const float* hyper, int use_wd,
+                          float max_norm, int renorm_write, float* cs_out, float cs_scale, int eps_mode, float cs_eps,
+                          const float* proj_cs, float proj_inv_scale, float* radial, void* dst16, int Dp, AdamRowsArgs& a) {
+    a = AdamRowsArgs{};
+    if (d <= 0 || (d & 3) || (ld & 3) || n < 0) return SREC_BAD_ARG;
+    if (dst16 != nullptr && (d > 1024 || Dp < d || (Dp & 3) || Dp > 1024)) return SREC_BAD_ARG;
+    a.W = W; a.G = G; a.M = M; a.Vv = V; a.n = n; a.d = d; a.ld = ld; a.hyper = hyper; a.use_wd = use_wd; a.max_norm = max_norm;
+    a.renorm_write = renorm_write; a.cs_out = cs_out; a.cs_scale = cs_scale; a.eps_mode = eps_mode; a.cs_eps = cs_eps;
+    a.proj_cs = proj_cs; a.proj_inv_scale = proj_inv_scale; a.radial = radial;
+    a.dst16 = d <= 1024 ? (unsigned short*)dst16 : nullptr; a.Dp = d <= 1024 ? Dp : 0;
+    return 0;
+}
+
+static int adam_rows_launch(const AdamRowsArgs& a, void* stream) {
+    if (a.n <= 0) return 0;
+    if (a.d <= 1024) hipLaunchKernelGGL(adam_rows_kernel, dim3(cdiv(a.n, 4)), dim3(256), 0, (hipStream_t)stream, a);
+    else {
+        AdamRowsArgs s = a;
+        s.row0 = 0; s.row1 = a.n; s.n_role = cdiv(a.n, 4); s.cfg = nullptr;
+        hipLaunchKernelGGL(adam_rows_stream_kernel, dim3(s.n_role), dim3(256), 0, (hipStream_t)stream, s);
+    }
+    SREC_LAUNCH_CHECK();
+    return 0;
+}
+
 static int adam_rows_run(float* W, const float* G, float* M, float* V, int n, int d, int ld, const float* hyper, int use_wd,
                          float max_norm, int renorm_write, float* cs_out, float cs_scale, int eps_mode, float cs_eps,
                          const float* proj_cs, float proj_inv_scale, float* radial, void* dst16, int Dp, void* stream) {
     if (n <= 0) return 0;
-    if (d <= 0 || (d & 3) || (ld & 3)) return SREC_BAD_ARG;
-    if (dst16 != nullptr && (d > 1024 || Dp < d || (Dp & 3) || Dp > 1024)) return SREC_BAD_ARG;
-    if (d <= 1024)
-        hipLaunchKernelGGL(adam_rows_kernel<true>, dim3(cdiv(n, 4)), dim3(256), 0, (hipStream_t)stream, W, G, M, V, n, d, ld, hyper,
-                           use_wd, max_norm, renorm_write, cs_out, cs_scale, eps_mode, cs_eps, proj_cs, proj_inv_scale, radial,
-                           (unsigned short*)dst16, Dp);
-    else
-        hipLaunchKernelGGL(adam_rows_kernel<false>, dim3(cdiv(n, 4)), dim3(256), 0, (hipStream_t)stream, W, G, M, V, n, d, ld, hyper,
-                           use_wd, max_norm, renorm_write, cs_out, cs_scale, eps_mode, cs_eps, proj_cs, proj_inv_scale, radial,
-                           (unsigned short*)nullptr, 0);
+    AdamRowsArgs a;
+    if (int rc = adam_rows_fill(W, G, M, V, n, d, ld, hyper, use_wd, max_norm, renorm_write, cs_out, cs_scale, eps_mode, cs_eps, proj_cs,
+                                proj_inv_scale, radial, dst16, Dp, a)) return rc;
+    return adam_rows_launch(a, stream);
+}
+
+int srec_table_pass_args(const void* ptrs_, const int* ints, const float* flts, int early, int row0, int row1, int n_role,
+                         AdamRowsArgs& a) {
+    void* const* q = (void* const*)ptrs_;
+    if (q == nullptr || ints == nullptr || flts == nullptr) return SREC_BAD_ARG;
+    if (q[SREC_TP_STAMP] == nullptr || q[SREC_TP_COUNTER] == nullptr) return SREC_BAD_ARG;
+    if (q[SREC_TP_PROJ_CS] == nullptr && q[SREC_TP_RADIAL] != nullptr) return SREC_BAD_ARG;
+    if (int rc = adam_rows_fill((float*)q[SREC_TP_W], (const float*)q[SREC_TP_G], (float*)q[SREC_TP_M], (float*)q[SREC_TP_V],
+                                ints[SREC_TP_N], ints[SREC_TP_D], ints[SREC_TP_LD], (const float*)q[SREC_TP_HYPER], ints[SREC_TP_USE_WD],
+                                flts[SREC_TP_MAX_NORM], ints[SREC_TP_RENORM_WRITE], (float*)q[SREC_TP_CS_OUT], flts[SREC_TP_CS_SCALE],
+                                ints[SREC_TP_EPS_MODE], flts[SREC_TP_CS_EPS], (const float*)q[SREC_TP_PROJ_CS],
+                                flts[SREC_TP_PROJ_INV_SCALE], (float*)q[SREC_TP_RADIAL], q[SREC_TP_DST16], ints[SREC_TP_DP], a)) return rc;
+    if (a.W == nullptr || a.G == nullptr || a.M == nullptr || a.Vv == nullptr) return SREC_BAD_ARG;
+    a.stamp = (const int*)q[SREC_TP_STAMP]; a.counter = (const int*)q[SREC_TP_COUNTER];
+    if (early) {
+        if (q[SREC_TP_CFG] == nullptr || row0 < 0 || row1 > a.n || row0 > row1 || n_role <= 0) return SREC_BAD_ARG;
+        a.bias = 1; a.want = 0; a.cfg = (const double*)q[SREC_TP_CFG]; a.skip = (const int*)q[SREC_TP_SKIP]; a.hyper = nullptr;
+        a.row0 = row0; a.row1 = row1;
+        const int need = cdiv(row1 - row0, 4);
+        a.n_role = n_role < need ? n_role : need;
+        if (a.n_role < 1) a.n_role = 1;
+    } else {
+        if (a.hyper == nullptr) return SREC_BAD_ARG;
+        a.bias = 0; a.want = 1;
+    }
+    return 0;
+}
+
+extern "C" int srec_adam_rows_early(const void* tp_ptrs, const int* tp_ints, const float* tp_flts, int row0, int row1, int n_role,
+                                    void* stream) {
+    AdamRowsArgs a;
+    if (int rc = srec_table_pass_args(tp_ptrs, tp_ints, tp_flts, 1, row0, row1, n_role, a)) return rc;
+    if (row1 <= row0) return 0;
+    if (a.d <= 1024) hipLaunchKernelGGL(adam_rows_early_kernel, dim3(a.n_role), dim3(256), 0, (hipStream_t)stream, a);
+    else hipLaunchKernelGGL(adam_rows_stream_kernel, dim3(a.n_role), dim3(256), 0, (hipStream_t)stream, a);
+    SREC_LAUNCH_CHECK();
+    return 0;
+}
+
+extern "C" int srec_adam_rows_late(const void* tp_ptrs, const int* tp_ints, const float* tp_flts, void* stream) {
+    AdamRowsArgs a;
+    if (int rc = srec_table_pass_args(tp_ptrs, tp_ints, tp_flts, 0, 0, 0, 0, a)) return rc;
+    return adam_rows_launch(a, stream);
+}
+
+extern "C" int srec_adam_hyper_eval(const int* counter, const void* cfg, const int* skip, float* out, void* stream) {
+    if (counter == nullptr || cfg == nullptr || out == nullptr) return SREC_BAD_ARG;
+    hipLaunchKernelGGL(adam_hyper_eval_kernel, dim3(1), dim3(64), 0, (hipStream_t)stream, counter, (const double*)cfg, skip, out);
     SREC_LAUNCH_CHECK();
     return 0;
 }
diff --git a/sessionrec-pytorch_amd/csrc/adam_rows_role.h b/sessionrec-pytorch_amd/csrc/adam_rows_role.h
--- /dev/null
+++ b/sessionrec-pytorch_amd/csrc/adam_rows_role.h
@@ -0,0 +1,173 @@
+#pragma once
+#include "common.h"
+#include "hyper_role.h"
+#include "../../include/srec_hg.h"
+
+struct AdamRowsArgs {
+    float* W; const float* G; float* M; float* Vv;
+    int n, d, ld;
+    const float* hyper;
+    int use_wd; float max_norm; int renorm_write;
+    float* cs_out; float cs_scale; int eps_mode; float cs_eps;
+    const float* proj_cs; float proj_inv_scale; float* radial;
+    unsigned short* dst16; int Dp;
+    const int* stamp; const int* counter; int bias, want;
+    const double* cfg; const int* skip;
+    int row0, row1, n_role;
+};
+
+int srec_table_pass_args(const void* ptrs, const int* ints, const float* flts, int early, int row0, int row1, int n_role,
+                         AdamRowsArgs& a);
+
+namespace {
+
+struct Hyper { float step, b1, b2, eps, wd, omb1, omb2, bc2s; };
+
+__device__ __forceinline__ Hyper load_hyper(const float* __restrict__ h) {
+    Hyper r{h[0], h[1], h[2], h[3], h[4], h[5], h[6], h[7]};
+    return r;
+}
+
+__device__ __forceinline__ float adam1(float& p, float g, float& m, float& v, const Hyper& h, float wd,
+                                       float step, float bc2s) {
+    g += wd * p;
+    m = m + h.omb1 * (g - m);
+    v = h.b2 * v + h.omb2 * g * g;
+    p -= step * (m / (sqrtf(v) / bc2s + h.eps));
+    return p;
+}
+
+__device__ __forceinline__ bool adam_rows_wanted(const AdamRowsArgs& a, const int i) {
+    return a.stamp == nullptr || (a.stamp[i] == *a.counter + a.bias) == (a.want != 0);
+}
+
+template <bool HOLD, int NJ = 4>
+__device__ __forceinline__ void adam_rows_row(const AdamRowsArgs& a, const int i, const int lane, const Hyper& h) {
+    float* __restrict__ W = a.W; const float* __restrict__ G = a.G; float* __restrict__ M = a.M; float* __restrict__ Vv = a.Vv;
+    const int d = a.d, ld = a.ld, eps_mode = a.eps_mode, Dp = a.Dp;
+    int renorm_write = a.renorm_write;
+    const float max_norm = a.max_norm, cs_scale = a.cs_scale, cs_eps = a.cs_eps, proj_inv_scale = a.proj_inv_scale;
+    float* __restrict__ cs_out = a.cs_out; const float* __restrict__ proj_cs = a.proj_cs; float* __restrict__ radial = a.radial;
+    unsigned short* __restrict__ dst16 = a.dst16;
+    const float wd = a.use_wd ? h.wd : 0.f, step = h.step, rs2 = h.bc2s;
+    if (h.step == 0.f && h.omb1 == 0.f && h.omb2 == 0.f && h.b2 == 1.f) renorm_write = 0;
+    const size_t off = (size_t)i * ld;
+    float pcoef = 0.f;
+    float4 pw[NJ], gw[NJ];
+    if (HOLD) {
+#pragma unroll
+        for (int j = 0; j < NJ; ++j) {
+            const int c = lane * 4 + j * 256;
+            pw[j] = make_float4(0.f, 0.f, 0.f, 0.f); gw[j] = pw[j];
+            if (c < d) { pw[j] = *reinterpret_cast<const float4*>(W + off + c); gw[j] = *reinterpret_cast<const float4*>(G + off + c); }
+        }
+    }
+    if (proj_cs != nullptr) {
+        float dot = 0.f;
+        if (HOLD) {
+#pragma unroll
+            for (int j = 0; j < NJ; ++j) dot += pw[j].x * gw[j].x + pw[j].y * gw[j].y + pw[j].z * gw[j].z + pw[j].w * gw[j].w;
+        } else {
+            for (int c = lane * 4; c < d; c += 256) {
+                const float4 pp = *reinterpret_cast<const float4*>(W + off + c);
+                const float4 gg = *reinterpret_cast<const float4*>(G + off + c);
+                dot += pp.x * gg.x + pp.y * gg.y + pp.z * gg.z + pp.w * gg.w;
+            }
+        }
+        dot = wave_sum(dot);
+        const float iv = proj_cs[i] * proj_inv_scale;
+        if (radial != nullptr) {
+            dot -= radial[i];
+            if (lane == 0) radial[i] = 0.f;
+        }
+        pcoef = dot * iv * iv;
+    }
+    float ss = 0.f;
+    if (HOLD) {
+#pragma unroll
+        for (int j = 0; j < NJ; ++j) {
+            const int c = lane * 4 + j * 256;
+            if (c < d) {
+                float4 pp = pw[j], gg = gw[j];
+                gg.x -= pp.x * pcoef; gg.y -= pp.y * pcoef; gg.z -= pp.z * pcoef; gg.w -= pp.w * pcoef;
+                float4 mm = *reinterpret_cast<float4*>(M + off + c);
+                float4 vv = *reinterpret_cast<float4*>(Vv + off + c);
+                adam1(pp.x, gg.x, mm.x, vv.x, h, wd, step, rs2);
+                adam1(pp.y, gg.y, mm.y, vv.y, h, wd, step, rs2);
+                adam1(pp.z, gg.z, mm.z, vv.z, h, wd, step, rs2);
+                adam1(pp.w, gg.w, mm.w, vv.w, h, wd, step, rs2);
+                ss += pp.x * pp.x + pp.y * pp.y + pp.z * pp.z + pp.w * pp.w;
+                pw[j] = pp;
+                *reinterpret_cast<float4*>(M + off + c) = mm;
+                *reinterpret_cast<float4*>(Vv + off + c) = vv;
+            }
+        }
+        float nrm = 0.f;
+        float sc = 1.f;
+        if (max_norm > 0.f || cs_out != nullptr) {
+            nrm = sqrtf(wave_sum(ss));
+            if (max_norm > 0.f && nrm > max_norm) {
+                const float s1 = max_norm / (nrm + 1e-7f);
+                if (renorm_write) sc = s1;
+                nrm *= s1;
+            }
+        }
+#pragma unroll
+        for (int j = 0; j < NJ; ++j) {
+            const int c = lane * 4 + j * 256;
+            float4 pp = pw[j];
+            if (sc != 1.f) { pp.x *= sc; pp.y *= sc; pp.z *= sc; pp.w *= sc; }
+            if (c < d) *reinterpret_cast<float4*>(W + off + c) = pp;
+            if (dst16 != nullptr && c < Dp)
+                *reinterpret_cast<uint2*>(dst16 + (size_t)i * Dp + c) = make_uint2(srec_pack_bf16(pp.x, pp.y), srec_pack_bf16(pp.z, pp.w));
+        }
+        if (cs_out != nullptr && lane == 0)
+            cs_out[i] = cs_scale * (eps_mode == 0 ? 1.f / fmaxf(nrm, cs_eps) : 1.f / (nrm + cs_eps));
+        return;
+    }
+    for (int c = lane * 4; c < d; c += 256) {
+        float4 pp = *reinterpret_cast<float4*>(W + off + c);
+        float4 gg = *reinterpret_cast<const float4*>(G + off + c);
+        gg.x -= pp.x * pcoef; gg.y -= pp.y * pcoef; gg.z -= pp.z * pcoef; gg.w -= pp.w * pcoef;
+        float4 mm = *reinterpret_cast<float4*>(M + off + c);
+        float4 vv = *reinterpret_cast<float4*>(Vv + off + c);
+        adam1(pp.x, gg.x, mm.x, vv.x, h, wd, step, rs2);
+        adam1(pp.y, gg.y, mm.y, vv.y, h, wd, step, rs2);
+        adam1(pp.z, gg.z, mm.z, vv.z, h, wd, step, rs2);
+        adam1(pp.w, gg.w, mm.w, vv.w, h, wd, step, rs2);
+        ss += pp.x * pp.x + pp.y * pp.y + pp.z * pp.z + pp.w * pp.w;
+        *reinterpret_cast<float4*>(W + off + c) = pp;
+        *reinterpret_cast<float4*>(M + off + c) = mm;
+        *reinterpret_cast<float4*>(Vv + off + c) = vv;
+    }
+    if (max_norm <= 0.f && cs_out == nullptr) return;
+    float nrm = sqrtf(wave_sum(ss));
+    if (max_norm > 0.f && nrm > max_norm) {
+        const float sc = max_norm / (nrm + 1e-7f);
+        for (int c = lane * 4; renorm_write && c < d; c += 256) {
+            float4 pp = *reinterpret_cast<float4*>(W + off + c);
+            pp.x *= sc; pp.y *= sc; pp.z *= sc; pp.w *= sc;
+            *reinterpret_cast<float4*>(W + off + c) = pp;
+        }
+        nrm *= sc;
+    }
+    if (cs_out != nullptr && lane == 0)
+        cs_out[i] = cs_scale * (eps_mode == 0 ? 1.f / fmaxf(nrm, cs_eps) : 1.f / (nrm + cs_eps));
+}
+
+template <bool HOLD, int NJ = 4>
+__device__ __forceinline__ void adam_rows_role(const AdamRowsArgs& a, const int wg, float* role_h ) {
+    if (threadIdx.x == 0) {
+        float h8[8];
+        hyper_eval(*a.counter + 1, a.cfg, a.skip != nullptr && *a.skip != 0, h8);
+#pragma unroll
+        for (int k = 0; k < 8; ++k) role_h[k] = h8[k];
+    }
+    __syncthreads();
+    const Hyper h = load_hyper(role_h);
+    const int lane = threadIdx.x & 63;
+    for (int i = a.row0 + wg * 4 + (int)(threadIdx.x >> 6); i < a.row1; i += a.n_role * 4)
+        if (adam_rows_wanted(a, i)) adam_rows_row<HOLD, NJ>(a, i, lane, h);
+}
+
+}
diff --git a/sessionrec-pytorch_amd/csrc/hgat.hip b/sessionrec-pytorch_amd/csrc/hgat.hip
--- a/sessionrec-pytorch_amd/csrc/hgat.hip
+++ b/sessionrec-pytorch_amd/csrc/hgat.hip
@@ -1,7 +1,10 @@
 #include "common.h"
+#include "adam_rows_role.h"
 #include "../../include/srec_hg.h"
 
 extern "C" int srec_hg_fold(const void* desc, void* stream);
+extern "C" int srec_adam_rows_early(const void* tp_ptrs, const int* tp_ints, const float* tp_flts, int row0, int row1, int n_role,
+                                    void* stream);
 
 namespace {
 
@@ -777,13 +780,18 @@
     return t;
 }
 
-template <typename T, int DIF, int WV>
-__global__ __launch_bounds__(256, WV) void hg_bwd_dst_node_kernel(DstArgs a) {
+template <typename T, int DIF, int WV, bool ROLE = false>
+__global__ __launch_bounds__(256, WV) void hg_bwd_dst_node_kernel(DstArgs a, AdamRowsArgs r) {
     __shared__ float da[WPB][MAXDEG][MAXH];
     __shared__ int su[WPB][MAXDEG];
+    int bx = (int)blockIdx.x;
+    if (ROLE) {
+        if (bx < r.n_role) { adam_rows_role<true, 1>(r, bx, &da[0][0][0]); return; }
+        bx -= r.n_role;
+    }
     const int w = __builtin_amdgcn_readfirstlane(threadIdx.x >> 6), lane = threadIdx.x & 63;
     HGT_BEGIN();
-    const int row = blockIdx.x * WPB + w;
+    const int row = bx * WPB + w;
     if (row >= a.row0_t[a.nt]) return;
     const int t = find_range(a.row0_t, a.nt, row);
     const int v = row - a.row0_t[t];
@@ -987,9 +995,10 @@
 };
 
 constexpr int WPB_SRC = 4;
-template <typename T, int WV, bool DER_FIRST>
-__global__ __launch_bounds__(64 * WPB_SRC, WV) void hg_bwd_src_kernel(SrcArgs a) {
+template <typename T, int WV, bool DER_FIRST, bool ROLE = false>
+__global__ __launch_bounds__(64 * WPB_SRC, WV) void hg_bwd_src_kernel(SrcArgs a, AdamRowsArgs r) {
     extern __shared__ __attribute__((aligned(16))) float alr[];
+    if (ROLE && (int)blockIdx.x < r.n_role) { adam_rows_role<true, 1>(r, (int)blockIdx.x, alr); return; }
     HGT_BEGIN();
     const int b = find_range(a.start, a.nb, (int)blockIdx.x);
     const int lane = threadIdx.x & 63;
@@ -1497,11 +1506,21 @@
     return 0;
 }
 
-extern "C" int srec_hg_bwd(const void* desc_, const float* x, int ld_x, const float* g, int ld_g, const unsigned char* arg,
-                           float* dx, int ld_dx, float* ws, void* stream) {
+namespace {
+struct Carry { const void* ptrs; const int* ints; const float* flts; int rows_dst, n_role; };
+
+int hg_bwd_run(const void* desc_, const float* x, int ld_x, const float* g, int ld_g, const unsigned char* arg,
+               float* dx, int ld_dx, float* ws, const Carry* cy, void* stream) {
     const srec_hg_desc* d = (const srec_hg_desc*)desc_;
     if (bad_desc(d) || (ld_g & 3) || (ld_dx & 3) || (ld_x & 3) || ws == nullptr) return SREC_BAD_ARG;
     hipStream_t st = (hipStream_t)stream;
+    int carry_n = 0, carry_from = 0;
+    if (cy != nullptr) {
+        AdamRowsArgs probe;
+        if (int rc = srec_table_pass_args(cy->ptrs, cy->ints, cy->flts, 1, 0, 0, cy->n_role, probe)) return rc;
+        if (probe.d > 256 || probe.Dp > 256 || cy->rows_dst < 0 || cy->rows_dst > probe.n) return SREC_BAD_ARG;
+        carry_n = probe.n;
+    }
     const int H = d->H, D = d->D, HD = H * D;
     const size_t esz = (d->p16 & SREC_HG_P16_BF16) ? 2 : 4;
     int ninst_t[MAXT] = {0, 0, 0, 0};
@@ -1544,8 +1563,14 @@
             node = node && al16(a.A[i]) && al16(a.Mk[i]) && al16(a.eLs[i]) && al16(a.eRd[i]) && al16(a.DP[i]) && al16(a.der[i]);
         }
         if (node && trows > 0) {
-            if (d->p16 & SREC_HG_P16_BF16) hipLaunchKernelGGL((hg_bwd_dst_node_kernel<unsigned short, 2, 4>), dim3(cdiv(trows, WPB)), dim3(256), 0, st, a);
-            else hipLaunchKernelGGL((hg_bwd_dst_node_kernel<float, 1, 3>), dim3(cdiv(trows, WPB)), dim3(256), 0, st, a);
+            AdamRowsArgs r{};
+            if (cy != nullptr && cy->rows_dst > 0) {
+                if (int rc = srec_table_pass_args(cy->ptrs, cy->ints, cy->flts, 1, 0, cy->rows_dst, cy->n_role, r)) return rc;
+                carry_from = cy->rows_dst;
+                if (d->p16 & SREC_HG_P16_BF16) hipLaunchKernelGGL((hg_bwd_dst_node_kernel<unsigned short, 2, 4, true>), dim3(r.n_role + cdiv(trows, WPB)), dim3(256), 0, st, a, r);
+                else hipLaunchKernelGGL((hg_bwd_dst_node_kernel<float, 1, 3, true>), dim3(r.n_role + cdiv(trows, WPB)), dim3(256), 0, st, a, r);
+            } else if (d->p16 & SREC_HG_P16_BF16) hipLaunchKernelGGL((hg_bwd_dst_node_kernel<unsigned short, 2, 4>), dim3(cdiv(trows, WPB)), dim3(256), 0, st, a, r);
+            else hipLaunchKernelGGL((hg_bwd_dst_node_kernel<float, 1, 3>), dim3(cdiv(trows, WPB)), dim3(256), 0, st, a, r);
         } else if (blocks > 0) {
             if (d->p16 & SREC_HG_P16_BF16) hipLaunchKernelGGL(hg_bwd_dst_kernel<unsigned short>, dim3(blocks), dim3(256), 0, st, a);
             else hipLaunchKernelGGL(hg_bwd_dst_kernel<float>, dim3(blocks), dim3(256), 0, st, a);
@@ -1577,10 +1602,19 @@
         }
         if (blocks > 0) {
             const size_t lds = (size_t)2 * HD * sizeof(float);
-            if (d->p16 & SREC_HG_P16_BF16) hipLaunchKernelGGL((hg_bwd_src_kernel<unsigned short, 6, false>), dim3(blocks), dim3(64 * WPB_SRC), lds, st, a);
-            else hipLaunchKernelGGL((hg_bwd_src_kernel<float, 4, false>), dim3(blocks), dim3(64 * WPB_SRC), lds, st, a);
-        }
-    }
+            AdamRowsArgs r{};
+            if (carry_from < carry_n) {
+                if (int rc = srec_table_pass_args(cy->ptrs, cy->ints, cy->flts, 1, carry_from, carry_n, cy->n_role, r)) return rc;
+                carry_from = carry_n;
+                for (int b = 0; b <= d->n_blocks; ++b) a.start[b] += r.n_role;
+                if (d->p16 & SREC_HG_P16_BF16) hipLaunchKernelGGL((hg_bwd_src_kernel<unsigned short, 6, false, true>), dim3(r.n_role + blocks), dim3(64 * WPB_SRC), lds, st, a, r);
+                else hipLaunchKernelGGL((hg_bwd_src_kernel<float, 4, false, true>), dim3(r.n_role + blocks), dim3(64 * WPB_SRC), lds, st, a, r);
+            } else if (d->p16 & SREC_HG_P16_BF16) hipLaunchKernelGGL((hg_bwd_src_kernel<unsigned short, 6, false>), dim3(blocks), dim3(64 * WPB_SRC), lds, st, a, r);
+            else hipLaunchKernelGGL((hg_bwd_src_kernel<float, 4, false>), dim3(blocks), dim3(64 * WPB_SRC), lds, st, a, r);
+        }
+    }
+    if (carry_from < carry_n)
+        if (int rc = srec_adam_rows_early(cy->ptrs, cy->ints, cy->flts, carry_from, carry_n, cy->n_role, stream)) return rc;
     {
         ColArgs a{};
         a.nt = d->n_types; a.nm = d->n_mods; a.H = H; a.D = D; a.g = g; a.ld_g = ld_g; a.arg = arg; a.part = ws;
@@ -1634,6 +1668,19 @@
     }
     SREC_LAUNCH_CHECK();
     return 0;
+}
+}
+
+extern "C" int srec_hg_bwd(const void* desc_, const float* x, int ld_x, const float* g, int ld_g, const unsigned char* arg,
+                           float* dx, int ld_dx, float* ws, void* stream) {
+    return hg_bwd_run(desc_, x, ld_x, g, ld_g, arg, dx, ld_dx, ws, nullptr, stream);
+}
+
+extern "C" int srec_hg_bwd_carry(const void* desc_, const float* x, int ld_x, const float* g, int ld_g, const unsigned char* arg,
+                                 float* dx, int ld_dx, float* ws, const void* tp_ptrs, const int* tp_ints, const float* tp_flts,
+                                 int rows_dst, int n_role, void* stream) {
+    const Carry cy{tp_ptrs, tp_ints, tp_flts, rows_dst, n_role};
+    return hg_bwd_run(desc_, x, ld_x, g, ld_g, arg, dx, ld_dx, ws, &cy, stream);
 }
 
 namespace {
diff --git a/sessionrec-pytorch_amd/csrc/hyper_role.h b/sessionrec-pytorch_amd/csrc/hyper_role.h
--- a/sessionrec-pytorch_amd/csrc/hyper_role.h
+++ b/sessionrec-pytorch_amd/csrc/hyper_role.h
@@ -9,24 +9,30 @@
     const int* skip;
 };
 
+__device__ __forceinline__ void hyper_eval(const int t, const double* __restrict__ cfg, const bool skip, float (&h)[8]) {
+    const double lr = cfg[0], b1 = cfg[1], b2 = cfg[2], eps = cfg[3], wd = cfg[4];
+    if (skip) {
+        h[0] = 0.f; h[1] = 1.f; h[2] = 1.f; h[3] = (float)eps; h[4] = 0.f; h[5] = 0.f; h[6] = 0.f;
+        h[7] = 1.f;
+        return;
+    }
+    h[0] = (float)(lr / (1.0 - pow(b1, (double)t)));
+    h[1] = (float)b1; h[2] = (float)b2; h[3] = (float)eps; h[4] = (float)wd;
+    h[5] = (float)(1.0 - b1); h[6] = (float)(1.0 - b2);
+    h[7] = (float)sqrt(1.0 - pow(b2, (double)t));
+}
+
 __device__ __forceinline__ void hyper_role(const HyperArgs& a, const int i) {
     if (i >= a.n) return;
     const int t = *a.counter[i] + 1;
     *a.counter[i] = t;
     const bool skip = a.skip != nullptr && *a.skip != 0;
     if (a.tap_ring != nullptr && a.counter[i] == a.tap_counter) a.tap_ring[(t - 1) % a.tap_n] = skip ? __int_as_float(0x7fc00000) : *a.tap_src;
-    const double* cfg = a.cfg[i];
+    float h[8];
+    hyper_eval(t, a.cfg[i], skip, h);
     float* hyper = a.hyper[i];
-    const double lr = cfg[0], b1 = cfg[1], b2 = cfg[2], eps = cfg[3], wd = cfg[4];
-    if (skip) {
-        hyper[0] = 0.f; hyper[1] = 1.f; hyper[2] = 1.f; hyper[3] = (float)eps; hyper[4] = 0.f; hyper[5] = 0.f; hyper[6] = 0.f;
-        hyper[7] = 1.f;
-        return;
-    }
-    hyper[0] = (float)(lr / (1.0 - pow(b1, (double)t)));
-    hyper[1] = (float)b1; hyper[2] = (float)b2; hyper[3] = (float)eps; hyper[4] = (float)wd;
-    hyper[5] = (float)(1.0 - b1); hyper[6] = (float)(1.0 - b2);
-    hyper[7] = (float)sqrt(1.0 - pow(b2, (double)t));
+#pragma unroll
+    for (int k = 0; k < 8; ++k) hyper[k] = h[k];
 }
 
 inline int hyper_fill(int n, const void* counter, const void* cfg, const void* hyper, const int* tap_counter, const float* tap_src,
diff --git a/sessionrec-pytorch_amd/csrc/rowops.hip b/sessionrec-pytorch_amd/csrc/rowops.hip
--- a/sessionrec-pytorch_amd/csrc/rowops.hip
+++ b/sessionrec-pytorch_amd/csrc/rowops.hip
@@ -3,11 +3,22 @@
 namespace {
 
 constexpr int WPB = 4;
+
+struct StampArgs { const int* items; int u_cap; const int* dyn_u; int* stamp; const int* counter; int n_rows; };
 
 __global__ void gather_rows_kernel(const float* __restrict__ src, int ld_src, const int* __restrict__ idx,
                                    float* __restrict__ out, int ld_out, int n_cap, const int* __restrict__ dyn,
-                                   int d, srec_rng rng) {
+                                   int d, srec_rng rng, StampArgs sa) {
     const int row = blockIdx.x * WPB + (threadIdx.x >> 6), lane = threadIdx.x & 63;
+    const int nb = (n_cap + WPB - 1) / WPB;
+    if ((int)blockIdx.x >= nb) {
+        const int u = ((int)blockIdx.x - nb) * 256 + (int)threadIdx.x;
+        if (sa.stamp != nullptr && u < dyn_count(sa.dyn_u, sa.u_cap)) {
+            const int it = sa.items[u];
+            if (it >= 0 && it < sa.n_rows) sa.stamp[it] = *sa.counter + 1;
+        }
+        return;
+    }
     if (row >= n_cap) return;
     const int n = dyn_count(dyn, n_cap);
     const int s = row < n ? idx[row] : -1;
@@ -467,7 +478,7 @@
     if (n_cap <= 0) return 0;
     if (bad_row_args(d, ld_src) || (ld_out & 3)) return SREC_BAD_ARG;
     hipLaunchKernelGGL(gather_rows_kernel, dim3(cdiv(n_cap, WPB)), dim3(256), 0, (hipStream_t)stream, src, ld_src, idx,
-                       out, ld_out, n_cap, dyn, d, srec_rng{0u, nullptr, 0u, 0.f});
+                       out, ld_out, n_cap, dyn, d, srec_rng{0u, nullptr, 0u, 0.f}, StampArgs{});
     SREC_LAUNCH_CHECK();
     return 0;
 }
@@ -478,7 +489,20 @@
     if (n_cap <= 0) return 0;
     if (bad_row_args(d, ld_src) || (ld_out & 3) || p < 0.f || p >= 1.f || (long)n_cap * d > 0xffffffffL) return SREC_BAD_ARG;
     hipLaunchKernelGGL(gather_rows_kernel, dim3(cdiv(n_cap, WPB)), dim3(256), 0, (hipStream_t)stream, src, ld_src, idx,
-                       out, ld_out, n_cap, dyn, d, srec_rng{(unsigned)seed, counter, (unsigned)salt, p});
+                       out, ld_out, n_cap, dyn, d, srec_rng{(unsigned)seed, counter, (unsigned)salt, p}, StampArgs{});
+    SREC_LAUNCH_CHECK();
+    return 0;
+}
+
+extern "C" int srec_gather_rows_stamp(const float* src, int ld_src, const int* idx, float* out, int ld_out, int n_cap,
+                                      const int* dyn, int d, float p, int seed, const int* counter, int salt, const int* items,
+                                      int u_cap, const int* dyn_u, int* stamp, const int* stamp_counter, int n_rows, void* stream) {
+    if (n_cap <= 0) return SREC_BAD_ARG;
+    if (bad_row_args(d, ld_src) || (ld_out & 3) || p < 0.f || p >= 1.f || (p > 0.f && (long)n_cap * d > 0xffffffffL)) return SREC_BAD_ARG;
+    if (items == nullptr || stamp == nullptr || stamp_counter == nullptr || u_cap < 0 || n_rows <= 0) return SREC_BAD_ARG;
+    hipLaunchKernelGGL(gather_rows_kernel, dim3(cdiv(n_cap, WPB) + cdiv(u_cap, 256)), dim3(256), 0, (hipStream_t)stream, src, ld_src,
+                       idx, out, ld_out, n_cap, dyn, d, srec_rng{p > 0.f ? (unsigned)seed : 0u, p > 0.f ? counter : nullptr,
+                       p > 0.f ? (unsigned)salt : 0u, p}, StampArgs{items, u_cap, dyn_u, stamp, stamp_counter, n_rows});
     SREC_LAUNCH_CHECK();
     return 0;
 }
diff --git a/sessionrec-pytorch_amd/graph.py b/sessionrec-pytorch_amd/graph.py
--- a/sessionrec-pytorch_amd/graph.py
+++ b/sessionrec-pytorch_amd/graph.py
@@ -85,6 +85,8 @@
                     skip = self._mb['err'] if self._mb is not None else None
                     if hasattr(optimizer, 'hyper_rider') and os.environ.get('SREC_HYPER_RIDER', '1') != '0':
                         optimizer.hyper_rider(tap, skip)
+                    if hasattr(optimizer, 'table_rider'):
+                        optimizer.table_rider(skip)
                     self.loss.backward(self._one)
                     if self.after_backward is not None:
                         self.after_backward()
diff --git a/sessionrec-pytorch_amd/hgat.py b/sessionrec-pytorch_amd/hgat.py
--- a/sessionrec-pytorch_amd/hgat.py
+++ b/sessionrec-pytorch_amd/hgat.py
@@ -174,7 +174,13 @@
     ws = _HG_WS.get(key)
     if ws is None:
         ws = _HG_WS[key] = torch.empty(max(n.value, 1), device=x.device, dtype=torch.float32)
-    lib.srec_hg_bwd(_ct.addressof(desc), ptr(x), _ld(x), ptr(g), _ld(g), ptr(arg), ptr(dx), x.shape[1], ptr(ws), stream())
+    tp = ops.STEP.take_table_pass() if (plan.H == 8 and len(plan.blocks) > 0) else None
+    if tp is not None:
+        lib.srec_hg_bwd_carry(_ct.addressof(desc), ptr(x), _ld(x), ptr(g), _ld(g), ptr(arg), ptr(dx), x.shape[1], ptr(ws),
+                              _ct.addressof(tp['ptrs']), _ct.addressof(tp['ints']), _ct.addressof(tp['flts']), tp['rows_dst'],
+                              tp['n_role'], stream())
+    else:
+        lib.srec_hg_bwd(_ct.addressof(desc), ptr(x), _ld(x), ptr(g), _ld(g), ptr(arg), ptr(dx), x.shape[1], ptr(ws), stream())
     return desc, dP, grads, dx
 
 
diff --git a/sessionrec-pytorch_amd/ops.py b/sessionrec-pytorch_amd/ops.py
--- a/sessionrec-pytorch_amd/ops.py
+++ b/sessionrec-pytorch_amd/ops.py
@@ -416,7 +416,7 @@
 class EmbeddingLookup(torch.autograd.Function):
 
     @staticmethod
-    def forward(ctx, table, idx, uniq, tgrad, dyn_n, dyn_u, drop=None):
+    def forward(ctx, table, idx, uniq, tgrad, dyn_n, dyn_u, drop=None, stamp=None):
         n = idx.numel()
         d = table.shape[1]
         out = torch.empty(n, d, device=table.device, dtype=torch.float32)
@@ -424,6 +424,13 @@
         if drop is not None and drop[0] > 0:
             seed, cnt = rng_args(table.device)
             ctx.drop = (float(drop[0]), seed, cnt, int(drop[1]))
+        if stamp is not None and n > 0 and uniq[0].numel() > 0:
+            pdrop, seed, cnt, salt = ctx.drop if ctx.drop is not None else (0.0, 0, None, 0)
+            lib.srec_gather_rows_stamp(ptr(table), table.stride(0), ptr(idx), ptr(out), d, n, ptr(dyn_n), d, pdrop, seed, cnt, salt,
+                                       ptr(uniq[0]), uniq[0].numel(), ptr(dyn_u), ptr(stamp[0]), ptr(stamp[1]), stamp[0].numel(),
+                                       stream())
+        elif ctx.drop is not None:
+            seed, cnt = ctx.drop[1], ctx.drop[2]
             lib.srec_gather_rows_drop(ptr(table), table.stride(0), ptr(idx), ptr(out), d, n, ptr(dyn_n), d, ctx.drop[0],
                                       seed, cnt, ctx.drop[3], stream())
         else:
@@ -476,11 +483,11 @@
         else:
             first_level(ptr(g), _ld(g), ptr(items), ptr(uptr), ptr(upos), ptr(dst), dst.stride(0), items.numel(),
                         ptr(ctx.dyn_u), acc)
-        return ret, None, None, None, None, None, None
-
-
-def embedding_lookup(table, idx, uniq, tgrad=None, dyn_n=None, dyn_u=None, drop=None):
-    return EmbeddingLookup.apply(table, idx, uniq, tgrad, dyn_n, dyn_u, drop)
+        return ret, None, None, None, None, None, None, None
+
+
+def embedding_lookup(table, idx, uniq, tgrad=None, dyn_n=None, dyn_u=None, drop=None, stamp=None):
+    return EmbeddingLookup.apply(table, idx, uniq, tgrad, dyn_n, dyn_u, drop, stamp)
 
 
 class RowGather(torch.autograd.Function):
diff --git a/sessionrec-pytorch_amd/optim.py b/sessionrec-pytorch_amd/optim.py
--- a/sessionrec-pytorch_amd/optim.py
+++ b/sessionrec-pytorch_amd/optim.py
@@ -1,10 +1,12 @@
 import ctypes as _ct
+import os
 
 import torch
 
-from ._lib import STRUCTS, lib, ptr, ptr_array, stream
+from ._lib import CONST, STRUCTS, lib, ptr, ptr_array, stream
 
 _AdamMultiDesc = STRUCTS['srec_adam_multi_desc']
+TABLE_SPLIT = 0.35
 
 
 class FusedAdam(torch.optim.Optimizer):
@@ -25,6 +27,9 @@
                     tg.radial = torch.zeros(tg.buf.shape[0], device=tg.buf.device, dtype=torch.float32)
         self._hyper = {}
         self._frozen = None
+        self._stamp = None
+        self._stamp_counter = None
+        self.last_table_pass = None
 
     def folds_table_prep(self):
         m = self.model
@@ -186,6 +191,94 @@
             tapped = (None, None, None, 0)
         return (n, _ct.addressof(cs), _ct.addressof(cf), _ct.addressof(hy)) + tapped + (ptr(skip),), (cs, cf, hy, tap, skip)
 
+    def _table_args(self, p, g, tgrad, st):
+        model = self.model
+        cos = model._cosine() if hasattr(model, '_cosine') else None
+        cs_out, cs_scale, eps_mode = None, 1.0, 0
+        if cos is not None and st is not None and st.get('cs') is not None:
+            cs_out, cs_scale, eps_mode = st['cs'], float(cos[0]), int(cos[1])
+        mn_model = float(getattr(model, '_max_norm', 0.0) or 0.0)
+        mn = mn_model if cs_out is not None else 0.0
+        fold = st is not None and self.folds_table_prep()
+        tb = model._table_copy(st, p) if (fold and hasattr(model, '_table_copy')) else None
+        renorm_write = 1 if (fold and mn_model > 0) else 0
+        if renorm_write:
+            mn = mn_model
+        d16, dp16 = (tb.E16, tb.E16.shape[1]) if tb is not None else (None, 0)
+        shard = getattr(model, 'shard', None)
+        n_rows = shard.n_live if (shard is not None and 0 < shard.n_live < p.shape[0]) else p.shape[0]
+        pend = tgrad.pending if (tgrad is not None and g.data_ptr() == tgrad.buf.data_ptr()) else None
+        return dict(cs_out=cs_out, cs_scale=cs_scale, eps_mode=eps_mode, mn=mn, mn_model=mn_model, fold=fold, tb=tb,
+                    renorm_write=renorm_write, d16=d16, dp16=dp16, n_rows=n_rows, pend=pend)
+
+    @staticmethod
+    def _table_key(p, g, state, a, ent):
+        pend = a['pend']
+        return (p.data_ptr(), g.data_ptr(), state['exp_avg'].data_ptr(), state['exp_avg_sq'].data_ptr(), a['n_rows'], p.shape[1],
+                p.stride(0), a['mn'], a['renorm_write'], ptr(a['cs_out']), a['cs_scale'], a['eps_mode'], ptr(a['d16']), a['dp16'],
+                None if pend is None else (ptr(pend[1]), float(pend[2])), ent['counter'].data_ptr())
+
+    def _offer_stamp(self, p, ent, ok):
+        model = self.model
+        if model is None:
+            return
+        if not ok or getattr(model, 'shard', None) is not None:
+            model.__dict__.pop('_srec_stamp', None)
+            self._stamp_counter = None
+            return
+        if self._stamp is None or self._stamp.shape[0] != p.shape[0] or self._stamp.device != p.device:
+            self._stamp = torch.full((p.shape[0],), -1, dtype=torch.int32, device=p.device)
+        if self._stamp_counter is not ent['counter'] or model.__dict__.get('_srec_stamp') is None:
+            self._stamp_counter = ent['counter']
+            model.__dict__['_srec_stamp'] = (self._stamp, ent['counter'])
+
+    def table_rider(self, skip=None):
+        from . import ops
+        ops.STEP.table_pass_result()
+        model = self.model
+        if os.environ.get('SREC_TABLE_EARLY', '1') == '0' or model is None or self._stamp_counter is None:
+            return False
+        if getattr(model, 'shard', None) is not None or getattr(model, 'extra', False) or getattr(model, 'fusion', False):
+            return False
+        if model.__dict__.get('_srec_stamp') is None or not isinstance(getattr(self, '_hyper', None), dict):
+            return False
+        frac = min(max(float(os.environ.get('SREC_TABLE_SPLIT', TABLE_SPLIT)), 0.0), 1.0)
+
+        def build():
+            table, tgrad, st = self._table_info()
+            if tgrad is None or table.grad is not None or (self.grad_override and id(table) in self.grad_override):
+                return None
+            state = self.state.get(table)
+            gi = next((i for i, grp in enumerate(self.param_groups) if any(q is table for q in grp['params'])), None)
+            if gi is None or not state or 'exp_avg' not in state or table.dim() != 2 or not table.is_contiguous():
+                return None
+            ent = self._hyper.get((gi, getattr(self, '_T', 0) - state['step']))
+            if ent is None or ent.get('cfg_host') is None or ent['counter'] is not self._stamp_counter:
+                return None
+            g = tgrad.buf
+            a = self._table_args(table, g, tgrad, st)
+            n, d = a['n_rows'], table.shape[1]
+            if not a['fold'] or (d & 3) or d > 256 or n != table.shape[0] or not g.is_contiguous() or n <= 0:
+                return None
+            pend, C = a['pend'], CONST
+            ptrs, ints, flts = (_ct.c_void_p * C['SREC_TP_NPTR'])(), (_ct.c_int * C['SREC_TP_NINT'])(), (_ct.c_float * C['SREC_TP_NFLT'])()
+            for k, t in (('W', table), ('G', g), ('M', state['exp_avg']), ('V', state['exp_avg_sq']), ('CS_OUT', a['cs_out']),
+                         ('PROJ_CS', pend[1] if pend is not None else None), ('RADIAL', tgrad.radial if pend is not None else None),
+                         ('DST16', a['d16']), ('STAMP', self._stamp), ('COUNTER', ent['counter']), ('CFG', ent['cfg']), ('SKIP', skip)):
+                ptrs[C['SREC_TP_' + k]] = ptr(t)
+            for k, v in (('N', n), ('D', d), ('LD', table.stride(0)), ('USE_WD', 1 if self.param_groups[gi]['weight_decay'] != 0 else 0),
+                         ('RENORM_WRITE', a['renorm_write']), ('EPS_MODE', a['eps_mode']), ('DP', a['dp16'])):
+                ints[C['SREC_TP_' + k]] = v
+            for k, v in (('MAX_NORM', a['mn']), ('CS_SCALE', a['cs_scale']), ('CS_EPS', 1e-12),
+                         ('PROJ_INV_SCALE', float(pend[2]) if pend is not None else 0.0)):
+                flts[C['SREC_TP_' + k]] = v
+            n_role = int(os.environ.get('SREC_TABLE_ROLE_WGS', 0)) or torch.cuda.get_device_properties(table.device).multi_processor_count
+            return dict(ptrs=ptrs, ints=ints, flts=flts, rows_dst=int(frac * n), n_role=max(n_role, 1),
+                        key=self._table_key(table, g, state, a, ent), keep=(skip, pend, state))
+
+        ops.STEP.offer_table_pass(build)
+        return True
+
     def hyper_rider(self, tap=None, skip=None):
         from . import ops
         ops.STEP.rider_result()
@@ -202,6 +295,7 @@
     def launch(self, work, tap=None, skip=None):
         from . import ops as _ops
         done = _ops.STEP.rider_result()
+        taken = _ops.STEP.table_pass_result()
         table, tgrad, st = self._table_info()
         model = self.model
         T = getattr(self, '_T', 0)
@@ -238,34 +332,36 @@
                     multi.setdefault(slot_of[state['step']], []).append((p, g, state))
                     continue
                 if is_table and p.dim() == 2 and (p.shape[1] & 3) == 0:
-                    cos = model._cosine() if hasattr(model, '_cosine') else None
-                    cs_out, cs_scale, eps_mode = None, 1.0, 0
-                    if cos is not None and st is not None and st.get('cs') is not None:
-                        cs_out, cs_scale, eps_mode = st['cs'], float(cos[0]), int(cos[1])
-                    mn_model = float(getattr(model, '_max_norm', 0.0) or 0.0)
-                    mn = mn_model if cs_out is not None else 0.0
-                    fold = st is not None and self.folds_table_prep()
-                    tb = model._table_copy(st, p) if (fold and hasattr(model, '_table_copy')) else None
-                    renorm_write = 1 if (fold and mn_model > 0) else 0
-                    if renorm_write:
-                        mn = mn_model
-                    d16, dp16 = (tb.E16, tb.E16.shape[1]) if tb is not None else (None, 0)
-                    shard = getattr(model, 'shard', None)
-                    n_rows = shard.n_live if (shard is not None and 0 < shard.n_live < p.shape[0]) else p.shape[0]
-                    pend = tgrad.pending if (tgrad is not None and g.data_ptr() == tgrad.buf.data_ptr()) else None
-                    if pend is not None:
-                        lib.srec_adam_rows_proj(ptr(p), ptr(g), ptr(state['exp_avg']), ptr(state['exp_avg_sq']), n_rows,
-                                                p.shape[1], p.stride(0), ptr(hyper), use_wd, mn, renorm_write, ptr(cs_out), cs_scale,
-                                                eps_mode, 1e-12, ptr(pend[1]), float(pend[2]), ptr(tgrad.radial), ptr(d16), dp16,
+                    a = self._table_args(p, g, tgrad, st)
+                    cs_out, fold, tb, renorm_write, mn_model, pend = (a[k] for k in ('cs_out', 'fold', 'tb', 'renorm_write', 'mn_model', 'pend'))
+                    owner = tgrad is not None and g.data_ptr() == tgrad.buf.data_ptr()
+                    ent = self._buffers(gi, slot_of[state['step']], p.device)
+                    self._offer_stamp(p, ent, owner and fold)
+                    if taken is not None:
+                        if taken['key'] != self._table_key(p, g, state, a, ent):
+                            raise RuntimeError('the early part of the table pass ran with other arguments than this step uses (table_rider)')
+                        taken['ptrs'][CONST['SREC_TP_HYPER']] = ptr(hyper)
+                        lib.srec_adam_rows_late(_ct.addressof(taken['ptrs']), _ct.addressof(taken['ints']), _ct.addressof(taken['flts']),
+                                                stream())
+                        taken, self.last_table_pass = None, 'split'
+                        if pend is not None:
+                            tgrad.pending = None
+                            tgrad.radial_dirty = False
+                    elif pend is not None:
+                        self.last_table_pass = 'whole'
+                        lib.srec_adam_rows_proj(ptr(p), ptr(g), ptr(state['exp_avg']), ptr(state['exp_avg_sq']), a['n_rows'],
+                                                p.shape[1], p.stride(0), ptr(hyper), use_wd, a['mn'], renorm_write, ptr(cs_out), a['cs_scale'],
+                                                a['eps_mode'], 1e-12, ptr(pend[1]), float(pend[2]), ptr(tgrad.radial), ptr(a['d16']), a['dp16'],
                                                 stream())
                         tgrad.pending = None
                         tgrad.radial_dirty = False
                     else:
+                        self.last_table_pass = 'whole'
                         if tgrad is not None:
                             tgrad.materialize()
-                        lib.srec_adam_rows(ptr(p), ptr(g), ptr(state['exp_avg']), ptr(state['exp_avg_sq']), n_rows,
-                                           p.shape[1], p.stride(0), ptr(hyper), use_wd, mn, renorm_write, ptr(cs_out), cs_scale,
-                                           eps_mode, 1e-12, ptr(d16), dp16, stream())
+                        lib.srec_adam_rows(ptr(p), ptr(g), ptr(state['exp_avg']), ptr(state['exp_avg_sq']), a['n_rows'],
+                                           p.shape[1], p.stride(0), ptr(hyper), use_wd, a['mn'], renorm_write, ptr(cs_out), a['cs_scale'],
+                                           a['eps_mode'], 1e-12, ptr(a['d16']), a['dp16'], stream())
                     if fold:
                         st['table_prepared'] = (bool(renorm_write) or mn_model <= 0, tb is not None, p._version)
                     if cs_out is not None:
@@ -287,6 +383,8 @@
                 elif wd != 0 and ent[1] == 0:
                     ent[0], ent[1] = gi, wd
                 ent[2] += [(p, g, st_, use_wd) for p, g, st_ in rows]
+        if taken is not None:
+            raise RuntimeError('the early part of the table pass ran, but this step does not update the item table (table_rider)')
         self._join_grads()
         for key, (gi, _, rows) in merged.items():
             slot = key[4]
diff --git a/sessionrec-pytorch_amd/srgnn.py b/sessionrec-pytorch_amd/srgnn.py
--- a/sessionrec-pytorch_amd/srgnn.py
+++ b/sessionrec-pytorch_amd/srgnn.py
@@ -109,7 +109,12 @@
             return rows if (fused or drop is None) else drop(rows)
         if drop is not None and not isinstance(drop, nn.Dropout):
             return drop(ops.embedding_lookup(self._table(), idx, uniq, tgrad, dyn_n, dyn_u))
-        return ops.embedding_lookup(self._table(), idx, uniq, tgrad, dyn_n, dyn_u, (p, 7) if p > 0 else None)
+        stamp = None
+        if tgrad is not None and self.training and torch.is_grad_enabled() and W.is_cuda and torch.cuda.is_current_stream_capturing():
+            stamp = self.__dict__.get('_srec_stamp')
+            if stamp is not None and (stamp[0].device != W.device or stamp[0].shape[0] != W.shape[0]):
+                stamp = None
+        return ops.embedding_lookup(self._table(), idx, uniq, tgrad, dyn_n, dyn_u, (p, 7) if p > 0 else None, stamp)
 
     def fused_loss(self, *inputs_and_labels, dynB=None):
         *inputs, labels = inputs_and_labels
diff --git a/sessionrec-pytorch_amd/stepq.py b/sessionrec-pytorch_amd/stepq.py
--- a/sessionrec-pytorch_amd/stepq.py
+++ b/sessionrec-pytorch_amd/stepq.py
@@ -10,6 +10,7 @@
         self._on, self._depth = False, 0
         self._sums, self._intake = [], []
         self._rider, self._done = None, None
+        self._tpass, self._ttaken = None, None
 
     @property
     def may_defer(self):
@@ -65,6 +66,21 @@
         done, self._rider, self._done = self._done, None, None
         return done
 
+    def offer_table_pass(self, build):
+        self._tpass, self._ttaken = build, None
+
+    def take_table_pass(self):
+        if self._tpass is None:
+            return None
+        rec = self._tpass()
+        if rec is not None:
+            self._tpass, self._ttaken = None, rec
+        return rec
+
+    def table_pass_result(self):
+        rec, self._tpass, self._ttaken = self._ttaken, None, None
+        return rec
+
     def offer_intake(self, entries):
         self._intake = list(entries)
 
@@ -82,3 +98,4 @@
 
     def abort(self):
         self._sums, self._intake, self._rider, self._done = [], [], None, None
+        self._tpass, self._ttaken = None, None
```

Result: slower. 641,700 sessions/s (-5.0%).
